# V-Sense/LFBM5D

Hardware: AMD Instinct MI355X
Metric: SAI-megapixels/sec (HT+Wiener, sigma=25) (higher is better)
Workload: dtype f32; 1 GPU; lf17x17x512x512_sigma25; light_field=17x17x512x512x3, asw=1, color_space=opp, noise=MT19937 seed 1 (utilities.cpp:176-183), window_lanes=2, spatial_bands=1, parallelism=single GPU

## Files before the change

lfbm5d_amd/core.py:

```python
import ctypes as C
import os
import subprocess

from typing import NamedTuple, Optional

import numpy as np

_HERE = os.path.dirname(os.path.abspath(__file__))

YUV, YCBCR, OPP, RGB, ID, DCT, SADCT, BIOR, HADAMARD, HAAR = range(10)
ROWMAJOR, COLMAJOR = 11, 12
TAU = {"id": ID, "dct": DCT, "sadct": SADCT, "bior": BIOR, "hw": HADAMARD, "haar": HAAR}
COLOR_SPACE = {"yuv": YUV, "ycbcr": YCBCR, "opp": OPP, "rgb": RGB}
UNIQUE_ID_BYTES = 128
SR_BICUBIC, SR_GAUSSIAN = 0, 1
SR_UP, SR_DOWN = 0, 1
SR_KERNEL = {"bicubic": SR_BICUBIC, "gaussian": SR_GAUSSIAN}


class LfBm5dError(RuntimeError):
    pass


class Params(C.Structure):
# ... 136 lines not shown
        L.lfbm5d_sr_backproject_device.argtypes = [vp, sp, fp, fp, up, fp] + [C.c_uint] * 4
        L.lfbm5d_superres_device.argtypes = [vp, sp, pp, fp, up, fp] + [C.c_uint] * 7
        L.lfbm5d_superres_host_sai.argtypes = [vp, sp, pp, fp, up, fp] + [C.c_uint] * 7
    L.lfbm5d_malloc.argtypes = [C.POINTER(vp), C.c_size_t]
    L.lfbm5d_free.argtypes = [vp]
    L.lfbm5d_memcpy_h2d.argtypes = [vp, vp, C.c_size_t]
    L.lfbm5d_memcpy_d2h.argtypes = [vp, vp, C.c_size_t]
    L.lfbm5d_device_count.restype = C.c_int
    _lib = L
    return L


def plan_windows(awidth, aheight, an=1, ang_major=None, mask=None):
    ang_major = ROWMAJOR if ang_major is None else ang_major
    m = np.ones(awidth * aheight, np.uint32) if mask is None else _u32(mask)
    out = np.zeros(awidth * aheight, np.uint32)
    n = lib().lfbm5d_plan_windows(awidth, aheight, an, ang_major, m.ctypes.data_as(C.POINTER(C.c_uint)),
                                  out.ctypes.data_as(C.POINTER(C.c_uint)), out.size)
    if n < 0:
        raise LfBm5dError("lfbm5d_plan_windows: bad arguments")
    return out[:n].copy()


def plan_graph(awidth, aheight, world, lanes=1, an=1, ang_major=None, mask=None):
    ang_major = ROWMAJOR if ang_major is None else ang_major
    m = np.ones(awidth * aheight, np.uint32) if mask is None else _u32(mask)
    mp = m.ctypes.data_as(C.POINTER(C.c_uint))
    n = lib().lfbm5d_plan_graph(awidth, aheight, an, ang_major, mp, world, lanes, None, None, None, 0)
    if n < 0:
        raise LfBm5dError("lfbm5d_plan_graph: bad arguments")
    r, l, t = (np.zeros(max(n, 1), np.uint32) for _ in range(3))
    p = lambda a: a.ctypes.data_as(C.POINTER(C.c_uint))
    lib().lfbm5d_plan_graph(awidth, aheight, an, ang_major, mp, world, lanes, p(r), p(l), p(t), n)
    return r[:n], l[:n], t[:n]


def plan_messages(awidth, aheight, world, an=1, ang_major=None, mask=None):
    ang_major = ROWMAJOR if ang_major is None else ang_major
    m = np.ones(awidth * aheight, np.uint32) if mask is None else _u32(mask)
    mp = m.ctypes.data_as(C.POINTER(C.c_uint))
    n = lib().lfbm5d_plan_messages(awidth, aheight, an, ang_major, mp, world, None, 0)
    if n < 0:
        raise LfBm5dError("lfbm5d_plan_messages: bad arguments")
    out = np.zeros((max(n, 1), 4), np.uint32)
    lib().lfbm5d_plan_messages(awidth, aheight, an, ang_major, mp, world, out.ctypes.data_as(C.POINTER(C.c_uint)), n)
    return out[:n]


def plan_job(awidth, aheight, world, lanes=1, an=(1, 1), cost=None, ang_major=None, mask=None):
    ang_major = ROWMAJOR if ang_major is None else ang_major
    m = np.ones(awidth * aheight, np.uint32) if mask is None else _u32(mask)
    p = lambda a: a.ctypes.data_as(C.POINTER(C.c_uint))
    an_a = _u32(list(an))
    cost_a = _u32(list(cost)) if cost is not None else None
    cnt = np.zeros(4, np.uint32)
    n = lib().lfbm5d_plan_job(awidth, aheight, ang_major, p(m), len(an_a), p(an_a), p(cost_a) if cost_a is not None else None,
                              world, lanes, None, 0, None, 0, p(cnt))
    if n < 0:
        raise LfBm5dError("lfbm5d_plan_job: bad arguments")
    nodes = np.zeros((max(int(cnt[0]), 1), 8), np.uint32)
    msgs = np.zeros((max(int(cnt[1]), 1), 6), np.uint32)
    lib().lfbm5d_plan_job(awidth, aheight, ang_major, p(m), len(an_a), p(an_a), p(cost_a) if cost_a is not None else None,
                          world, lanes, p(nodes), int(cnt[0]), p(msgs), int(cnt[1]), p(cnt))
    return nodes[:int(cnt[0])], msgs[:int(cnt[1])], {"windows": int(cnt[0]), "messages": int(cnt[1]), "makespan": int(cnt[2]),
                                                     "centre_ok": bool(cnt[3])}


def auto_bands(awidth, aheight, height, halo, world):
    return int(lib().lfbm5d_auto_bands(int(awidth), int(aheight), int(height), int(halo), int(world)))


def noise_level_statistic(cov):
    cov = np.ascontiguousarray(cov, np.float64)
    d = cov.shape[0]
    sig, m, lam = C.c_double(), C.c_uint(), np.zeros(d, np.float64)
    dp = C.POINTER(C.c_double)
    if lib().lfbm5d_noise_level_statistic(d, cov.ctypes.data_as(dp), C.byref(sig), C.byref(m), lam.ctypes.data_as(dp)) != 0:
        raise LfBm5dError("lfbm5d_noise_level_statistic: bad arguments (d must be 1..64)")
    return sig.value, m.value, lam


def sr_defaults(scale, /, **changes):
    sr = SrParams()
    if lib().lfbm5d_sr_defaults(int(scale), C.byref(sr)) != 0:
        raise LfBm5dError("lfbm5d_sr_defaults: scale must be 2, 3 or 4")
    for k, v in changes.items():
        if k == "kernel" and isinstance(v, str):
            v = SR_KERNEL[v]
        if k not in dict(SrParams._fields_):
            raise LfBm5dError(f"SrParams has no field {k}")
        setattr(sr, k, v)
    return sr


def sr_taps(op, sr, n_in):
    op = {"up": SR_UP, "down": SR_DOWN}.get(op, op)
    T = C.c_uint(0)
    if lib().lfbm5d_sr_taps(int(op), C.byref(sr), int(n_in), None, None, C.byref(T), 0) != 0:
        raise LfBm5dError("lfbm5d_sr_taps: rejected parameters (scale, kernel, blur_sigma, n_in)")
    n_out = int(n_in) * sr.scale if op == SR_UP else int(n_in) // sr.scale
    first, w = np.zeros(n_out, np.int32), np.zeros((n_out, T.value), np.float32)
    if lib().lfbm5d_sr_taps(int(op), C.byref(sr), int(n_in), first.ctypes.data, w.ctypes.data, C.byref(T), w.size) != 0:
        raise LfBm5dError("lfbm5d_sr_taps failed")
    return first, w


def shard_rows(n_rows, rank, world):
    b, e = C.c_uint(), C.c_uint()
    lib().lfbm5d_shard_rows(n_rows, rank, world, C.byref(b), C.byref(e))
    return b.value, e.value


def make_params(sigma, lam, N, nSim, nDisp, k, p, tau_2D, tau_4D, tau_5D, useSD=0, color_space=OPP):
    t = lambda v: TAU[v] if isinstance(v, str) else int(v)
    cs = COLOR_SPACE[color_space] if isinstance(color_space, str) else int(color_space)
    return Params(float(sigma), float(lam), int(N), int(nSim), int(nDisp), int(k), int(p),
                  int(bool(useSD)), t(tau_2D), t(tau_4D), t(tau_5D), cs)


def make_bm3d_params(sigma, lam, N, nHW, k, p, tau_2D, useSD=0, color_space=OPP):
    cs = COLOR_SPACE[color_space] if isinstance(color_space, str) else int(color_space)
    return Bm3dParams(float(sigma), float(lam), int(N), int(nHW), int(k), int(p), int(bool(useSD)),
                      TAU[tau_2D] if isinstance(tau_2D, str) else int(tau_2D), cs)


def _u32(a):
    return np.ascontiguousarray(np.asarray(a, dtype=np.uint32))


def _dev_ptr(t):
    import torch
    if not (isinstance(t, torch.Tensor) and t.is_cuda and t.dtype == torch.float32 and t.is_contiguous()):
        raise LfBm5dError("device entry points need contiguous float32 CUDA tensors")
    torch.cuda.current_stream(t.device).synchronize()
    return C.c_void_p(t.data_ptr())


def _sai_ptrs(arrays, mask):
    out = (C.c_void_p * len(arrays))()
    for i, a in enumerate(arrays):
        if a is None or not mask[i]:
            continue
        if not (isinstance(a, np.ndarray) and a.dtype == np.float32 and a.flags.c_contiguous):
            raise LfBm5dError("per-SAI host buffers must be contiguous float32 numpy arrays")
        out[i] = a.ctypes.data
    return out


OPTION_ENV = ("LFBM5D_LANES", "LFBM5D_EMULATE_WORLD", "LFBM5D_MAX_WINDOWS", "LFBM5D_FUSED", "LFBM5D_STEP_SHARDING",
              "LFBM5D_DATA_DRIVEN_SCHEDULE", "LFBM5D_HOST_BLOCKING", "LFBM5D_BAND_MB", "LFBM5D_BM3D_LANES", "LFBM5D_SCAN_LDS_CAP",
              "LFBM5D_FORCE_REDO", "LFBM5D_SPATIAL_BANDS", "LFBM5D_BAND_HALO", "LFBM5D_SCAN_V1", "LFBM5D_SCAN_ANY", "LFBM5D_SCAN_FULL_TABLES", "LFBM5D_DCT8W_V2",
              "LFBM5D_GROUP_GENERIC", "LFBM5D_NO_SA_KERNELS", "LFBM5D_NO_SLAB_KERNEL", "LFBM5D_WIDE_NOSPLIT", "LFBM5D_AGG_64BIT",
              "LFBM5D_AGG_SCALAR_SCAN", "LFBM5D_SUBSET_LIST_HOST", "LFBM5D_SUBSET_SCAN_V1", "LFBM5D_FILT_GROUP_MAJOR",
              "LFBM5D_HT_REF_ORDER", "LFBM5D_WINDOW_SUMS_PADDED")
OPTION_ENV_EMPTY_OFF = ("LFBM5D_WINDOW_SUMS_PADDED",)


class Context:

    def __init__(self, device=0):
        self._L = lib()
        h = C.c_void_p()
        if self._L.lfbm5d_create(C.byref(h), int(device)) != 0:
            raise LfBm5dError(self._L.lfbm5d_last_error(None).decode())
        self._handle = h
        self._env_seen = {k: os.environ.get(k) for k in OPTION_ENV}
        self.device = int(device)

    @property
    def _h(self):
        h = self._handle
        if h and hasattr(self._L, "lfbm5d_set_option"):
            for k in OPTION_ENV:
                v = os.environ.get(k)
                if v != self._env_seen[k]:
                    self._env_seen[k] = v
                    if not v and k in OPTION_ENV_EMPTY_OFF:
                        v = None
                    self._L.lfbm5d_set_option(h, k.encode(), None if v is None else (v or "1").encode())
        return h

    def set_option(self, key, value):
        if self._L.lfbm5d_set_option(self._handle, key.encode(), None if value is None else str(value).encode()) != 0:
            raise LfBm5dError(self._L.lfbm5d_last_error(self._handle).decode())

    def get_option(self, key):
        buf = C.create_string_buffer(64)
        if self._L.lfbm5d_get_option(self._handle, key.encode(), buf, 64) != 0:
            raise LfBm5dError(self._L.lfbm5d_last_error(self._handle).decode())
        return buf.value.decode()

    def close(self):
        if getattr(self, "_handle", None):
            self._L.lfbm5d_destroy(self._handle)
            self._handle = None

    def __del__(self):
        try:
            self.close()
        except Exception:
            pass

    def _ck(self, rc):
        if rc != 0:
            raise LfBm5dError(self._L.lfbm5d_last_error(self._h).decode())

    @staticmethod
    def unique_id():
        buf = (C.c_ubyte * UNIQUE_ID_BYTES)()
        if lib().lfbm5d_comm_unique_id(buf) != 0:
            raise LfBm5dError("ncclGetUniqueId failed")
        return bytes(buf)

    def comm_init(self, unique_id, rank, world):
        buf = (C.c_ubyte * UNIQUE_ID_BYTES).from_buffer_copy(unique_id)
        self._ck(self._L.lfbm5d_comm_init(self._h, buf, rank, world))

    def comm_init_ipc(self, rank, world, rendezvous_dir, timeout_s=30.0):
        self._ck(self._L.lfbm5d_comm_init_ipc(self._h, rank, world, os.fsencode(rendezvous_dir), float(timeout_s)))

    def comm_selftest(self, n=1 << 20):
        self._ck(self._L.lfbm5d_comm_selftest(self._h, n))

    def comm_ranks(self):
        return int(self._L.lfbm5d_comm_ranks(self._h))

    def set_shard(self, rank, world):
        self._ck(self._L.lfbm5d_set_shard(self._h, rank, world))

    def set_tiles(self, nb_tiles):
        self._ck(self._L.lfbm5d_set_tiles(self._h, int(nb_tiles)))

    def reset_stats(self):
        self._L.lfbm5d_reset_stats(self._h)

    def stats(self):
        s = Stats()
        self._L.lfbm5d_get_stats(self._h, C.byref(s))
        return s

    def stream(self):
        return self._L.lfbm5d_stream(self._h)

    def step1(self, P, noisy, mask, basic, ang_major, awidth, aheight, an, W, H, Cc):
        m = _u32(mask)
        mp = m.ctypes.data_as(C.POINTER(C.c_uint))
        tail = (ang_major, awidth, aheight, an, W, H, Cc)
        if isinstance(noisy, (list, tuple)):
            self._ck(self._L.lfbm5d_step1_host_sai(self._h, C.byref(P), _sai_ptrs(noisy, m), mp, _sai_ptrs(basic, m), *tail))
        elif isinstance(noisy, np.ndarray):
            self._ck(self._L.lfbm5d_step1_host(self._h, C.byref(P), noisy.ctypes.data_as(C.c_void_p), mp,
                                               basic.ctypes.data_as(C.c_void_p), *tail))
        else:
            self._ck(self._L.lfbm5d_step1_device(self._h, C.byref(P), _dev_ptr(noisy), mp, _dev_ptr(basic), *tail))

    def step2(self, P, noisy, mask, basic, denoised, ang_major, awidth, aheight, an, W, H, Cc):
        m = _u32(mask)
        mp = m.ctypes.data_as(C.POINTER(C.c_uint))
        tail = (ang_major, awidth, aheight, an, W, H, Cc)
        if isinstance(noisy, (list, tuple)):
            self._ck(self._L.lfbm5d_step2_host_sai(self._h, C.byref(P), _sai_ptrs(noisy, m), mp, _sai_ptrs(basic, m), _sai_ptrs(denoised, m), *tail))
        elif isinstance(noisy, np.ndarray):
            self._ck(self._L.lfbm5d_step2_host(self._h, C.byref(P), noisy.ctypes.data_as(C.c_void_p), mp,
                                               basic.ctypes.data_as(C.c_void_p),
                                               denoised.ctypes.data_as(C.c_void_p), *tail))
        else:
            self._ck(self._L.lfbm5d_step2_device(self._h, C.byref(P), _dev_ptr(noisy), mp, _dev_ptr(basic),
                                                 _dev_ptr(denoised), *tail))

    def denoise(self, P1, P2, noisy, mask, basic, denoised, ang_major, awidth, aheight, an1, an2, W, H, Cc):
        m = _u32(mask)
        mp = m.ctypes.data_as(C.POINTER(C.c_uint))
        tail = (ang_major, awidth, aheight, an1, an2, W, H, Cc)
        if isinstance(noisy, (list, tuple)):
            self._ck(self._L.lfbm5d_denoise_host_sai(self._h, C.byref(P1), C.byref(P2), _sai_ptrs(noisy, m), mp, _sai_ptrs(basic, m),
                                                     _sai_ptrs(denoised, m), *tail))
        elif isinstance(noisy, np.ndarray):
            self._ck(self._L.lfbm5d_denoise_host(self._h, C.byref(P1), C.byref(P2), noisy.ctypes.data_as(C.c_void_p), mp,
                                                 basic.ctypes.data_as(C.c_void_p), denoised.ctypes.data_as(C.c_void_p), *tail))
        else:
            self._ck(self._L.lfbm5d_denoise_device(self._h, C.byref(P1), C.byref(P2), _dev_ptr(noisy), mp, _dev_ptr(basic),
                                                   _dev_ptr(denoised), *tail))

    def core_pass(self, step, P, aw, ah, Wb, Hb, Cc, noisy, basic, num, den, mask, procSAI, cst, pst):
        m, pr = _u32(mask), _u32(procSAI)
        self._ck(self._L.lfbm5d_pass_device(
            self._h, step, C.byref(P), aw, ah, Wb, Hb, Cc, _dev_ptr(noisy),
            _dev_ptr(basic) if basic is not None else None, _dev_ptr(num), _dev_ptr(den),
            m.ctypes.data_as(C.POINTER(C.c_uint)), pr.ctypes.data_as(C.POINTER(C.c_uint)), cst, pst))

    def bm3d_step(self, step, P, Wb, Hb, Cc, noisy, basic, out):
        self._ck(self._L.lfbm5d_bm3d_step_device(self._h, step, C.byref(P), Wb, Hb, Cc, _dev_ptr(noisy),
                                                 _dev_ptr(basic) if basic is not None else None, _dev_ptr(out)))

    def bm3d_lf(self, hard, wien, noisy, mask, basic, denoised, W, H, Cc):
        m = _u32(mask)
        mp = m.ctypes.data_as(C.POINTER(C.c_uint))
        if isinstance(noisy, np.ndarray):
            self._ck(self._L.lfbm5d_bm3d_lf_host(self._h, C.byref(hard), C.byref(wien), noisy.ctypes.data_as(C.c_void_p), mp,
                                                 basic.ctypes.data_as(C.c_void_p), denoised.ctypes.data_as(C.c_void_p),
                                                 m.size, W, H, Cc))
        else:
            self._ck(self._L.lfbm5d_bm3d_lf_device(self._h, C.byref(hard), C.byref(wien), _dev_ptr(noisy), mp, _dev_ptr(basic),
                                                   _dev_ptr(denoised), m.size, W, H, Cc))

    def noise_level(self, LF, LF_SAI_mask, width, height, chnls, patch=8, per_sai=False):
        m = _u32(LF_SAI_mask)
# ... 192 lines not shown
```

lfbm5d_amd/csrc/lfbm5d_aggregate.hip:

```cpp
#include "lfbm5d_kernels.h"

#include <algorithm>
#include <cstdlib>

namespace lfbm5d {

namespace {



constexpr int kAggFlush = 64;
template <bool WINDOWED, int TW, int TH, int kAggPF, int kAggU, bool BIG, bool VEC4>
__global__ __launch_bounds__(64) __attribute__((amdgpu_waves_per_eu((VEC4 && TW == 8 && !BIG) ? 8 : 1))) void k_aggregate(AggArgs a) {
    constexpr int kAggCap = kAggFlush + kAggPF * 64 + kAggU;
    __shared__ uint4 hit_a[kAggCap];
    __shared__ float hit_w2[kAggCap];
    __shared__ float kai[WINDOWED ? 256 : 1];
    const int lane = threadIdx.x;
    const unsigned org = a.direct ? a.nHW : 0u, Wt = a.Wb - 2 * org, Ht = a.Hb - 2 * org;
    const unsigned gx = (Wt + TW - 1) / TW, gy = (Ht + TH - 1) / TH, total_wg = gx * gy * a.A;
    const unsigned per_xcd = gridDim.x / 8;
    const unsigned lin2 = (blockIdx.x % 8) * per_xcd + blockIdx.x / 8;
    if (lin2 >= total_wg) return;
    const int st = (int)(lin2 / (gx * gy));
    const int tile_y = (int)((lin2 / gx) % gy), tile_x = (int)(lin2 % gx);
    if (a.proc_bits.test((unsigned)st)) return;
    if (!a.mask_bits.test((unsigned)st)) return;
    const int tx0 = (int)org + tile_x * TW, ty0 = (int)org + tile_y * TH;
    const int x = tx0 + lane % TW, y = ty0 + lane / TW;
    const bool inside = x < (int)(org + Wt) && y < (int)(org + Ht);
    const int k = a.k, k2 = k * k, C = a.C, N = a.N, A = a.A;
    const int logN = 31 - __builtin_clz((unsigned)N);
    const size_t plane = (size_t)Wt * Ht;
    const int reach = (st == (int)a.pst) ? (int)a.nSim : (int)a.nHW;
    if (WINDOWED) for (int i = lane; i < k2; i += 64) kai[i] = a.tb->kaiser[i];

    const int last_r = (int)a.Hb - k - (int)a.nHW, last_c = (int)a.Wb - k - (int)a.nHW;
    auto lo_idx = [&](int v) { int d = v - (int)a.nHW; return d <= 0 ? 0 : (d + (int)a.p - 1) / (int)a.p; };
    auto hi_idx = [&](int v, int n, int lastv) {
        if (v >= lastv) return n - 1;
        int d = v - (int)a.nHW; if (d < 0) return -1;
        int i = d / (int)a.p; return i > n - 2 ? n - 2 : i;
    };
    int r_lo = lo_idx(ty0 - k + 1 - reach), r_hi = hi_idx(ty0 + TH - 1 + reach, (int)a.n_ref_rows, last_r);
    int c_lo = lo_idx(tx0 - k + 1 - reach), c_hi = hi_idx(tx0 + TW - 1 + reach, (int)a.n_ref_cols, last_c);
    if (r_lo > (int)a.n_ref_rows - 1) r_lo = (int)a.n_ref_rows - 1;
    if (c_lo > (int)a.n_ref_cols - 1) c_lo = (int)a.n_ref_cols - 1;
    if (!a.irregular && a.n_ref_cols) {
        r_lo = max(r_lo, (int)(a.ref_begin / a.n_ref_cols));
        r_hi = min(r_hi, (int)((a.ref_begin + a.n_groups - 1) / a.n_ref_cols));
    }
    const int ncols_span = c_hi - c_lo + 1;
    const int n_rr = a.irregular ? (int)a.n_groups : ((r_hi >= r_lo && c_hi >= c_lo) ? (r_hi - r_lo + 1) * ncols_span : 0);
    const int n_cand = n_rr << logN;
    if (n_cand == 0) return;

    float accn[3] = {0, 0, 0}, accd[3] = {0, 0, 0};
    const size_t pix = (a.direct ? (size_t)a.sai.st[st] * a.lf_stride : (size_t)st * C * plane) + (size_t)(y - (int)org) * Wt + (size_t)(x - (int)org);
    if (inside) for (int c = 0; c < C; c++) { accn[c] = a.num[pix + c * plane]; accd[c] = a.den[pix + c * plane]; }

    const bool mul_div = !a.irregular && (long long)n_rr * ncols_span < (1 << 20);
    const unsigned div_m = ((1u << 20) + (unsigned)max(ncols_span, 1) - 1) / (unsigned)max(ncols_span, 1);
    const unsigned g_end = a.ref_begin + a.n_groups;
    const bool sai_major = a.filt_sai_stride != 0;
    const unsigned Af = sai_major ? 1u : (unsigned)A, stf = sai_major ? 0u : (unsigned)st;
    const float* const filt = a.filt + (sai_major ? (size_t)st * a.filt_sai_stride : (size_t)0);
    const unsigned long long filt_bytes = sai_major ? a.filt_sai_stride * sizeof(float) : a.filt_bytes;
    const bool small24 = (((unsigned long long)a.n_refs_total << logN) + 1) * Af < (1ull << 24);
    const unsigned* apos = a.aggpos + (size_t)st * a.n_refs_total * N;
    const unsigned cstride = C > 1 ? (unsigned)k2 * 4u : 0u;
    const __amdgpu_buffer_rsrc_t rs_filt = __builtin_amdgcn_make_buffer_rsrc((void*)filt, 0, BIG ? 0 : (int)(unsigned)filt_bytes, 0x00020000u);
    unsigned nh = 0;

    auto consume = [&]() {
        const unsigned nh_pad = (nh + kAggU - 1) / kAggU * kAggU;
        if (nh + lane < nh_pad) { hit_a[nh + lane] = make_uint4(0xffffffffu, 0u, 0u, 0u); hit_w2[nh + lane] = 0.0f; }
        __builtin_amdgcn_wave_barrier();
        for (unsigned h0 = 0; h0 < nh_pad; h0 += kAggU) {
            float val[kAggU][3], kw[kAggU][3];
#pragma unroll
            for (int u = 0; u < kAggU; u++) {
                const uint4 ha = hit_a[h0 + u];
                const float w2 = hit_w2[h0 + u];
                const int dy = y - (int)(ha.x >> 16), dx = x - (int)(ha.x & 0xffffu);
                const bool on = (unsigned)dy < (unsigned)k && (unsigned)dx < (unsigned)k;
                const unsigned o = __umul24((unsigned)min(max(dy, 0), k - 1), (unsigned)k) + (unsigned)min(max(dx, 0), k - 1);
                const float kz = WINDOWED ? kai[o] : 1.0f;
                if (BIG) {
                    const char* fp = reinterpret_cast<const char*>(filt) + ((size_t)ha.y + o) * 4;
                    val[u][0] = *reinterpret_cast<const float*>(fp);
                    val[u][1] = *reinterpret_cast<const float*>(fp + cstride);
                    val[u][2] = *reinterpret_cast<const float*>(fp + 2 * cstride);
                } else {
                    const int vo = (int)((ha.y + o) * 4u);
                    val[u][0] = __builtin_bit_cast(float, __builtin_amdgcn_raw_buffer_load_b32(rs_filt, vo, 0, kFiltLoadAux));
                    val[u][1] = __builtin_bit_cast(float, __builtin_amdgcn_raw_buffer_load_b32(rs_filt, vo, (int)cstride, kFiltLoadAux));
                    val[u][2] = __builtin_bit_cast(float, __builtin_amdgcn_raw_buffer_load_b32(rs_filt, vo, (int)(2 * cstride), kFiltLoadAux));
                }
                kw[u][0] = on ? kz * __uint_as_float(ha.z) : 0.0f;
                kw[u][1] = on ? kz * __uint_as_float(ha.w) : 0.0f;
                kw[u][2] = on ? kz * w2 : 0.0f;
            }
#pragma unroll
            for (int u = 0; u < kAggU; u++)
#pragma unroll
                for (int c = 0; c < 3; c++) {
#pragma clang fp contract(off)
                    accn[c] += kw[u][c] * val[u][c];
                    accd[c] += kw[u][c];
                }
        }
        nh = 0;
        __builtin_amdgcn_wave_barrier();
    };

    __builtin_amdgcn_wave_barrier();
    if (VEC4) {
        constexpr unsigned cap_hits = (unsigned)(kAggCap - kAggU);
        const unsigned lo_y = (unsigned)(ty0 - k + 1), lo_x = (unsigned)(tx0 - k + 1);
        const unsigned span_y = (unsigned)(TH + k - 1), span_x = (unsigned)(TW + k - 1);
        const unsigned pstep = Af * (unsigned)(C * k2);
        auto try_append = [&](const int c0, const unsigned l0, const unsigned l1) -> bool {
            const int e = c0 + lane * 4;
            unsigned g = 0, n0 = 0;
            uint4 p4 = make_uint4(0xffffffffu, 0xffffffffu, 0xffffffffu, 0xffffffffu);
            if (e < n_cand && (unsigned)lane >= l0 && (unsigned)lane < l1) {
                n0 = (unsigned)e & (unsigned)(N - 1);
                const unsigned rr = (unsigned)e >> logN;
                if (a.irregular) g = a.ref_begin + rr;
                else {
                    unsigned q = __umul24(rr, div_m) >> 20;
                    if (!mul_div) { asm volatile("" ::: "memory"); q = rr / (unsigned)ncols_span; }
                    g = __umul24((unsigned)r_lo + q, a.n_ref_cols) + (unsigned)c_lo + (rr - __umul24(q, (unsigned)ncols_span));
                }
                if (g >= a.ref_begin && g < g_end) p4 = *reinterpret_cast<const uint4*>(apos + ((size_t)g << logN) + n0);
            }
            const unsigned pj[4] = {p4.x, p4.y, p4.z, p4.w};
            unsigned m4 = 0;
#pragma unroll
            for (int j = 0; j < 4; j++) {
                const bool h = ((pj[j] >> 16) - lo_y) < span_y && ((pj[j] & 0xffffu) - lo_x) < span_x;
                m4 |= h ? (1u << j) : 0u;
            }
            const unsigned cnt = (unsigned)__popc(m4);
            const unsigned long long b0 = __ballot(cnt & 1u), b1 = __ballot(cnt & 2u), b2 = __ballot(cnt & 4u);
            auto below = [&](unsigned long long b) { return __builtin_amdgcn_mbcnt_hi((unsigned)(b >> 32), __builtin_amdgcn_mbcnt_lo((unsigned)b, 0u)); };
            const unsigned total = (unsigned)__popcll(b0) + 2u * (unsigned)__popcll(b1) + 4u * (unsigned)__popcll(b2);
            if (nh + total > cap_hits) return false;
            if (m4) {
                unsigned slot = nh + below(b0) + 2u * below(b1) + 4u * below(b2);
                size_t wbase; unsigned off;
                const unsigned gl = g - a.ref_begin;
                if (small24) { wbase = __umul24(g, (unsigned)C); off = __umul24(__umul24((gl << logN) + n0, Af) + stf, (unsigned)(C * k2)); }
                else { asm volatile("" ::: "memory"); wbase = (size_t)g * C; off = (((gl << logN) + n0) * Af + stf) * C * k2; }
                float w[3];
#pragma unroll
                for (int c = 0; c < 3; c++) w[c] = c < C ? a.wgt[wbase + (a.wchan0 ? 0 : c)] : 0.0f;
#pragma unroll
                for (int j = 0; j < 4; j++) {
                    if (m4 & (1u << j)) {
                        hit_a[slot] = make_uint4(pj[j], off, __float_as_uint(w[0]), __float_as_uint(w[1]));
                        hit_w2[slot] = w[2];
                        slot++;
                    }
                    off += pstep;
                }
            }
            nh += total;
            __builtin_amdgcn_wave_barrier();
            return true;
        };
        for (int c0 = 0; c0 < n_cand; c0 += 256) {
            if (!try_append(c0, 0u, 64u))
                for (unsigned l0 = 0; l0 < 64; l0 += 16) { consume(); (void)try_append(c0, l0, l0 + 16); }
            if (nh >= kAggFlush) consume();
        }
    } else
    for (int c0 = 0; c0 < n_cand; c0 += 64 * kAggPF) {
        unsigned g[kAggPF], p[kAggPF], nn[kAggPF];
#pragma unroll
        for (int u = 0; u < kAggPF; u++) {
            const int e = c0 + u * 64 + lane;
            p[u] = 0xffffffffu; g[u] = 0; nn[u] = 0;
            if (e < n_cand) {
                const unsigned n = (unsigned)e & (unsigned)(N - 1), rr = (unsigned)e >> logN;
                nn[u] = n;
                if (a.irregular) g[u] = a.ref_begin + rr;
                else {
                    unsigned q = __umul24(rr, div_m) >> 20;
                    if (!mul_div) { asm volatile("" ::: "memory"); q = rr / (unsigned)ncols_span; }
                    g[u] = __umul24((unsigned)r_lo + q, a.n_ref_cols) + (unsigned)c_lo + (rr - __umul24(q, (unsigned)ncols_span));
                }
                if (g[u] >= a.ref_begin && g[u] < g_end) p[u] = apos[((size_t)g[u] << logN) + n];
            }
        }
        bool hit[kAggPF];
        float w[kAggPF][3];
        size_t wbase[kAggPF];
        if (small24) {
#pragma unroll
            for (int u = 0; u < kAggPF; u++) wbase[u] = __umul24(g[u], (unsigned)C);
        } else {
            asm volatile("" ::: "memory");
#pragma unroll
            for (int u = 0; u < kAggPF; u++) wbase[u] = (size_t)g[u] * C;
        }
#pragma unroll
        for (int u = 0; u < kAggPF; u++) {
            const int py = (int)(p[u] >> 16), px = (int)(p[u] & 0xffffu);
            hit[u] = p[u] != 0xffffffffu && py < ty0 + TH && py + k > ty0 && px < tx0 + TW && px + k > tx0;
#pragma unroll
            for (int c = 0; c < 3; c++) w[u][c] = (hit[u] && c < C) ? a.wgt[wbase[u] + (a.wchan0 ? 0 : c)] : 0.0f;
        }
#pragma unroll
        for (int u = 0; u < kAggPF; u++) {
            const unsigned long long bal = __ballot(hit[u]);
            if (hit[u]) {
                const unsigned slot = nh + __popcll(bal & ((1ull << lane) - 1ull));
                unsigned off;
                const unsigned gl = g[u] - a.ref_begin;
                if (small24) off = __umul24(__umul24((gl << logN) + nn[u], Af) + stf, (unsigned)(C * k2));
                else { asm volatile("" ::: "memory"); off = (((gl << logN) + nn[u]) * Af + stf) * C * k2; }
                hit_a[slot] = make_uint4(p[u], off, __float_as_uint(w[u][0]), __float_as_uint(w[u][1]));
                hit_w2[slot] = w[u][2];
            }
            nh += __popcll(bal);
        }
        __builtin_amdgcn_wave_barrier();
        if (nh >= kAggFlush) consume();
    }
    if (nh) consume();
    if (inside) for (int c = 0; c < C; c++) { a.num[pix + c * plane] = accn[c]; a.den[pix + c * plane] = accd[c]; }
}

}

hipError_t launch_aggregate(hipStream_t s, const AggArgs& a) {
    const bool wide = a.k >= 12;
    constexpr int kAgg16TW = 16, kAgg16TH = 4, kAgg8TW = 8, kAgg8TH = 8;
    const unsigned tw = wide ? (a.k == 12 ? 16 : kAgg16TW) : (a.k == 8 ? kAgg8TW : 8), th = wide ? (a.k == 12 ? 4 : kAgg16TH) : (a.k == 8 ? kAgg8TH : 8);
    const unsigned org = a.direct ? a.nHW : 0u;
    const unsigned tiles = ((a.Wb - 2 * org + tw - 1) / tw) * ((a.Hb - 2 * org + th - 1) / th) * a.A;
    const dim3 grid(((tiles + 7) / 8) * 8), block(64);
    const bool big = (a.filt_sai_stride ? a.filt_sai_stride * sizeof(float) : a.filt_bytes) > 0xfffff000ull || (a.opt & kOptAgg64Bit);
    const bool vec4 = a.N % 4 == 0 && !wide && !(a.opt & kOptAggScalarScan);
#define LFBM5D_AGG(W_, TW_, TH_, PF_, U_) \
    do { if (big && vec4) hipLaunchKernelGGL((k_aggregate<W_, TW_, TH_, PF_, U_, true, true>), grid, block, 0, s, a); \
         else if (big)    hipLaunchKernelGGL((k_aggregate<W_, TW_, TH_, PF_, U_, true, false>), grid, block, 0, s, a); \
         else if (vec4)   hipLaunchKernelGGL((k_aggregate<W_, TW_, TH_, PF_, U_, false, true>), grid, block, 0, s, a); \
         else             hipLaunchKernelGGL((k_aggregate<W_, TW_, TH_, PF_, U_, false, false>), grid, block, 0, s, a); } while (0)
    constexpr int kAgg16PF = 3, kAgg16U = 12, kAgg8PF = 3, kAgg8U = 6;
    if (a.k == 12)      LFBM5D_AGG(true, 16, 4, 3, 12);
    else if (a.k == 8)  LFBM5D_AGG(true, kAgg8TW, kAgg8TH, kAgg8PF, kAgg8U);
    else if (wide)      LFBM5D_AGG(false, kAgg16TW, kAgg16TH, kAgg16PF, kAgg16U);
    else                LFBM5D_AGG(false, 8, 8, 2, 6);
#undef LFBM5D_AGG
    return hipGetLastError();
}

}
```

lfbm5d_amd/csrc/lfbm5d_group_device.h:

```cpp
#ifndef LFBM5D_GROUP_DEVICE_H
#define LFBM5D_GROUP_DEVICE_H

#include "lfbm5d_kernels.h"

#include <algorithm>
#include <cstdlib>
#include <type_traits>

namespace lfbm5d {

hipError_t launch_group_ht(hipStream_t s, const GroupArgs& a, bool all_sa, bool* launched);
hipError_t launch_group_wiener(hipStream_t s, const GroupArgs& a, bool all_sa, bool* launched);
hipError_t launch_group_wide(hipStream_t s, const GroupArgs& a, bool* launched);
hipError_t prepare_group_wide();
hipError_t launch_group_slab(hipStream_t s, const GroupArgs& a, bool* launched);
hipError_t prepare_group_slab();
bool group_uses_slab(const GroupArgs& a);
size_t group_slab_scratch_bytes(const GroupArgs& a);
hipError_t prepare_group_ht();
hipError_t prepare_group_wiener();
constexpr int kDedicatedLdsLimit = 160 * 1024 - 4096;

namespace {

typedef const __attribute__((address_space(4))) GroupTables* TbPtr;
typedef const __attribute__((address_space(4))) float* TbFloats;
static inline dim3 grid1d(size_t n, unsigned b = 256) { return dim3((unsigned)((n + b - 1) / b)); }


constexpr int kThreads = 256;

template <int MA, int MW>
struct ShapeInfoT {
    int mask[MA], idx[MA], mask_col[MA], idx_col[MA], mask_dct[MA];
    int row_n[MW], col_n[MW];
    int use_sadct;
};
typedef ShapeInfoT<kMaxA, kMaxAw> ShapeInfo;
typedef ShapeInfoT<kBigA, kBigAw> ShapeInfoBig;
static_assert(sizeof(ShapeInfo) == kShapeInfoBytes && sizeof(ShapeInfoBig) == kShapeInfoBigBytes, "GroupArgs::gshape stride");
typedef const __attribute__((address_space(4))) ShapeInfo& ShRef;
typedef const __attribute__((address_space(4))) ShapeInfoBig& ShRefBig;
__device__ __forceinline__ int window_side(int A) { int w = 1; while (w * w < A) w++; return w; }

template <class SH>
__device__ void build_shape(SH& sh, const int* m, int aw) {
    const int A = aw * aw;
    int size = 0;
    for (int i = 0; i < A; i++) { sh.mask[i] = m[i]; sh.idx[i] = 0; sh.mask_col[i] = 0; sh.idx_col[i] = 0; sh.mask_dct[i] = 0; size += m[i]; }
    for (int s = 0; s < aw; s++) {
        int r = 0;
        for (int t = 0; t < aw; t++) if (m[s * aw + t]) sh.idx[s * aw + r++] = t;
        sh.row_n[s] = r;
        for (int t = 0; t < r; t++) sh.mask_col[s * aw + t] = 1;
    }
    for (int t = 0; t < aw; t++) {
        int r = 0;
        for (int s = 0; s < aw; s++) if (sh.mask_col[s * aw + t]) sh.idx_col[(r++) * aw + t] = s;
        sh.col_n[t] = r;
        for (int s = 0; s < r; s++) sh.mask_dct[s * aw + t] = 1;
    }
    sh.use_sadct = size != A;
}

__device__ __forceinline__ void dct9_fwd(float* x, TbPtr tb) {
    float t[9];
#pragma unroll
    for (int s = 0; s < 3; s++)
#pragma unroll
        for (int u = 0; u < 3; u++)
            t[s * 3 + u] = 2.0f * (x[s * 3] * tb->cos3[u * 3] + x[s * 3 + 1] * tb->cos3[u * 3 + 1] + x[s * 3 + 2] * tb->cos3[u * 3 + 2]);
#pragma unroll
    for (int v = 0; v < 3; v++)
#pragma unroll
        for (int u = 0; u < 3; u++)
            x[v * 3 + u] = 2.0f * (t[u] * tb->cos3[v * 3] + t[3 + u] * tb->cos3[v * 3 + 1] + t[6 + u] * tb->cos3[v * 3 + 2]) * tb->cn4[v * 3 + u];
}
__device__ __forceinline__ void dct9_inv(float* x, TbPtr tb) {
    float t[9];
#pragma unroll
    for (int i = 0; i < 9; i++) x[i] *= tb->cni4[i];
#pragma unroll
    for (int s = 0; s < 3; s++)
#pragma unroll
        for (int j = 0; j < 3; j++)
            t[s * 3 + j] = x[s * 3] + 2.0f * (x[s * 3 + 1] * tb->cos3[3 + j] + x[s * 3 + 2] * tb->cos3[6 + j]);
#pragma unroll
    for (int i = 0; i < 3; i++)
#pragma unroll
        for (int j = 0; j < 3; j++)
            x[i * 3 + j] = (t[j] + 2.0f * (t[3 + j] * tb->cos3[3 + i] + t[6 + j] * tb->cos3[6 + i])) * tb->coef4inv;
}

typedef float v2f __attribute__((ext_vector_type(2)));
typedef float v4f __attribute__((ext_vector_type(4)));
struct __attribute__((packed, aligned(4))) f4u { float v[4]; };
__device__ __forceinline__ void dct9_fwd2(v2f* x, TbPtr tb) {
#pragma clang fp contract(on)
    v2f t[9];
#pragma unroll
    for (int s = 0; s < 3; s++)
#pragma unroll
        for (int u = 0; u < 3; u++)
            t[s * 3 + u] = 2.0f * (x[s * 3] * tb->cos3[u * 3] + x[s * 3 + 1] * tb->cos3[u * 3 + 1] + x[s * 3 + 2] * tb->cos3[u * 3 + 2]);
#pragma unroll
    for (int v = 0; v < 3; v++)
#pragma unroll
        for (int u = 0; u < 3; u++)
            x[v * 3 + u] = 2.0f * (t[u] * tb->cos3[v * 3] + t[3 + u] * tb->cos3[v * 3 + 1] + t[6 + u] * tb->cos3[v * 3 + 2]) * tb->cn4[v * 3 + u];
}
__device__ __forceinline__ void dct9_inv2(v2f* x, TbPtr tb) {
    v2f t[9];
#pragma unroll
    for (int i = 0; i < 9; i++) x[i] *= tb->cni4[i];
#pragma unroll
    for (int s = 0; s < 3; s++)
#pragma unroll
        for (int j = 0; j < 3; j++)
            t[s * 3 + j] = x[s * 3] + 2.0f * (x[s * 3 + 1] * tb->cos3[3 + j] + x[s * 3 + 2] * tb->cos3[6 + j]);
#pragma unroll
    for (int i = 0; i < 3; i++)
#pragma unroll
        for (int j = 0; j < 3; j++)
            x[i * 3 + j] = (t[j] + 2.0f * (t[3 + j] * tb->cos3[3 + i] + t[6 + j] * tb->cos3[6 + i])) * tb->coef4inv;
}
__device__ __forceinline__ void dct9_fwd2_fast(v2f* x, TbPtr tb) {
    const float c2 = 2.0f * tb->cos3[3];
    v2f t[9];
#pragma unroll
    for (int s = 0; s < 3; s++) {
        const v2f a = x[s * 3] + x[s * 3 + 2];
        t[s * 3] = 2.0f * (a + x[s * 3 + 1]);
        t[s * 3 + 1] = c2 * (x[s * 3] - x[s * 3 + 2]);
        t[s * 3 + 2] = a - 2.0f * x[s * 3 + 1];
    }
#pragma unroll
    for (int u = 0; u < 3; u++) {
        const v2f a = t[u] + t[6 + u];
        x[u] = (a + t[3 + u]) * (2.0f * tb->cn4[u]);
        x[3 + u] = (t[u] - t[6 + u]) * (c2 * tb->cn4[3 + u]);
        x[6 + u] = (a - 2.0f * t[3 + u]) * tb->cn4[6 + u];
    }
}
__device__ __forceinline__ void dct9_inv2_fast(v2f* x, TbPtr tb) {
    const float c2 = 2.0f * tb->cos3[3];
    v2f t[9];
#pragma unroll
    for (int s = 0; s < 3; s++) {
        const v2f X0 = x[s * 3] * tb->cni4[s * 3], X1 = x[s * 3 + 1] * (c2 * tb->cni4[s * 3 + 1]), X2 = x[s * 3 + 2] * tb->cni4[s * 3 + 2];
        const v2f p = X0 + X2;
        t[s * 3] = p + X1; t[s * 3 + 1] = X0 - 2.0f * X2; t[s * 3 + 2] = p - X1;
    }
#pragma unroll
    for (int j = 0; j < 3; j++) {
        const v2f T0 = t[j] * tb->coef4inv, T1 = t[3 + j] * (c2 * tb->coef4inv), T2 = t[6 + j] * tb->coef4inv;
        const v2f p = T0 + T2;
        x[j] = p + T1; x[3 + j] = T0 - 2.0f * T2; x[6 + j] = p - T1;
    }
}
template <int NS> __device__ __forceinline__ void haar_fwd_pairs(v2f* P) {
#pragma clang fp contract(on)
    const float s = 0.70710678118654752f;
    if (NS == 8) {
        const v2f S01 = (P[0] + P[1]) * s, D01 = (P[0] - P[1]) * s, S23 = (P[2] + P[3]) * s, D23 = (P[2] - P[3]) * s;
        const v2f SS = (S01 + S23) * s, DD = (S01 - S23) * s;
// ... 1191 lines not shown
```

lfbm5d_amd/csrc/lfbm5d_group_generic.hip:

```cpp
#include "lfbm5d_group_device.h"

namespace lfbm5d {

namespace {

__global__ __launch_bounds__(256) void k_group_pos(GroupArgs a) {
    const int A = a.A, N = a.N, NA = N * A;
    const size_t plane = (size_t)a.Wb * a.Hb;
    const size_t idx = (size_t)blockIdx.x * blockDim.x + threadIdx.x;
    if (idx == 0 && a.sa_list) a.sa_list[0] = 0u;
    if (idx >= (size_t)a.n_groups * N) return;
    const unsigned g = a.ref_begin + (unsigned)(idx / N);
    const int n = (int)(idx % N);
    const int nSx = (int)a.self_cnt[g];
    const unsigned k_r = a.refs[g];
    const unsigned ind_pst = n < nSx ? a.self_idx[(size_t)g * N + n] : 0u;
    const bool want_ofs = A == 9 && a.tau2 == 4 && a.step == 1 && (size_t)A * a.C * plane * 4 < 0x7fffffffull;
    unsigned bits = 0;
    for (int st = 0; st < A; st++) {
        const bool masked = a.mask_bits.test((unsigned)st);
        unsigned p = 0xffffffffu;
        if (n < nSx && masked) p = (st == (int)a.pst) ? ind_pst : a.best[(size_t)st * plane + ind_pst];
        const bool zero_patch = a.fill_quirk && p != 0xffffffffu && (p % a.Wb) >= a.Wb - a.k;
        const int i = n * A + st;
        a.gpos[(size_t)g * NA + i] = zero_patch ? 0xffffffffu : p;
        if (want_ofs) {
            const bool there = !zero_patch && p != 0xffffffffu;
            a.gofs[(size_t)g * NA + i] = there ? (unsigned)(((size_t)st * a.C * plane + p) * 4) : 0u;
            bits |= there ? 1u << st : 0u;
        }
        const bool in_shape = st == (int)a.pst || (masked && a.shape[(size_t)st * plane + k_r]);
        a.aggpos[((size_t)st * a.n_refs_total + g) * N + n] = ((a.tau4 != 6 || in_shape) && p != 0xffffffffu) ? ((p / a.Wb) << 16) | (p % a.Wb) : 0xffffffffu;
    }
    if (want_ofs) a.gok[(size_t)g * N + n] = bits;
}
template <bool BIG>
__global__ __launch_bounds__(256) void k_group_shape(GroupArgs a) {
    typedef typename std::conditional<BIG, ShapeInfoBig, ShapeInfo>::type SH;
    const unsigned i = blockIdx.x * blockDim.x + threadIdx.x;
    if (i >= a.n_groups) return;
    const unsigned g = a.ref_begin + i;
    const size_t plane = (size_t)a.Wb * a.Hb;
    const unsigned k_r = a.refs[g];
    SH* out = reinterpret_cast<SH*>(a.gshape) + g;
    if (a.tau4 != 6) { out->use_sadct = 0; return; }
    const int A = (int)a.A, aw = window_side(A);
    if (BIG) {
        int* m = out->mask_dct;
        int full = 0;
        for (int st = 0; st < A; st++) {
            const bool masked = a.mask_bits.test((unsigned)st);
            m[st] = (st == (int)a.pst || (masked && a.shape[(size_t)st * plane + k_r])) ? 1 : 0;
            full += m[st];
        }
        if (full == A) { out->use_sadct = 0; return; }
        for (int st = 0; st < A; st++) out->mask[st] = m[st];
        build_shape(*out, out->mask, aw);
        return;
    }
    SH sh;
    int m[BIG ? 1 : kMaxA], full = 0;
    for (int st = 0; st < A; st++) {
        const bool masked = a.mask_bits.test((unsigned)st);
        m[st] = (st == (int)a.pst || (masked && a.shape[(size_t)st * plane + k_r])) ? 1 : 0;
        full += m[st];
    }
    if (full == A) { out->use_sadct = 0; return; }
    build_shape(sh, m, aw);
    for (int q = 0; q < A; q++) {
        out->mask[q] = sh.mask[q]; out->idx[q] = sh.idx[q]; out->mask_col[q] = sh.mask_col[q];
        out->idx_col[q] = sh.idx_col[q]; out->mask_dct[q] = sh.mask_dct[q];
    }
    for (int q = 0; q < aw; q++) { out->row_n[q] = sh.row_n[q]; out->col_n[q] = sh.col_n[q]; }
    out->use_sadct = sh.use_sadct;
    if (sh.use_sadct && a.sa_list) a.sa_list[1u + atomicAdd(&a.sa_list[0], 1u)] = g | (7u << 29);
}
template <int STEP, bool BIG = false>
__device__ __forceinline__ void group_generic(const GroupArgs& a, const unsigned g, const int c, float* S0, float* S1, float* tmp,
                                              unsigned* pos, float (*red)[kThreads / 64]) {
    const int tid = threadIdx.x;
    const int k = a.k, k2 = k * k, A = a.A, N = a.N;
    const int aw = window_side(A);
    const int nSx = (int)a.self_cnt[g];
    const size_t plane = (size_t)a.Wb * a.Hb;
    const int stack = nSx * A * k2;
    const TbPtr tb = (TbPtr)a.tb;

    for (int i = tid; i < nSx * A; i += kThreads) pos[i] = a.gpos[(size_t)g * N * A + i];
    typename std::conditional<BIG, ShRefBig, ShRef>::type sh = [&]() -> typename std::conditional<BIG, ShRefBig, ShRef>::type {
        if constexpr (BIG) return group_shape_big(a, g); else return group_shape(a, g); }();
    __syncthreads();
    const bool use_sadct = a.tau4 == 6 && sh.use_sadct;

    {
        constexpr int G = 12;
        for (int e0 = tid; e0 < stack; e0 += kThreads * G) {
            float v0[G], v1[G];
#pragma unroll
            for (int u = 0; u < G; u++) {
                const int e = e0 + u * kThreads;
                v0[u] = 0.0f; v1[u] = 0.0f;
                if (e < stack) {
                    const int pq = e % k2, ns = e / k2;
                    const int st = ns % A;
                    const unsigned p = pos[ns];
                    if (p != 0xffffffffu) {
                        const size_t off = ((size_t)st * a.C + c) * plane + p + (size_t)(pq / k) * a.Wb + pq % k;
                        v0[u] = a.noisy[off];
                        if (STEP == 2) v1[u] = a.basic[off];
                    }
                }
            }
#pragma unroll
            for (int u = 0; u < G; u++) {
                const int e = e0 + u * kThreads;
                if (e < stack) { S0[e] = v0[u]; if (STEP == 2) S1[e] = v1[u]; }
            }
        }
    }
    __syncthreads();

    if (a.tau2 != 4) {
        fwd2d(S0, tmp, nSx * A, k, a.tau2, tb);
        if (STEP == 2) fwd2d(S1, tmp, nSx * A, k, a.tau2, tb);
    }

    const bool do_dct4 = a.tau4 == 5 || (a.tau4 == 6 && !use_sadct);
    const bool do_sa4 = !do_dct4 && a.tau4 == 6;
    if (do_dct4 || do_sa4) {
        for (int f = tid; f < nSx * k2; f += kThreads) {
            const int n = f / k2, pq = f % k2;
            for (int s = 0; s < (STEP == 2 ? 2 : 1); s++) {
                float* S = s ? S1 : S0;
                if constexpr (BIG) {
                    float x[kBigA], t[kBigA];
                    for (int st = 0; st < A; st++) x[st] = S[(size_t)(n * A + st) * k2 + pq];
                    if (do_dct4) dctw_fwd_rt(x, t, aw, tb); else sadctw_fwd<ShRefBig>(x, aw, sh, tb);
                    for (int st = 0; st < A; st++) S[(size_t)(n * A + st) * k2 + pq] = x[st];
                } else
                if (A == 9) {
                    float x[9];
#pragma unroll
                    for (int st = 0; st < 9; st++) x[st] = S[(n * A + st) * k2 + pq];
                    if (do_dct4) dct9_fwd(x, tb); else sadct9_fwd(x, sh, tb);
#pragma unroll
                    for (int st = 0; st < 9; st++) S[(n * A + st) * k2 + pq] = x[st];
                } else if (do_dct4 && A == 25) {
                    float x[25];
#pragma unroll
                    for (int st = 0; st < 25; st++) x[st] = S[(n * 25 + st) * k2 + pq];
                    dctw_fwd_t<5>(x, tb);
#pragma unroll
                    for (int st = 0; st < 25; st++) S[(n * 25 + st) * k2 + pq] = x[st];
                } else if (do_dct4) {
                    float x[49];
#pragma unroll
                    for (int st = 0; st < 49; st++) x[st] = S[(n * 49 + st) * k2 + pq];
                    dctw_fwd_t<7>(x, tb);
#pragma unroll
                    for (int st = 0; st < 49; st++) S[(n * 49 + st) * k2 + pq] = x[st];
                } else {
                    float x[kMaxA];
                    for (int st = 0; st < A; st++) x[st] = S[(n * A + st) * k2 + pq];
                    if constexpr (!BIG) sadctw_fwd<ShRef>(x, aw, sh, tb);
                    for (int st = 0; st < A; st++) S[(n * A + st) * k2 + pq] = x[st];
                }
            }
        }
        __syncthreads();
    }

    float wacc = 0.0f, s1 = 0.0f, s2 = 0.0f;
    {
        const float sig = a.sigma[c];
        const float T = a.bm3d ? a.lambda * sig : a.lambda * sig * 1.41421356237309505f;
        const float sig2 = sig * sig;
        for (int f = tid; f < A * k2; f += kThreads) {
            const int st = f / k2, pq = f % k2;
            const bool in_shape = !use_sadct || sh.mask_dct[st];
            const int base = st * k2 + pq, stride = A * k2;
            switch (nSx) {
                case 1:  filter5<1, STEP>(S0, S1, base, stride, a.tau5, T, sig2, in_shape, wacc, s1, s2, tb); break;
                case 2:  filter5<2, STEP>(S0, S1, base, stride, a.tau5, T, sig2, in_shape, wacc, s1, s2, tb); break;
                case 4:  filter5<4, STEP>(S0, S1, base, stride, a.tau5, T, sig2, in_shape, wacc, s1, s2, tb); break;
                case 8:  filter5<8, STEP>(S0, S1, base, stride, a.tau5, T, sig2, in_shape, wacc, s1, s2, tb); break;
                case 16: filter5<16, STEP>(S0, S1, base, stride, a.tau5, T, sig2, in_shape, wacc, s1, s2, tb); break;
                default: filter5<32, STEP>(S0, S1, base, stride, a.tau5, T, sig2, in_shape, wacc, s1, s2, tb); break;   
            }
        }
    }
    for (int o = 32; o > 0; o >>= 1) { wacc += __shfl_xor(wacc, o); s1 += __shfl_xor(s1, o); s2 += __shfl_xor(s2, o); }
    if ((tid & 63) == 0) { red[0][tid >> 6] = wacc; red[1][tid >> 6] = s1; red[2][tid >> 6] = s2; }
    __syncthreads();
    if (tid == 0) {
        float w = 0.0f, m = 0.0f, q = 0.0f;
        for (int i = 0; i < kThreads / 64; i++) { w += red[0][i]; m += red[1][i]; q += red[2][i]; }
        float wx;
        if (a.useSD) {
            const float Nn = a.bm3d ? (float)(nSx * k2) : (float)(nSx * A);
            const float res = (q - m * m / Nn) / (Nn - 1.0f);
            wx = res > 0.0f ? 1.0f / sqrtf(res) : 0.0f;
        } else {
            const float sig = a.sigma[c];
            wx = w > 0.0f ? (sig > 0.0f ? 1.0f / (sig * sig * w) : 1.0f / w) : 1.0f;
        }
        a.wgt[(size_t)g * a.C + c] = wx;
        if (c == 0) {
            atomicAdd(&a.counters[0], (unsigned long long)nSx);
            if (use_sadct) atomicAdd(&a.counters[1], 1ull);
        }
    }
    float* F = STEP == 2 ? S1 : S0;

    if (do_dct4 || do_sa4) {
        for (int f = tid; f < nSx * k2; f += kThreads) {
            const int n = f / k2, pq = f % k2;
            if constexpr (BIG) {
                float x[kBigA], t[kBigA];
                for (int st = 0; st < A; st++) x[st] = F[(size_t)(n * A + st) * k2 + pq];
                if (do_dct4) dctw_inv_rt(x, t, aw, tb); else sadctw_inv<ShRefBig>(x, aw, sh, tb);
                for (int st = 0; st < A; st++) F[(size_t)(n * A + st) * k2 + pq] = x[st];
            } else
            if (A == 9) {
                float x[9];
#pragma unroll
                for (int st = 0; st < 9; st++) x[st] = F[(n * A + st) * k2 + pq];
                if (do_dct4) dct9_inv(x, tb); else sadct9_inv(x, sh, tb);
#pragma unroll
                for (int st = 0; st < 9; st++) F[(n * A + st) * k2 + pq] = x[st];
            } else if (do_dct4 && A == 25) {
                float x[25];
#pragma unroll
                for (int st = 0; st < 25; st++) x[st] = F[(n * 25 + st) * k2 + pq];
                dctw_inv_t<5>(x, tb);
#pragma unroll
                for (int st = 0; st < 25; st++) F[(n * 25 + st) * k2 + pq] = x[st];
            } else if (do_dct4) {
                float x[49];
#pragma unroll
                for (int st = 0; st < 49; st++) x[st] = F[(n * 49 + st) * k2 + pq];
                dctw_inv_t<7>(x, tb);
#pragma unroll
                for (int st = 0; st < 49; st++) F[(n * 49 + st) * k2 + pq] = x[st];
            } else {
                float x[kMaxA];
                for (int st = 0; st < A; st++) x[st] = F[(n * A + st) * k2 + pq];
                if constexpr (!BIG) sadctw_inv<ShRef>(x, aw, sh, tb);
                for (int st = 0; st < A; st++) F[(n * A + st) * k2 + pq] = x[st];
            }
        }
    }
    __syncthreads();
    if (a.tau2 != 4) inv2d(F, tmp, nSx * A, k, a.tau2, tb);

    for (int e = tid; e < stack; e += kThreads) {
        const int pq = e % k2, ns = e / k2;
        filt_put(&a.filt[filt_patch(a, g, ns / A, ns % A, k2) + (size_t)c * k2 + pq], F[e]);
    }
}

template <int STEP>
__global__ __launch_bounds__(kThreads) void k_group(GroupArgs a) {
    extern __shared__ float lds[];
    __shared__ unsigned pos[kMaxN3 * kMaxA];
    __shared__ float red[3][kThreads / 64];
    const unsigned g = a.ref_begin + blockIdx.x;
    const int stack = (int)a.self_cnt[g] * (int)a.A * (int)(a.k * a.k);
    group_generic<STEP>(a, g, (int)blockIdx.y, lds, STEP == 2 ? lds + stack : nullptr, lds + (STEP == 2 ? 2 : 1) * stack, pos, red);
}

template <int STEP, bool BIG>
__global__ __launch_bounds__(kThreads) void k_group_big(GroupArgs a, float* scratch, unsigned long long slice_floats, unsigned tmp_floats) {
    extern __shared__ float lds[];
    __shared__ unsigned pos_small[BIG ? 1 : kMaxN3 * kMaxA];
    __shared__ float red[3][kThreads / 64];
    unsigned* pos = BIG ? reinterpret_cast<unsigned*>(lds + tmp_floats) : pos_small;
    float* S0 = scratch + (size_t)blockIdx.x * slice_floats;
    const unsigned items = a.n_groups * a.C;
    for (unsigned it = blockIdx.x; it < items; it += gridDim.x) {
        const unsigned g = a.ref_begin + it / a.C;
        const int stack = (int)a.self_cnt[g] * (int)a.A * (int)(a.k * a.k);
        group_generic<STEP, BIG>(a, g, (int)(it % a.C), S0, STEP == 2 ? S0 + stack : nullptr, lds, pos, red);
        __syncthreads();
    }
}

}

constexpr int kGenericLdsLimit = 160 * 1024 - 8192;
hipError_t prepare_group_kernels() {
    const void* fns[] = {reinterpret_cast<const void*>(&k_group<1>), reinterpret_cast<const void*>(&k_group<2>)};
    for (const void* f : fns) {
        const hipError_t e = hipFuncSetAttribute(f, hipFuncAttributeMaxDynamicSharedMemorySize, kGenericLdsLimit);
        if (e != hipSuccess) return e;
    }
    hipError_t e = prepare_group_ht();
    if (e == hipSuccess) e = prepare_group_wiener();
    if (e == hipSuccess) e = prepare_group_wide();
    if (e == hipSuccess) e = prepare_group_slab();
    return e;
}

constexpr unsigned kBigBlocks = 1024;
static size_t group_tmp_floats(const GroupArgs& a) {
    const bool rows_form = (a.tau2 == 7 && (a.k == 8 || a.k == 16)) || (a.tau2 == 5 && (a.k == 8 || a.k == 12 || a.k == 16));
    return rows_form ? (size_t)(kThreads / a.k) * a.k * (a.k + 1) : std::max<size_t>(256, (size_t)a.k * a.k);
}
size_t group_lds_bytes(const GroupArgs& a) {
    const size_t stack = (size_t)a.N * a.A * a.k * a.k;
    return ((a.step == 2 ? 2 : 1) * stack + group_tmp_floats(a)) * sizeof(float);
}
static bool group_uses_generic(const GroupArgs& a) {
    if (a.opt & kOptGroupGeneric) return true;
    bool wide_window = false;
    for (unsigned w = 5; w <= 17; w += 2) wide_window |= a.A == w * w;
    if (wide_window && a.tau2 == 4 && a.step == 1 && !a.bm3d && a.N <= 8 && a.k * a.k <= 256 && (size_t)a.A * a.C * a.Wb * a.Hb * 4 < 0x7fffffffull) return false;
    if (a.A != 9 && !(a.bm3d && a.A == 1)) return true;
    if (a.A == 9 && a.tau2 == 4 && a.N <= 8 && a.k * a.k <= 256 && a.step == 1) return false;
    if (a.A == 9 && (a.tau2 == 7 || a.tau2 == 5) && a.k == 16 && a.N <= 8 && a.step == 1) return false;
    if (a.A == 9 && a.tau2 == 7 && a.k == 8 && a.step == 2 && a.N <= (unsigned)kMaxN) return false;
    if (a.A == 9 && a.tau2 == 5 && a.k == 8 && a.N <= (unsigned)kMaxN) return false;
    if (a.bm3d && a.A == 1 && a.k == 8 && a.tau5 == 8 && (a.tau2 == 5 || a.tau2 == 7)) return false;
    return true;
}
size_t group_scratch_bytes(const GroupArgs& a) {
    if (group_uses_generic(a) && !(a.opt & kOptGroupGeneric) && group_uses_slab(a)) return group_slab_scratch_bytes(a);
    if (!group_uses_generic(a) || (group_lds_bytes(a) <= (size_t)kGenericLdsLimit && a.A <= (unsigned)kMaxA)) return 0;
    return (size_t)kBigBlocks * (a.step == 2 ? 2 : 1) * a.N * a.A * a.k * a.k * sizeof(float);
}
hipError_t launch_group(hipStream_t s, const GroupArgs& a) {
    hipLaunchKernelGGL(k_group_pos, grid1d((size_t)a.n_groups * a.N), dim3(256), 0, s, a);
    const bool bigA = a.A > (unsigned)kMaxA;
    if (bigA) hipLaunchKernelGGL(k_group_shape<true>, grid1d(a.n_groups), dim3(256), 0, s, a);
    else      hipLaunchKernelGGL(k_group_shape<false>, grid1d(a.n_groups), dim3(256), 0, s, a);
    const bool all_sa = a.tau4 == 6 && !a.mask_bits.holds_all(a.A) && !(a.opt & kOptNoSaKernels);
    if (!(a.opt & kOptGroupGeneric)) {
        bool launched = false;
        hipError_t e = launch_group_ht(s, a, all_sa, &launched);
        if (launched) return e;
        e = launch_group_wiener(s, a, all_sa, &launched);
        if (launched) return e;
        e = launch_group_wide(s, a, &launched);
        if (launched) return e;
        e = launch_group_slab(s, a, &launched);
        if (launched) return e;
    }
    const size_t lds = group_lds_bytes(a);
    if (lds > (size_t)kGenericLdsLimit || bigA) {
        const unsigned long long slice = (unsigned long long)(a.step == 2 ? 2 : 1) * a.N * a.A * a.k * a.k;
        if (!a.scratch || a.scratch_floats < slice * kBigBlocks) return hipErrorInvalidValue;
        const unsigned blocks = std::min<unsigned>(kBigBlocks, a.n_groups * a.C);
        const unsigned tf = (unsigned)group_tmp_floats(a);
        const size_t ltmp = (size_t)tf * sizeof(float) + (bigA ? (size_t)a.N * a.A * sizeof(unsigned) : 0);
        if (bigA) {
            if (a.step == 2) hipLaunchKernelGGL((k_group_big<2, true>), dim3(blocks), dim3(kThreads), ltmp, s, a, a.scratch, slice, tf);
            else             hipLaunchKernelGGL((k_group_big<1, true>), dim3(blocks), dim3(kThreads), ltmp, s, a, a.scratch, slice, tf);
        }
        else if (a.step == 2) hipLaunchKernelGGL((k_group_big<2, false>), dim3(blocks), dim3(kThreads), ltmp, s, a, a.scratch, slice, tf);
        else                  hipLaunchKernelGGL((k_group_big<1, false>), dim3(blocks), dim3(kThreads), ltmp, s, a, a.scratch, slice, tf);
        return hipGetLastError();
    }
    if (a.step == 2) hipLaunchKernelGGL(k_group<2>, dim3(a.n_groups, a.C), dim3(kThreads), lds, s, a);
    else             hipLaunchKernelGGL(k_group<1>, dim3(a.n_groups, a.C), dim3(kThreads), lds, s, a);
    return hipGetLastError();
}
}
```

lfbm5d_amd/csrc/lfbm5d_group_ht.hip:

```cpp
#include "lfbm5d_group_device.h"

namespace lfbm5d {

namespace {

__device__ __forceinline__ constexpr float ht_guard(int st) { return st == 0 ? 1.0f / 65536.0f : (st == 3 || st == 6) ? 1.0f / 131072.0f : 1.0f / 262144.0f; }
template <int NS> __device__ __forceinline__ void haar_fwd_pairs_u(v2f* P) {
    if (NS == 8) {
        const v2f S01 = P[0] + P[1], D01 = P[0] - P[1], S23 = P[2] + P[3], D23 = P[2] - P[3];
        const v2f SS = S01 + S23, DD = S01 - S23;
        P[0] = v2f{SS.x + SS.y, SS.x - SS.y}; P[1] = DD; P[2] = D01; P[3] = D23;
    } else if (NS == 4) {
        const v2f S = P[0] + P[1], D = P[0] - P[1];
        P[0] = v2f{S.x + S.y, S.x - S.y}; P[1] = D;
    } else if (NS == 2) {
        P[0] = v2f{P[0].x + P[0].y, P[0].x - P[0].y};
    }
}
template <int NS> __device__ __forceinline__ void haar_inv_pairs_u(v2f* P) {
    if (NS == 8) {
        const v2f X = v2f{P[0].x + P[0].y, P[0].x - P[0].y};
        const v2f U = P[1] * 2.0f + X, V = X - P[1] * 2.0f, D01 = P[2], D23 = P[3];
        P[0] = D01 * 4.0f + U; P[1] = U - D01 * 4.0f; P[2] = D23 * 4.0f + V; P[3] = V - D23 * 4.0f;
    } else if (NS == 4) {
// ... 26 lines not shown
            const v2f p = t[u] + t[6 + u];
            V[h][u] = p + t[3 + u]; V[h][3 + u] = t[u] - t[6 + u]; V[h][6 + u] = p - 2.0f * t[3 + u];
        }
    }
    const float inv_n = 1.0f / (float)NS;
    unsigned kept = 0;
    unsigned long long near = 0ull;
#pragma unroll
    for (int st = 0; st < 9; st++) {
        v2f P[NH];
#pragma unroll
        for (int h = 0; h < NH; h++) P[h] = V[h][st];
        haar_fwd_pairs_u<NS>(P);
        const float gs = fmaxf(ht_guard(st), a.ht3_K[c][st] * M);
#pragma unroll
        for (int h = 0; h < NH; h++) {
            const int lvl = h == 0 ? LV : (NS == 8 && h == 1) ? 2 : 1;
            const float Tq = a.ht3_T[c][st][lvl], Gq = Tq * gs;
            const float ax = fabsf(P[h].x), ay = fabsf(P[h].y);
            const bool kx = ax > Tq, ky = (NS > 1) && ay > Tq;
            near |= __ballot(fabsf(ax - Tq) < Gq);
            if (NS > 1) near |= __ballot(fabsf(ay - Tq) < Gq);
            kept += (unsigned)__popcll(__ballot(kx)) + (NS > 1 ? (unsigned)__popcll(__ballot(ky)) : 0u);
            P[h].x = kx ? P[h].x : 0.0f;
            P[h].y = ky ? P[h].y : 0.0f;
        }
        haar_inv_pairs_u<NS>(P);
#pragma unroll
        for (int h = 0; h < NH; h++) V[h][st] = P[h];
    }
    if (near) return true;
    wacc += (__lane_id() == 0) ? (float)kept : 0.0f;
    if (a.useSD) {
#pragma unroll
        for (int h = 0; h < NH; h++)
#pragma unroll
            for (int st = 0; st < 9; st++) {
                const v2f y = V[h][st] * (tb->ht3_f[st] * inv_n);
                s1 += y.x; s2 += y.x * y.x;
                if (NS > 1) { s1 += y.y; s2 += y.y * y.y; }
            }
    }
#pragma unroll
    for (int h = 0; h < NH; h++) {
        v2f t[9];
#pragma unroll
        for (int s = 0; s < 3; s++) {
            const v2f Z0 = V[h][s * 3] * (tb->ht3_gf[s * 3] * inv_n), Z1 = V[h][s * 3 + 1] * (tb->ht3_gf[s * 3 + 1] * inv_n), Z2 = V[h][s * 3 + 2] * (tb->ht3_gf[s * 3 + 2] * inv_n);
            const v2f p = Z0 + Z2;
            t[s * 3] = p + Z1; t[s * 3 + 1] = Z0 - 2.0f * Z2; t[s * 3 + 2] = p - Z1;
        }
#pragma unroll
        for (int j = 0; j < 3; j++) {
            const v2f p = t[j] + t[6 + j];
            V[h][j] = p + t[3 + j]; V[h][3 + j] = t[j] - 2.0f * t[6 + j]; V[h][6 + j] = p - t[3 + j];
        }
    }
    return false;
}

template <int NS, bool HAAR, int SA_MODE = 0>
__device__ __forceinline__ void group_id_compute(const GroupArgs& a, int c, ShRef sh, bool use_sadct, v2f (&V)[NS > 1 ? NS / 2 : 1][9],
                                                 float& wacc, float& s1, float& s2, float* sa_lds = nullptr) {
    constexpr int NH = NS > 1 ? NS / 2 : 1;
    const TbPtr tb = (TbPtr)a.tb;
    const bool do_dct4 = a.tau4 == 5 || (a.tau4 == 6 && !use_sadct);
    const bool do_sa4 = SA_MODE != 3 && !do_dct4 && a.tau4 == 6;
    auto sadct_pairs = [&](bool fwd) {
#pragma unroll
        for (int h = 0; h < NH; h++)
#pragma unroll
            for (int half = 0; half < (NS > 1 ? 2 : 1); half++) {
                if (SA_MODE == 1) {
#pragma unroll
                    for (int i = 0; i < 9; i++) sa_lds[i] = half ? V[h][i].y : V[h][i].x;
                    if (fwd) sadct9_fwd_lds(sa_lds, sh, tb); else sadct9_inv_lds(sa_lds, sh, tb);
#pragma unroll
                    for (int i = 0; i < 9; i++) { if (half) V[h][i].y = sa_lds[i]; else V[h][i].x = sa_lds[i]; }
                } else {
                    float t9[9];
#pragma unroll
                    for (int i = 0; i < 9; i++) t9[i] = half ? V[h][i].y : V[h][i].x;
                    if (SA_MODE == 2) { if (fwd) sadct9_fwd_sel(t9, sh, tb); else sadct9_inv_sel(t9, sh, tb); }
                    else if (fwd) sadct9_fwd(t9, sh, tb); else sadct9_inv(t9, sh, tb);
#pragma unroll
                    for (int i = 0; i < 9; i++) { if (half) V[h][i].y = t9[i]; else V[h][i].x = t9[i]; }
                }
            }
    };
    if (do_dct4) {
#pragma unroll
        for (int h = 0; h < NH; h++) dct9_fwd2(V[h], tb);
    } else if (do_sa4) sadct_pairs(true);
    const float sig = a.sigma[c];
    const float T = a.lambda * sig * 1.41421356237309505f;
#pragma unroll
    for (int st = 0; st < 9; st++) {
        const bool in_shape = !use_sadct || sh.mask_dct[st];
        if (HAAR) {
            v2f P[NH];
#pragma unroll
            for (int h = 0; h < NH; h++) P[h] = V[h][st];
            haar_fwd_pairs<NS>(P);
            if (in_shape) {
#pragma unroll
                for (int h = 0; h < NH; h++) {
                    const bool kx = fabsf(P[h].x) > T, ky = (NS > 1) && fabsf(P[h].y) > T;
                    wacc += (kx ? 1.0f : 0.0f) + (ky ? 1.0f : 0.0f);
                    P[h].x = kx ? P[h].x : 0.0f;
                    P[h].y = ky ? P[h].y : 0.0f;
                }
            }
            haar_inv_pairs<NS>(P);
#pragma unroll
            for (int h = 0; h < NH; h++) V[h][st] = P[h];
        } else {
            float o[NS], e[1] = {0.0f};
#pragma unroll
            for (int n = 0; n < NS; n++) o[n] = n < NH ? V[n][st].x : V[n - NH][st].y;
            shrink_fibre<NS, 1>(o, e, a.tau5, T, sig * sig, in_shape, wacc, tb);
#pragma unroll
            for (int n = 0; n < NS; n++) { if (n < NH) V[n][st].x = o[n]; else V[n - NH][st].y = o[n]; }
        }
    }
    if (a.useSD) {
#pragma unroll
        for (int h = 0; h < NH; h++)
#pragma unroll
            for (int st = 0; st < 9; st++) {
                s1 += V[h][st].x; s2 += V[h][st].x * V[h][st].x;
                if (NS > 1) { s1 += V[h][st].y; s2 += V[h][st].y * V[h][st].y; }
            }
    }
    if (do_dct4) {
#pragma unroll
        for (int h = 0; h < NH; h++) dct9_inv2(V[h], tb);
    } else if (do_sa4) sadct_pairs(false);
}

template <int NS, bool HAAR, bool LDSW = false, int SA_MODE = 0, bool FAST = false>
__device__ __forceinline__ bool group_id_body(const GroupArgs& a, unsigned g, int c, int pq, const __attribute__((address_space(4))) unsigned* pos,
                                              ShRef sh, bool use_sadct, float& wacc, float& s1, float& s2, float* work = nullptr) {
    const int k = a.k, k2 = k * k, A = 9;
    const unsigned plane = a.Wb * a.Hb;
    const unsigned kRsrcFlags = 0x00020000u;
    const __amdgpu_buffer_rsrc_t rs_in = __builtin_amdgcn_make_buffer_rsrc((void*)a.noisy, 0, (int)((size_t)a.A * a.C * plane * 4), kRsrcFlags);
    float* const out = a.filt + (size_t)g * a.N * A * a.C * k2;
    const __amdgpu_buffer_rsrc_t rs_out = __builtin_amdgcn_make_buffer_rsrc((void*)out, 0, (int)((size_t)a.N * A * a.C * k2 * 4), kRsrcFlags);
    constexpr int NH = NS > 1 ? NS / 2 : 1;
    v2f V[NH][9];
    const int voff = (int)(((unsigned)(pq / k) * a.Wb + pq % k) * 4u);
    const int woff = (pq / k) * (k + 1) + pq % k;
    unsigned okbits[NS];
    typedef const __attribute__((address_space(4))) unsigned* cuptr_;
    const cuptr_ ofs = (cuptr_)(a.gofs + (size_t)g * a.N * A), ok = (cuptr_)(a.gok + (size_t)g * a.N);
    const unsigned cbase = (unsigned)c * plane * 4u;
    auto load_all = [&]() {
        if (LDSW) {
#pragma unroll
            for (int n = 0; n < NS; n++)
#pragma unroll
                for (int st = 0; st < 9; st++) {
                    const float x = work[(n * A + st) * kT16Patch + woff];
                    if (n < NH) V[n][st].x = x; else V[n - NH][st].y = x;
                    okbits[n] = 0x1ffu;
                }
        } else
#pragma unroll
        for (int n = 0; n < NS; n++) {
            okbits[n] = ok[n];
#pragma unroll
            for (int st = 0; st < 9; st++) {
                const unsigned so = ofs[n * A + st] + cbase;
                const float x = __builtin_bit_cast(float, __builtin_amdgcn_raw_buffer_load_b32(rs_in, voff, (int)so, 0));
                if (n < NH) V[n][st].x = x; else V[n - NH][st].y = x;
            }
        }
        if (NS == 1) {
#pragma unroll
            for (int st = 0; st < 9; st++) V[0][st].y = 0.0f;
        }
#pragma unroll
        for (int n = 0; n < NS; n++)
            if (okbits[n] != 0x1ffu) {
#pragma unroll
                for (int st = 0; st < 9; st++) {
                    if (n < NH) V[n][st].x = ((okbits[n] >> st) & 1) ? V[n][st].x : 0.0f;
                    else V[n - NH][st].y = ((okbits[n] >> st) & 1) ? V[n - NH][st].y : 0.0f;
                }
            }
    };
    load_all();
    bool near = false;
    if (FAST) near = group_id_compute_fast<NS>(a, c, V, wacc, s1, s2);
    else
    group_id_compute<NS, HAAR, SA_MODE>(a, c, sh, use_sadct, V, wacc, s1, s2);
    const int vout = pq * 4;
#pragma unroll
    for (int n = 0; n < NS; n++)
#pragma unroll
        for (int st = 0; st < 9; st++) {
            const float r = n < NH ? V[n][st].x : V[n - NH][st].y;
            if (LDSW) work[(n * A + st) * kT16Patch + woff] = r;
            else __builtin_amdgcn_raw_buffer_store_b32(__builtin_bit_cast(int, r), rs_out, vout, (int)((((unsigned)(n * A + st) * a.C + c) * k2) * 4u), kFiltStoreAux);
        }
    return near;
}

template <bool HAAR, int SA_MODE, bool FAST = false>
__device__ __forceinline__ void group_id_one(const GroupArgs& a, const unsigned g, const int c, float (*red)[4]) {
    const int tid = threadIdx.x;
    const int A = 9, N = a.N;
    const int nSx = (int)a.self_cnt[g];
    typedef const __attribute__((address_space(4))) unsigned* cuptr;
    const cuptr pos = (cuptr)(a.gpos + (size_t)g * N * A);
    ShRef sh = group_shape(a, g);
    const bool use_sadct = a.tau4 == 6 && sh.use_sadct;
    if (SA_MODE == 3 && use_sadct) return;
    float wacc = 0.0f, s1 = 0.0f, s2 = 0.0f;
    bool near = false;
    if (tid < (int)(a.k * a.k)) {
        switch (nSx) {
            case 1:  near = group_id_body<1, HAAR, false, SA_MODE, FAST>(a, g, c, tid, pos, sh, use_sadct, wacc, s1, s2); break;
            case 2:  near = group_id_body<2, HAAR, false, SA_MODE, FAST>(a, g, c, tid, pos, sh, use_sadct, wacc, s1, s2); break;
            case 4:  near = group_id_body<4, HAAR, false, SA_MODE, FAST>(a, g, c, tid, pos, sh, use_sadct, wacc, s1, s2); break;
            default: near = group_id_body<8, HAAR, false, SA_MODE, FAST>(a, g, c, tid, pos, sh, use_sadct, wacc, s1, s2); break;
        }
    }
    for (int o = 32; o > 0; o >>= 1) { wacc += __shfl_xor(wacc, o); s1 += __shfl_xor(s1, o); s2 += __shfl_xor(s2, o); }
    if ((tid & 63) == 0) { red[0][tid >> 6] = wacc; red[1][tid >> 6] = s1; red[2][tid >> 6] = s2; if (FAST) red[3][tid >> 6] = near ? 1.0f : 0.0f; }
    __syncthreads();
    if (tid == 0) {
        if (FAST) {
            float nr = 0.0f;
            for (unsigned i = 0; i < (blockDim.x + 63) / 64; i++) nr += red[3][i];
            if (nr != 0.0f) {
                a.sa_list[1u + atomicAdd(&a.sa_list[0], 1u)] = g | (1u << (29 + c)); return;
            }
        }
        float w = 0.0f, m = 0.0f, q = 0.0f;
        for (unsigned i = 0; i < (blockDim.x + 63) / 64; i++) { w += red[0][i]; m += red[1][i]; q += red[2][i]; }
        float wx;
        if (a.useSD) {
            const float Nn = (float)(nSx * A);
            const float res = (q - m * m / Nn) / (Nn - 1.0f);
            wx = res > 0.0f ? 1.0f / sqrtf(res) : 0.0f;
        } else {
            const float sig = a.sigma[c];
            wx = w > 0.0f ? (sig > 0.0f ? 1.0f / (sig * sig * w) : 1.0f / w) : 1.0f;
        }
        a.wgt[(size_t)g * a.C + c] = wx;
        if (c == 0) {
            atomicAdd(&a.counters[0], (unsigned long long)nSx);
            if (use_sadct) atomicAdd(&a.counters[1], 1ull);
        }
    }
}

template <bool HAAR, int SA_MODE, bool FAST>
__device__ __forceinline__ void group_id_kernel(const GroupArgs& a) {
    __shared__ float red[4][4];
    const unsigned gi = xcd_group_index(a);
    if (gi >= a.n_groups) return;
    group_id_one<HAAR, SA_MODE, FAST>(a, a.ref_begin + gi, (int)blockIdx.y, red);
}
template <bool HAAR>
__device__ __forceinline__ void group_id_list_kernel(const GroupArgs& a) {
    __shared__ float red[4][4];
    const unsigned n = a.sa_list[0];
    for (unsigned i = blockIdx.x; i < n; i += gridDim.x) {
        const unsigned e = a.sa_list[1u + i];
        for (unsigned c = 0; c < a.C; c++)
            if ((e >> (29 + c)) & 1u) {
                group_id_one<HAAR, 2>(a, e & 0x1fffffffu, (int)c, red);
                __syncthreads();
            }
    }
}
__global__ __launch_bounds__(256) void k_group_id_haar_fast(GroupArgs a) { group_id_kernel<true, 3, true>(a); }
__global__ __launch_bounds__(256) void k_group_id_haar(GroupArgs a) { group_id_kernel<true, 3, false>(a); }
__global__ __launch_bounds__(256) void k_group_id_any(GroupArgs a) { group_id_kernel<false, 3, false>(a); }
__global__ __launch_bounds__(256) __attribute__((amdgpu_waves_per_eu(3, 3))) void k_group_id_haar_sa(GroupArgs a) { group_id_kernel<true, 2, false>(a); }
__global__ __launch_bounds__(256) void k_group_id_any_sa(GroupArgs a) { group_id_kernel<false, 2, false>(a); }
constexpr unsigned kSaListBlocks = 2048;
__global__ __launch_bounds__(256) void k_group_id_haar_list(GroupArgs a) { group_id_list_kernel<true>(a); }
__global__ __launch_bounds__(256) void k_group_id_any_list(GroupArgs a) { group_id_list_kernel<false>(a); }

constexpr int kT16Groups = 3;
constexpr int kT16Half = 40;
constexpr int kT16Waves = 3;
template <bool HAAR, bool BIOR, bool MULTI, bool SPLIT = false, bool SA = false>
__device__ __forceinline__ void group_t16_kernel(const GroupArgs& a) {
    extern __shared__ float lds[];
    __shared__ float red[MULTI ? kT16Groups : 1][3][4];
    constexpr int K = 16, RS = K + 1, PSZ = kT16Patch, A = 9;
    const int tid = threadIdx.x;
    const unsigned g = a.ref_begin + blockIdx.x * (MULTI ? kT16Groups : 1);
    const int ngr = MULTI ? (int)min((unsigned)kT16Groups, a.ref_begin + a.n_groups - g) : 1;
    const int c = blockIdx.y;
    const int N = a.N;
    const int nSx = MULTI ? 1 : (int)a.self_cnt[g], NP = MULTI ? ngr * A : nSx * A;
    typedef const __attribute__((address_space(4))) unsigned* cuptr;
    const cuptr pos = (cuptr)(a.gpos + (size_t)g * N * A);
    ShRef sh = group_shape(a, g);
    const bool use_sadct = a.tau4 == 6 && sh.use_sadct;
    const TbPtr tb = (TbPtr)a.tb;
    float* work = lds;
#ifdef LFBM5D_PHASE_TIMING
    long long tq[6]; int tqi = 0;
#define T16_MARK() do { if (tid == 0) tq[tqi] = (long long)__builtin_readcyclecounter(); tqi++; } while (0)
    T16_MARK();
#else
#define T16_MARK() do {} while (0)
#endif
    const size_t plane = (size_t)a.Wb * a.Hb;
    auto patch_src = [&](int patch, bool& ok) -> const float* {
        const unsigned p = a.gpos[(size_t)g * N * A + patch];
        ok = p != 0xffffffffu;
        return a.noisy + ((size_t)(patch % A) * a.C + c) * plane + (ok ? p : 0u);
    };
    auto fwd2d = [&](const int base, const int np) {
        if (BIOR) {
            constexpr int TPP = 8, PPI = kThreads / TPP;
            const int slot = tid / TPP, r = tid % TPP;
            for (int p0 = 0; p0 < np; p0 += PPI) {
                const int patch = p0 + slot;
                if (patch < np) {
                    bool ok;
                    const float* src = patch_src(base + patch, ok);
                    v2f v[K], o[K];
    #pragma unroll
                    for (int q = 0; q < 4; q++) {
                        const f4u lo = *reinterpret_cast<const f4u*>(src + (size_t)r * a.Wb + 4 * q);
                        const f4u hi = *reinterpret_cast<const f4u*>(src + (size_t)(r + 8) * a.Wb + 4 * q);
    #pragma unroll
                        for (int e = 0; e < 4; e++) v[4 * q + e] = ok ? v2f{lo.v[e], hi.v[e]} : v2f{0.0f, 0.0f};
                    }
                    bior_taps2<K, true>(v, o, tb);
                    float* Tp = work + patch * PSZ;
    #pragma unroll
                    for (int cc = 0; cc < K; cc++) { Tp[r * RS + cc] = o[cc].x; Tp[(r + 8) * RS + cc] = o[cc].y; }
                    __builtin_amdgcn_wave_barrier();
                    bior16_pass2<K, true, false>(Tp, r, tb);
                }
            }
            __syncthreads();
            bior16_level_all<8, true>(work, np, tid, tb);
            bior16_level_all<4, true>(work, np, tid, tb);
            bior16_level_all<2, true>(work, np, tid, tb);
        } else {
            const int slot = tid / K, r = tid % K;
            for (int p0 = 0; p0 < np; p0 += kThreads / K) {
                const int patch = p0 + slot;
                if (patch < np) {
                    bool ok;
                    const float* src = patch_src(base + patch, ok);
                    float x[K];
// ... 35 lines not shown
                    v2f v[K], o[K];
    #pragma unroll
                    for (int cc = 0; cc < K; cc++) v[cc] = v2f{Tp[r * RS + cc], Tp[(r + 8) * RS + cc]};
                    bior_taps2<K, false>(v, o, tb);
                    float4* dst = reinterpret_cast<float4*>(out + ((size_t)(base + patch) * a.C + c) * K * K);
    #pragma unroll
                    for (int q = 0; q < 4; q++) {
                        filt_put4(&dst[r * 4 + q], make_float4(o[4 * q].x, o[4 * q + 1].x, o[4 * q + 2].x, o[4 * q + 3].x));
                        filt_put4(&dst[(r + 8) * 4 + q], make_float4(o[4 * q].y, o[4 * q + 1].y, o[4 * q + 2].y, o[4 * q + 3].y));
                    }
                }
            }
        } else {
            const int slot = tid / K, r = tid % K;
            for (int p0 = 0; p0 < np; p0 += kThreads / K) {
                const int patch = p0 + slot;
                if (patch < np) {
                    float* Tp = work + patch * PSZ;
                    float x[K];
    #pragma unroll
                    for (int i = 0; i < K; i++) x[i] = Tp[i * RS + r];
                    dct16_inv(x);
    #pragma unroll
                    for (int i = 0; i < K; i++) Tp[i * RS + r] = x[i];
                    __builtin_amdgcn_wave_barrier();
    #pragma unroll
                    for (int cc = 0; cc < K; cc++) x[cc] = Tp[r * RS + cc];
                    dct16_inv(x);
                    float4* dst = reinterpret_cast<float4*>(out + ((size_t)(base + patch) * a.C + c) * K * K);
    #pragma unroll
                    for (int q = 0; q < 4; q++) filt_put4(&dst[r * 4 + q], make_float4(x[4 * q], x[4 * q + 1], x[4 * q + 2], x[4 * q + 3]));
                }
            }
        }
    };
    float wacc[MULTI ? kT16Groups : 1], s1[MULTI ? kT16Groups : 1], s2[MULTI ? kT16Groups : 1];
    const bool split = SPLIT && !MULTI;
    if (!split) { fwd2d(0, NP); T16_MARK(); }
    if (MULTI) {
#pragma unroll
        for (int gi = 0; gi < kT16Groups; gi++) {
            wacc[gi] = 0.0f; s1[gi] = 0.0f; s2[gi] = 0.0f;
            if (gi < ngr) {
                ShRef shg = group_shape(a, g + gi);
                group_id_body<1, HAAR, true, SA ? 2 : 0>(a, g + gi, c, tid, pos + gi * A, shg, a.tau4 == 6 && shg.use_sadct, wacc[gi], s1[gi], s2[gi],
                                                         work + gi * A * PSZ);
            }
        }
    } else if (SPLIT) {
        wacc[0] = 0.0f; s1[0] = 0.0f; s2[0] = 0.0f;
        const int woff = (tid / K) * RS + tid % K;
        auto rounds = [&](auto ns_tag) {
            constexpr int NS = decltype(ns_tag)::value, NH = NS > 1 ? NS / 2 : 1, NPc = NS * A, PR = kT16Half, NR = (NPc + PR - 1) / PR, F0 = NPc - (NR - 1) * PR;
            v2f V[NH][9];
            auto put = [&](const int pch, const float x) { if (pch / 9 < NH) V[pch / 9][pch % 9].x = x; else V[pch / 9 - NH][pch % 9].y = x; };
            auto get = [&](const int pch) { return pch / 9 < NH ? V[pch / 9][pch % 9].x : V[pch / 9 - NH][pch % 9].y; };
            if (NS == 1) {
#pragma unroll
                for (int st = 0; st < 9; st++) V[0][st].y = 0.0f;
            }
#pragma unroll
            for (int r = 0; r < NR; r++) {
                const int b0 = r == 0 ? 0 : F0 + (r - 1) * PR, cnt = r == 0 ? F0 : PR;
                fwd2d(b0, cnt);
#pragma unroll
                for (int q = 0; q < PR; q++) if (q < cnt) put(b0 + q, work[q * PSZ + woff]);
                __syncthreads();
            }
            T16_MARK();
            group_id_compute<NS, HAAR, BIOR ? 2 : 1>(a, c, sh, use_sadct, V, wacc[0], s1[0], s2[0], work + tid * 9);
            __syncthreads();
            T16_MARK();
#pragma unroll
            for (int r = NR - 1; r >= 0; r--) {
                const int b0 = r == 0 ? 0 : F0 + (r - 1) * PR, cnt = r == 0 ? F0 : PR;
#pragma unroll
                for (int q = 0; q < PR; q++) if (q < cnt) work[q * PSZ + woff] = get(b0 + q);
                __syncthreads();
                inv2d(b0, cnt);
                if (r > 0) __syncthreads();
            }
        };
        switch (nSx) {
            case 1:  rounds(std::integral_constant<int, 1>{}); break;
            case 2:  rounds(std::integral_constant<int, 2>{}); break;
            case 4:  rounds(std::integral_constant<int, 4>{}); break;
            default: rounds(std::integral_constant<int, 8>{}); break;
        }
    } else {
        wacc[0] = 0.0f; s1[0] = 0.0f; s2[0] = 0.0f;
        switch (nSx) {
            case 1:  group_id_body<1, HAAR, true>(a, g, c, tid, pos, sh, use_sadct, wacc[0], s1[0], s2[0], work); break;
            case 2:  group_id_body<2, HAAR, true>(a, g, c, tid, pos, sh, use_sadct, wacc[0], s1[0], s2[0], work); break;
            case 4:  group_id_body<4, HAAR, true>(a, g, c, tid, pos, sh, use_sadct, wacc[0], s1[0], s2[0], work); break;
            default: group_id_body<8, HAAR, true>(a, g, c, tid, pos, sh, use_sadct, wacc[0], s1[0], s2[0], work); break;
        }
    }
    if (!split) { __syncthreads(); T16_MARK(); inv2d(0, NP); }
    T16_MARK();
#ifdef LFBM5D_PHASE_TIMING
    T16_MARK();
    if (tid == 0) { for (int i = 0; i < 5; i++) atomicAdd(&a.counters[4 + i], (unsigned long long)(tq[i + 1] - tq[i])); atomicAdd(&a.counters[9], 1ull); }
#endif
#pragma unroll
    for (int gi = 0; gi < (MULTI ? kT16Groups : 1); gi++) {
        for (int o = 32; o > 0; o >>= 1) { wacc[gi] += __shfl_xor(wacc[gi], o); s1[gi] += __shfl_xor(s1[gi], o); s2[gi] += __shfl_xor(s2[gi], o); }
        if ((tid & 63) == 0) { red[gi][0][tid >> 6] = wacc[gi]; red[gi][1][tid >> 6] = s1[gi]; red[gi][2][tid >> 6] = s2[gi]; }
    }
    __syncthreads();
    if (tid < ngr) {
        const int gi = tid;
        float w = 0.0f, m = 0.0f, q = 0.0f;
        for (int i = 0; i < 4; i++) { w += red[gi][0][i]; m += red[gi][1][i]; q += red[gi][2][i]; }
        float wx;
        if (a.useSD) {
            const float Nn = (float)(nSx * A);
            const float res = (q - m * m / Nn) / (Nn - 1.0f);
            wx = res > 0.0f ? 1.0f / sqrtf(res) : 0.0f;
        } else {
            const float sig = a.sigma[c];
            wx = w > 0.0f ? (sig > 0.0f ? 1.0f / (sig * sig * w) : 1.0f / w) : 1.0f;
        }
        a.wgt[(size_t)(g + gi) * a.C + c] = wx;
        if (c == 0) {
            atomicAdd(&a.counters[0], (unsigned long long)nSx);
            if (a.tau4 == 6 && group_shape(a, g + gi).use_sadct) atomicAdd(&a.counters[1], 1ull);
        }
    }
}
__global__ __launch_bounds__(256) __attribute__((amdgpu_waves_per_eu(kT16Waves, kT16Waves))) void k_group_bior16_haar(GroupArgs a) { group_t16_kernel<true, true, false, true>(a); }
__global__ __launch_bounds__(256) void k_group_bior16_any(GroupArgs a) { group_t16_kernel<false, true, false>(a); }
__global__ __launch_bounds__(256) __attribute__((amdgpu_waves_per_eu(kT16Waves, kT16Waves))) void k_group_dct16_haar(GroupArgs a) { group_t16_kernel<true, false, false, true>(a); }
__global__ __launch_bounds__(256) void k_group_dct16_any(GroupArgs a) { group_t16_kernel<false, false, false>(a); }
__global__ __launch_bounds__(256) void k_group_bior16_n1(GroupArgs a) { group_t16_kernel<true, true, true>(a); }
__global__ __launch_bounds__(256) void k_group_dct16_n1(GroupArgs a) { group_t16_kernel<true, false, true>(a); }
__global__ __launch_bounds__(256) void k_group_bior16_n1_sa(GroupArgs a) { group_t16_kernel<true, true, true, false, true>(a); }
__global__ __launch_bounds__(256) void k_group_dct16_n1_sa(GroupArgs a) { group_t16_kernel<true, false, true, false, true>(a); }

}

hipError_t prepare_group_ht() {
    const void* fns[] = {
        reinterpret_cast<const void*>(&k_group_bior16_haar), reinterpret_cast<const void*>(&k_group_bior16_any),
        reinterpret_cast<const void*>(&k_group_dct16_haar), reinterpret_cast<const void*>(&k_group_dct16_any),
        reinterpret_cast<const void*>(&k_group_bior16_n1), reinterpret_cast<const void*>(&k_group_dct16_n1),
        reinterpret_cast<const void*>(&k_group_bior16_n1_sa), reinterpret_cast<const void*>(&k_group_dct16_n1_sa)};
    for (const void* f : fns) {
        const hipError_t e = hipFuncSetAttribute(f, hipFuncAttributeMaxDynamicSharedMemorySize, kDedicatedLdsLimit);
        if (e != hipSuccess) return e;
    }
    return hipSuccess;
}

hipError_t launch_group_ht(hipStream_t s, const GroupArgs& a, bool all_sa, bool* launched) {
    *launched = true;
    if (a.tau2 == 4 && a.N <= 8 && a.k * a.k <= 256 && a.step == 1 && a.A == 9 && (size_t)a.A * a.C * a.Wb * a.Hb * 4 < 0x7fffffffull) {
        const unsigned threads = ((a.k * a.k + 63) / 64) * 64;
        const unsigned gx = ((a.n_groups + 7) / 8) * 8;
        if (all_sa) {
            if (a.tau5 == 9) hipLaunchKernelGGL(k_group_id_haar_sa, dim3(gx, a.C), dim3(threads), 0, s, a);
            else             hipLaunchKernelGGL(k_group_id_any_sa, dim3(gx, a.C), dim3(threads), 0, s, a);
        }
        else {
            if (!a.sa_list) return hipErrorInvalidValue;
            const bool fast = a.tau5 == 9 && (a.tau4 == 5 || a.tau4 == 6) && a.C <= 3 && !(a.opt & kOptHtReferenceOrder);
            if (fast)             hipLaunchKernelGGL(k_group_id_haar_fast, dim3(gx, a.C), dim3(threads), 0, s, a);
            else if (a.tau5 == 9) hipLaunchKernelGGL(k_group_id_haar, dim3(gx, a.C), dim3(threads), 0, s, a);
            else                  hipLaunchKernelGGL(k_group_id_any, dim3(gx, a.C), dim3(threads), 0, s, a);
            if (a.tau4 == 6 || fast) {
                if (a.tau5 == 9) hipLaunchKernelGGL(k_group_id_haar_list, dim3(kSaListBlocks), dim3(threads), 0, s, a);
                else             hipLaunchKernelGGL(k_group_id_any_list, dim3(kSaListBlocks), dim3(threads), 0, s, a);
            }
        }
        return hipGetLastError();
    }
    if ((a.tau2 == 7 || a.tau2 == 5) && a.k == 16 && a.N <= 8 && a.step == 1 && a.A == 9) {
        const size_t lb = (size_t)a.N * 9 * kT16Patch * sizeof(float);
        const dim3 grid(a.n_groups, a.C), block(256);
        if (a.N == 1 && a.tau5 != 5) {
            const dim3 grid8((a.n_groups + kT16Groups - 1) / kT16Groups, a.C);
            const size_t l1 = (size_t)kT16Groups * 9 * kT16Patch * sizeof(float);
            if (all_sa) {
                if (a.tau2 == 7) hipLaunchKernelGGL(k_group_bior16_n1_sa, grid8, block, l1, s, a);
                else             hipLaunchKernelGGL(k_group_dct16_n1_sa, grid8, block, l1, s, a);
            }
            else if (a.tau2 == 7) hipLaunchKernelGGL(k_group_bior16_n1, grid8, block, l1, s, a);
            else                  hipLaunchKernelGGL(k_group_dct16_n1, grid8, block, l1, s, a);
            return hipGetLastError();
        }
        if (a.tau2 == 7) {
            if (a.tau5 == 9) hipLaunchKernelGGL(k_group_bior16_haar, grid, block, std::min(lb, (size_t)kT16Half * kT16Patch * sizeof(float)), s, a);
            else             hipLaunchKernelGGL(k_group_bior16_any, grid, block, lb, s, a);
        } else {
            if (a.tau5 == 9) hipLaunchKernelGGL(k_group_dct16_haar, grid, block, std::min(lb, (size_t)kT16Half * kT16Patch * sizeof(float)), s, a);
            else             hipLaunchKernelGGL(k_group_dct16_any, grid, block, lb, s, a);
        }
        return hipGetLastError();
    }
    *launched = false;
    return hipSuccess;
}
}
```

lfbm5d_amd/csrc/lfbm5d_group_wiener.hip:

```cpp
#include "lfbm5d_group_device.h"

namespace lfbm5d {

namespace {

constexpr int kDct8Threads = 320;

__global__ __launch_bounds__(kDct8Threads) void k_group_dct8(GroupArgs a) {
    extern __shared__ float lds[];
    __shared__ unsigned pos[kMaxN * kA3];
    __shared__ float red[3][kDct8Threads / 64];
    const int tid = threadIdx.x;
    const unsigned g = a.ref_begin + blockIdx.x;
    const int c = blockIdx.y;
    constexpr int A = 9, K2 = 64;
    const int N = a.N;
    const int nSx = (int)a.self_cnt[g];
    const size_t plane = (size_t)a.Wb * a.Hb;
    const int NP = nSx * A;
    const int NPp = (N * A) | 1;
    float* S0 = lds;
    float* S1 = lds + K2 * NPp;
    const TbPtr tb = (TbPtr)a.tb;

// ... 713 lines not shown

    if (tid == 0) {
        float w = 0.0f, m = 0.0f, q = 0.0f;
        for (int i = 0; i < TH / 64; i++) { w += red[0][i]; m += red[1][i]; q += red[2][i]; }
        float wx;
        if (a.useSD) {
            const float Nn = (float)(nSx * A);
            const float res = (q - m * m / Nn) / (Nn - 1.0f);
            wx = res > 0.0f ? 1.0f / sqrtf(res) : 0.0f;
        } else {
            const float sig = a.sigma[c];
            wx = w > 0.0f ? (sig > 0.0f ? 1.0f / (sig * sig * w) : 1.0f / w) : 1.0f;
        }
        a.wgt[(size_t)g * a.C + c] = wx;
        if (c == 0) {
            atomicAdd(&a.counters[0], (unsigned long long)nSx);
            if (use_sadct) atomicAdd(&a.counters[1], 1ull);
        }
    }

    PHASE_MARK();
    const int NPh = (NP + 1) / 2;
    for (int it = tid; it < NPh * 8; it += TH) {
        const int j = (int)__umulhi((unsigned)it, rcpNPh), pa = it - j * NPh;
        const int pb = pa + NPh < NP ? pa + NPh : pa;
        float* ca = stackf + 2 * (j * NPp + pa) + 1;
        float* cb = stackf + 2 * (j * NPp + pb) + 1;
        v2f x[8];
#pragma unroll
        for (int i = 0; i < 8; i++) x[i] = v2f{ca[2 * (i * 8) * NPp], cb[2 * (i * 8) * NPp]};
        dct8_inv_t(x);
#pragma unroll
        for (int i = 0; i < 8; i++) { ca[2 * (i * 8) * NPp] = x[i].x; if (pb != pa) cb[2 * (i * 8) * NPp] = x[i].y; }
    }
    __syncthreads();
    PHASE_MARK();
    for (int it = tid; it < NP * 8; it += TH) {
        const int patch = it >> 3, i = it & 7;
        const float* ra = stackf + 2 * ((i * 8) * NPp + patch) + 1;
        float x[8];
#pragma unroll
        for (int j = 0; j < 8; j++) x[j] = ra[2 * j * NPp];
        dct8_inv_t(x);
        float4* oa = reinterpret_cast<float4*>(a.filt + ((size_t)g * N * A + patch) * a.C * K2 + (size_t)c * K2 + i * 8);
        filt_put4(&oa[0], make_float4(x[0], x[1], x[2], x[3]));
        filt_put4(&oa[1], make_float4(x[4], x[5], x[6], x[7]));
    }
#ifdef LFBM5D_PHASE_TIMING
    PHASE_MARK();
    if (tid == 0) {
        for (int i = 0; i < 5; i++) atomicAdd(&a.counters[4 + i], (unsigned long long)(tc[i + 1] - tc[i]));
        atomicAdd(&a.counters[9], 1ull);
    }
#endif
}

constexpr int kDct8w3Threads = 256;
constexpr int kW3Stride = 146;
constexpr unsigned kW3Lds = 64 * kW3Stride * sizeof(float);
constexpr unsigned kW3Empty = 0xf0000000u;

template <int NS, int TH> struct W3Rows {
    static constexpr int kIt = (((NS * 9 + 1) / 2) * 8 + TH - 1) / TH;
    v4f ra0[kIt], ra1[kIt], rb0[kIt], rb1[kIt];
};
template <int NS, int TH>
__device__ __forceinline__ void w3_load_rows(__amdgpu_buffer_rsrc_t img, unsigned row_bytes, const unsigned* pos, int tid, W3Rows<NS, TH>& r) {
    constexpr int A = 9, NP = NS * A, NPh = (NP + 1) / 2;
#pragma unroll
    for (int q = 0; q < W3Rows<NS, TH>::kIt; q++) {
        const int it = tid + q * TH;
        if (it < NPh * 8) {
            const int i = it / NPh, pp = it - i * NPh;
            const int pA = 2 * pp, pB = pA + 1 < NP ? pA + 1 : pA;
            const int oa = (int)(pos[pA] + (unsigned)i * row_bytes), ob = (int)(pos[pB] + (unsigned)i * row_bytes);
            r.ra0[q] = __builtin_bit_cast(v4f, __builtin_amdgcn_raw_buffer_load_b128(img, oa, 0, 0));
            r.ra1[q] = __builtin_bit_cast(v4f, __builtin_amdgcn_raw_buffer_load_b128(img, oa + 16, 0, 0));
            r.rb0[q] = __builtin_bit_cast(v4f, __builtin_amdgcn_raw_buffer_load_b128(img, ob, 0, 0));
            r.rb1[q] = __builtin_bit_cast(v4f, __builtin_amdgcn_raw_buffer_load_b128(img, ob + 16, 0, 0));
        }
    }
}
template <int NS, int TH, bool SA, bool U = false>
__device__ __forceinline__ void w3_forward(__amdgpu_buffer_rsrc_t img, unsigned row_bytes, float* S, const unsigned* pos,
                                           int tid, ShRef sh, bool do_dct4, bool do_sa4, TbPtr tb, const W3Rows<NS, TH>* pre = nullptr) {
    constexpr int A = 9, NP = NS * A, NPh = (NP + 1) / 2, NPf = kW3Stride;
    constexpr int kIt = (NPh * 8 + TH - 1) / TH;
    {
        W3Rows<NS, TH> own;
        if (!pre) w3_load_rows<NS, TH>(img, row_bytes, pos, tid, own);
        const W3Rows<NS, TH>& R = pre ? *pre : own;
        const v4f (&ra0)[kIt] = R.ra0; const v4f (&ra1)[kIt] = R.ra1; const v4f (&rb0)[kIt] = R.rb0; const v4f (&rb1)[kIt] = R.rb1;
#pragma unroll
        for (int q = 0; q < kIt; q++) {
            const int it = tid + q * TH;
            if (it < NPh * 8) {
                const int i = it / NPh, pp = it - i * NPh;
                v2f x[8];
#pragma unroll
                for (int j = 0; j < 4; j++) {
                    x[j] = v2f{ra0[q][j], rb0[q][j]};
                    x[4 + j] = v2f{ra1[q][j], rb1[q][j]};
                }
                dct8_fwd_t(x);
                float* dst = S + (i * 8) * NPf + 2 * pp;
#pragma unroll
                for (int j = 0; j < 8; j++) *reinterpret_cast<v2f*>(dst + j * NPf) = x[j];
            }
        }
    }
    __syncthreads();
    for (int it = tid; it < NPh * 8; it += TH) {
        const int j = it / NPh, pp = it - j * NPh;
        float* col = S + j * NPf + 2 * pp;
        v2f x[8];
#pragma unroll
        for (int i = 0; i < 8; i++) x[i] = *reinterpret_cast<const v2f*>(col + (i * 8) * NPf);
        dct8_fwd_t(x);
#pragma unroll
        for (int i = 0; i < 8; i++) *reinterpret_cast<v2f*>(col + (i * 8) * NPf) = x[i];
    }
    __syncthreads();
    if (do_dct4 || do_sa4) {
        for (int f = tid; f < NS * 32; f += TH) {
            int n, pq;
            if (NS > 1) { pq = (f & 15) | ((f >> 1) & 16); n = ((f >> 4) & 1) | ((f >> 5) & ~1); }
            else { n = 0; pq = f; }
            float* b0 = S + pq * NPf + n * A;
            float* b1 = b0 + 32 * NPf;
            v2f x[9];
#pragma unroll
            for (int st = 0; st < 9; st++) x[st] = v2f{b0[st], b1[st]};
            if (U) dct9_fwd2_u(x);
            else if (do_dct4) dct9_fwd2_fast(x, tb);
            else {
                float t9[9];
#pragma unroll
                for (int i = 0; i < 9; i++) t9[i] = x[i].x;
                if (SA) sadct9_fwd_sel(t9, sh, tb); else sadct9_fwd(t9, sh, tb);
#pragma unroll
                for (int i = 0; i < 9; i++) { x[i].x = t9[i]; t9[i] = x[i].y; }
                if (SA) sadct9_fwd_sel(t9, sh, tb); else sadct9_fwd(t9, sh, tb);
#pragma unroll
                for (int i = 0; i < 9; i++) x[i].y = t9[i];
            }
#pragma unroll
            for (int st = 0; st < 9; st++) { b0[st] = x[st].x; b1[st] = x[st].y; }
        }
        __syncthreads();
    }
}

template <int NS, int TH, bool SA>
__device__ __forceinline__ void w3_body(const GroupArgs& a, float* S, const unsigned* pos, float (*red)[TH / 64], int tid,
                                        unsigned g, int c) {
    constexpr int A = 9, K2 = 64, NP = NS * A, NPh = (NP + 1) / 2, NPf = kW3Stride;
    static_assert(TH == 256, "the fibre phases deal st 0..3 / 4..7 to 256 threads");
    const int N = a.N;
    const unsigned win_bytes = (unsigned)((size_t)A * a.C * a.Wb * a.Hb * 4);
    const TbPtr tb = (TbPtr)a.tb;
    ShRef sh = group_shape(a, g);
    const bool use_sadct = a.tau4 == 6 && sh.use_sadct;
    const bool do_dct4 = a.tau4 == 5 || (a.tau4 == 6 && !use_sadct);
    const bool do_sa4 = !do_dct4 && a.tau4 == 6;
    const float sig = a.sigma[c];
    const float sig2 = sig * sig;
    const bool useSD = a.useSD != 0;

    w3_forward<NS, TH, SA>(__builtin_amdgcn_make_buffer_rsrc((void*)a.basic, 0, (int)win_bytes, 0x00020000u), a.Wb * 4u, S, pos, tid, sh, do_dct4, do_sa4, tb);
    const int fpq = (tid & 15) | ((tid >> 1) & 48), fst = ((tid >> 4) & 1) | ((tid >> 6) & 2);
    float* const fbase = S + fpq * NPf + fst;
    float* const f8base = S + (tid & 63) * NPf + 8;
    const bool own8 = tid < 64;
    v2f vv[NS];
    float v8[NS];
    {
        v2f e[NS];
#pragma unroll
        for (int n = 0; n < NS; n++) e[n] = v2f{fbase[n * A], fbase[n * A + 4]};
        if (NS > 1) haar_fwd2<NS>(e);
#pragma unroll
        for (int n = 0; n < NS; n++) {
            const v2f value = e[n] * e[n], den = value + sig2;
            vv[n] = v2f{wiener_div(value.x, den.x), wiener_div(value.y, den.y)};
        }
        if (use_sadct) {
#pragma unroll
            for (int n = 0; n < NS; n++) {
                if (!sh.mask_dct[fst]) vv[n].x = e[n].x;
                if (!sh.mask_dct[fst + 4]) vv[n].y = e[n].y;
            }
        }
    }
    if (own8) {
        float e[NS];
#pragma unroll
        for (int n = 0; n < NS; n++) e[n] = f8base[n * A];
        if (NS > 1) haar_fwd<NS>(e);
        const bool in8 = !use_sadct || sh.mask_dct[8];
#pragma unroll
        for (int n = 0; n < NS; n++) {
            const float value = e[n] * e[n];
            v8[n] = in8 ? wiener_div(value, value + sig2) : e[n];
        }
    }
    __syncthreads();
    w3_forward<NS, TH, SA>(__builtin_amdgcn_make_buffer_rsrc((void*)a.noisy, 0, (int)win_bytes, 0x00020000u), a.Wb * 4u, S, pos, tid, sh, do_dct4, do_sa4, tb);
    float wacc = 0.0f, s1 = 0.0f, s2 = 0.0f;
    {
        v2f o[NS];
#pragma unroll
        for (int n = 0; n < NS; n++) o[n] = v2f{fbase[n * A], fbase[n * A + 4]};
        if (NS > 1) haar_fwd2<NS>(o);
        if (!use_sadct) {
            v2f w2 = v2f{0.f, 0.f};
#pragma unroll
            for (int n = 0; n < NS; n++) { o[n] = o[n] * vv[n]; w2 += vv[n]; }
            wacc = w2.x + w2.y;
        } else {
            const bool ina = sh.mask_dct[fst], inb = sh.mask_dct[fst + 4];
#pragma unroll
            for (int n = 0; n < NS; n++) {
                o[n].x = ina ? o[n].x * vv[n].x : vv[n].x;
                o[n].y = inb ? o[n].y * vv[n].y : vv[n].y;
                wacc += (ina ? vv[n].x : 0.f) + (inb ? vv[n].y : 0.f);
            }
        }
        if (NS > 1) haar_inv2<NS>(o);
#pragma unroll
        for (int n = 0; n < NS; n++) { fbase[n * A] = o[n].x; fbase[n * A + 4] = o[n].y; }
        if (useSD) {
#pragma unroll
            for (int n = 0; n < NS; n++) { s1 += o[n].x + o[n].y; s2 += o[n].x * o[n].x + o[n].y * o[n].y; }
        }
    }
    if (own8) {
        float o[NS];
#pragma unroll
        for (int n = 0; n < NS; n++) o[n] = f8base[n * A];
        if (NS > 1) haar_fwd<NS>(o);
        if (!use_sadct || sh.mask_dct[8]) {
#pragma unroll
            for (int n = 0; n < NS; n++) { o[n] = o[n] * v8[n]; wacc += v8[n]; }
        } else {
#pragma unroll
            for (int n = 0; n < NS; n++) o[n] = v8[n];
        }
        if (NS > 1) haar_inv<NS>(o);
#pragma unroll
        for (int n = 0; n < NS; n++) f8base[n * A] = o[n];
        if (useSD) {
#pragma unroll
            for (int n = 0; n < NS; n++) { s1 += o[n]; s2 += o[n] * o[n]; }
        }
    }
    for (int o = 32; o > 0; o >>= 1) { wacc += __shfl_xor(wacc, o); s1 += __shfl_xor(s1, o); s2 += __shfl_xor(s2, o); }
    if ((tid & 63) == 0) { red[0][tid >> 6] = wacc; red[1][tid >> 6] = s1; red[2][tid >> 6] = s2; }
    __syncthreads();
    if (do_dct4 || do_sa4) {
        for (int f = tid; f < NS * 32; f += TH) {
            int n, pq;
            if (NS > 1) { pq = (f & 15) | ((f >> 1) & 16); n = ((f >> 4) & 1) | ((f >> 5) & ~1); }
            else { n = 0; pq = f; }
            float* b0 = S + pq * NPf + n * A;
            float* b1 = b0 + 32 * NPf;
            v2f x[9];
#pragma unroll
            for (int st = 0; st < 9; st++) x[st] = v2f{b0[st], b1[st]};
            if (do_dct4) dct9_inv2_fast(x, tb);
            else {
                float t9[9];
#pragma unroll
                for (int i = 0; i < 9; i++) t9[i] = x[i].x;
                if (SA) sadct9_inv_sel(t9, sh, tb); else sadct9_inv(t9, sh, tb);
#pragma unroll
                for (int i = 0; i < 9; i++) { x[i].x = t9[i]; t9[i] = x[i].y; }
                if (SA) sadct9_inv_sel(t9, sh, tb); else sadct9_inv(t9, sh, tb);
#pragma unroll
                for (int i = 0; i < 9; i++) x[i].y = t9[i];
            }
#pragma unroll
            for (int st = 0; st < 9; st++) { b0[st] = x[st].x; b1[st] = x[st].y; }
        }
    }
    __syncthreads();
    if (tid == 0) {
        float w = 0.0f, m = 0.0f, q = 0.0f;
        for (int i = 0; i < TH / 64; i++) { w += red[0][i]; m += red[1][i]; q += red[2][i]; }
        float wx;
        if (a.useSD) {
            const float Nn = (float)(NS * A);
            const float res = (q - m * m / Nn) / (Nn - 1.0f);
            wx = res > 0.0f ? 1.0f / sqrtf(res) : 0.0f;
        } else {
            wx = w > 0.0f ? (sig > 0.0f ? 1.0f / (sig * sig * w) : 1.0f / w) : 1.0f;
        }
        a.wgt[(size_t)g * a.C + c] = wx;
        if (c == 0) {
            atomicAdd(&a.counters[0], (unsigned long long)NS);
            if (use_sadct) atomicAdd(&a.counters[1], 1ull);
        }
    }
    for (int it = tid; it < NPh * 8; it += TH) {
        const int j = it / NPh, pp = it - j * NPh;
        float* col = S + j * NPf + 2 * pp;
        v2f x[8];
#pragma unroll
        for (int i = 0; i < 8; i++) x[i] = *reinterpret_cast<const v2f*>(col + (i * 8) * NPf);
        dct8_inv_t(x);
#pragma unroll
        for (int i = 0; i < 8; i++) *reinterpret_cast<v2f*>(col + (i * 8) * NPf) = x[i];
    }
    __syncthreads();
    for (int it = tid; it < NPh * 8; it += TH) {
        const int pa = it >> 3, i = it & 7;
        const bool has_b = pa + NPh < NP;
        const float* ra = S + (i * 8) * NPf + pa;
        v2f x[8];
#pragma unroll
        for (int j = 0; j < 8; j++) x[j] = v2f{ra[j * NPf], ra[j * NPf + (NP > NPh ? NPh : 0)]};
        dct8_inv_t(x);
        v4f* oa = reinterpret_cast<v4f*>(a.filt + ((size_t)g * N * A + pa) * a.C * K2 + (size_t)c * K2 + i * 8);
        filt_put4_nt(oa, v4f{x[0].x, x[1].x, x[2].x, x[3].x});
        filt_put4_nt(oa + 1, v4f{x[4].x, x[5].x, x[6].x, x[7].x});
        if (has_b) {
            v4f* ob = oa + (size_t)NPh * a.C * (K2 / 4);
            filt_put4_nt(ob, v4f{x[0].y, x[1].y, x[2].y, x[3].y});
            filt_put4_nt(ob + 1, v4f{x[4].y, x[5].y, x[6].y, x[7].y});
        }
    }
}

template <int NS, int TH>
__device__ __forceinline__ void w3_body_u(const GroupArgs& a, float* S, const unsigned* pos, float (*red)[TH / 64], int tid, unsigned g, int c) {
    constexpr int A = 9, K2 = 64, NP = NS * A, NPh = (NP + 1) / 2, NPf = kW3Stride;
    constexpr int L = NS == 16 ? 4 : NS == 8 ? 3 : NS == 4 ? 2 : NS == 2 ? 1 : 0;
    static_assert(TH == 256, "the fibre phases deal st 0..3 / 4..7 to 256 threads");
    const int N = a.N;
    const unsigned win_bytes = (unsigned)((size_t)A * a.C * a.Wb * a.Hb * 4);
    const TbPtr tb = (TbPtr)a.tb;
    ShRef sh = group_shape(a, g);
    const float sig = a.sigma[c];
    const float sig2 = sig * sig;
    const bool useSD = a.useSD != 0;

    w3_forward<NS, TH, false, true>(__builtin_amdgcn_make_buffer_rsrc((void*)a.basic, 0, (int)win_bytes, 0x00020000u), a.Wb * 4u, S, pos, tid, sh, true, false, tb);
    const int fpq = (tid & 15) | ((tid >> 1) & 48), fst = ((tid >> 4) & 1) | ((tid >> 6) & 2);
    float* const fbase = S + fpq * NPf + fst;
    float* const f8base = S + (tid & 63) * NPf + 8;
    const bool own8 = tid < 64;
    v2f kq[L + 1];
    float k8[L + 1];
    {
        const float fa = tb->ht3_f[fst], fb = tb->ht3_f[fst + 4], f8 = tb->ht3_f[8];
        const v2f q = v2f{sig2 / (fa * fa), sig2 / (fb * fb)};
        const float q8 = sig2 / (f8 * f8);
#pragma unroll
        for (int l = 0; l <= L; l++) { kq[l] = q * (float)(1 << l); k8[l] = q8 * (float)(1 << l); }
    }
    v2f vv[NS];
    float v8[NS];
    {
        v2f e[NS];
#pragma unroll
        for (int n = 0; n < NS; n++) e[n] = v2f{fbase[n * A], fbase[n * A + 4]};
        haar_fwd_u<NS>(e);
#pragma unroll
        for (int n = 0; n < NS; n++) {
            const v2f value = e[n] * e[n], den = value + kq[haar_level<NS>(n)];
            vv[n] = v2f{wiener_div(value.x, den.x), wiener_div(value.y, den.y)};
        }
    }
    if (own8) {
        float e[NS];
#pragma unroll
        for (int n = 0; n < NS; n++) e[n] = f8base[n * A];
        haar_fwd_u<NS>(e);
#pragma unroll
        for (int n = 0; n < NS; n++) {
            const float value = e[n] * e[n];
            v8[n] = wiener_div(value, value + k8[haar_level<NS>(n)]);
        }
    }
    __syncthreads();
    w3_forward<NS, TH, false, true>(__builtin_amdgcn_make_buffer_rsrc((void*)a.noisy, 0, (int)win_bytes, 0x00020000u), a.Wb * 4u, S, pos, tid, sh, true, false, tb);
    float wacc = 0.0f, s1 = 0.0f, s2 = 0.0f;
    const float inv_n = 1.0f / (float)NS;
    {
        v2f o[NS];
#pragma unroll
        for (int n = 0; n < NS; n++) o[n] = v2f{fbase[n * A], fbase[n * A + 4]};
        haar_fwd_u<NS>(o);
        v2f w2 = v2f{0.f, 0.f};
#pragma unroll
        for (int n = 0; n < NS; n++) { o[n] = o[n] * vv[n]; w2 += vv[n]; }
        wacc = w2.x + w2.y;
        haar_inv_u<NS>(o);
#pragma unroll
        for (int n = 0; n < NS; n++) { fbase[n * A] = o[n].x; fbase[n * A + 4] = o[n].y; }
        if (useSD) {
            const v2f f2 = v2f{tb->ht3_f[fst], tb->ht3_f[fst + 4]} * inv_n;
#pragma unroll
            for (int n = 0; n < NS; n++) { const v2f y = o[n] * f2; s1 += y.x + y.y; s2 += y.x * y.x + y.y * y.y; }
        }
    }
    if (own8) {
        float o[NS];
#pragma unroll
        for (int n = 0; n < NS; n++) o[n] = f8base[n * A];
        haar_fwd_u<NS>(o);
#pragma unroll
        for (int n = 0; n < NS; n++) { o[n] = o[n] * v8[n]; wacc += v8[n]; }
        haar_inv_u<NS>(o);
#pragma unroll
        for (int n = 0; n < NS; n++) f8base[n * A] = o[n];
        if (useSD) {
            const float f2 = tb->ht3_f[8] * inv_n;
#pragma unroll
            for (int n = 0; n < NS; n++) { const float y = o[n] * f2; s1 += y; s2 += y * y; }
        }
    }
    for (int o = 32; o > 0; o >>= 1) { wacc += __shfl_xor(wacc, o); s1 += __shfl_xor(s1, o); s2 += __shfl_xor(s2, o); }
    if ((tid & 63) == 0) { red[0][tid >> 6] = wacc; red[1][tid >> 6] = s1; red[2][tid >> 6] = s2; }
    __syncthreads();
    for (int f = tid; f < NS * 32; f += TH) {
        int n, pq;
        if (NS > 1) { pq = (f & 15) | ((f >> 1) & 16); n = ((f >> 4) & 1) | ((f >> 5) & ~1); }
        else { n = 0; pq = f; }
        float* b0 = S + pq * NPf + n * A;
        float* b1 = b0 + 32 * NPf;
        v2f x[9];
#pragma unroll
        for (int st = 0; st < 9; st++) x[st] = v2f{b0[st], b1[st]};
        dct9_inv2_u(x, tb, inv_n);
#pragma unroll
        for (int st = 0; st < 9; st++) { b0[st] = x[st].x; b1[st] = x[st].y; }
    }
    __syncthreads();
    if (tid == 0) {
        float w = 0.0f, m = 0.0f, q = 0.0f;
        for (int i = 0; i < TH / 64; i++) { w += red[0][i]; m += red[1][i]; q += red[2][i]; }
        float wx;
        if (a.useSD) {
            const float Nn = (float)(NS * A);
            const float res = (q - m * m / Nn) / (Nn - 1.0f);
            wx = res > 0.0f ? 1.0f / sqrtf(res) : 0.0f;
        } else {
            wx = w > 0.0f ? (sig > 0.0f ? 1.0f / (sig * sig * w) : 1.0f / w) : 1.0f;
        }
        a.wgt[(size_t)g * a.C + c] = wx;
        if (c == 0) atomicAdd(&a.counters[0], (unsigned long long)NS);
    }
    for (int it = tid; it < NPh * 8; it += TH) {
        const int j = it / NPh, pp = it - j * NPh;
        float* col = S + j * NPf + 2 * pp;
        v2f x[8];
#pragma unroll
        for (int i = 0; i < 8; i++) x[i] = *reinterpret_cast<const v2f*>(col + (i * 8) * NPf);
        dct8_inv_t(x);
#pragma unroll
        for (int i = 0; i < 8; i++) *reinterpret_cast<v2f*>(col + (i * 8) * NPf) = x[i];
    }
    __syncthreads();
    for (int it = tid; it < NPh * 8; it += TH) {
        const int pa = it >> 3, i = it & 7;
        const bool has_b = pa + NPh < NP;
        const float* ra = S + (i * 8) * NPf + pa;
        v2f x[8];
#pragma unroll
        for (int j = 0; j < 8; j++) x[j] = v2f{ra[j * NPf], ra[j * NPf + (NP > NPh ? NPh : 0)]};
        dct8_inv_t(x);
        v4f* oa = reinterpret_cast<v4f*>(a.filt + ((size_t)g * N * A + pa) * a.C * K2 + (size_t)c * K2 + i * 8);
        filt_put4_nt(oa, v4f{x[0].x, x[1].x, x[2].x, x[3].x});
        filt_put4_nt(oa + 1, v4f{x[4].x, x[5].x, x[6].x, x[7].x});
        if (has_b) {
            v4f* ob = oa + (size_t)NPh * a.C * (K2 / 4);
            filt_put4_nt(ob, v4f{x[0].y, x[1].y, x[2].y, x[3].y});
            filt_put4_nt(ob + 1, v4f{x[4].y, x[5].y, x[6].y, x[7].y});
        }
    }
}

constexpr int kW3SaWaves = 4;
template <bool SA>
__global__ __launch_bounds__(kDct8w3Threads) __attribute__((amdgpu_waves_per_eu(SA ? kW3SaWaves : 1))) void k_group_dct8w3(GroupArgs a) {
    extern __shared__ float lds[];
    __shared__ float red[3][kDct8w3Threads / 64];
    __shared__ unsigned pos[kMaxN * kA3];
    constexpr int TH = kDct8w3Threads;
    const int tid = threadIdx.x;
    const unsigned gi = xcd_group_index(a);
    if (gi >= a.n_groups) return;
    const unsigned g = a.ref_begin + gi;
    const int c = blockIdx.y;
    const int nSx = (int)a.self_cnt[g];
    const unsigned plane = a.Wb * a.Hb;
    for (int i = tid; i < nSx * 9; i += TH) {
        const unsigned p = a.gpos[(size_t)g * a.N * 9 + i];
        pos[i] = p != 0xffffffffu ? (((unsigned)(i % 9) * a.C + c) * plane + p) * 4u : kW3Empty;
    }
    __syncthreads();
    switch (nSx) {
        case 1:  w3_body<1, TH, SA>(a, lds, pos, red, tid, g, c); break;
        case 2:  w3_body<2, TH, SA>(a, lds, pos, red, tid, g, c); break;
        case 4:  w3_body<4, TH, SA>(a, lds, pos, red, tid, g, c); break;
        case 8:  w3_body<8, TH, SA>(a, lds, pos, red, tid, g, c); break;
        default: w3_body<16, TH, SA>(a, lds, pos, red, tid, g, c); break;
    }
}

__global__ __launch_bounds__(kDct8w3Threads) void k_group_dct8w3_u(GroupArgs a) {
    extern __shared__ float lds[];
    __shared__ float red[3][kDct8w3Threads / 64];
    __shared__ unsigned pos[kMaxN * kA3];
    constexpr int TH = kDct8w3Threads;
    const int tid = threadIdx.x;
    const unsigned gi = xcd_group_index(a);
    if (gi >= a.n_groups) return;
    const unsigned g = a.ref_begin + gi;
    if (a.tau4 == 6 && group_shape(a, g).use_sadct) return;
    const int c = blockIdx.y;
    const int nSx = (int)a.self_cnt[g];
    const unsigned plane = a.Wb * a.Hb;
    for (int i = tid; i < nSx * 9; i += TH) {
        const unsigned p = a.gpos[(size_t)g * a.N * 9 + i];
        pos[i] = p != 0xffffffffu ? (((unsigned)(i % 9) * a.C + c) * plane + p) * 4u : kW3Empty;
    }
    __syncthreads();
    switch (nSx) {
        case 1:  w3_body_u<1, TH>(a, lds, pos, red, tid, g, c); break;
        case 2:  w3_body_u<2, TH>(a, lds, pos, red, tid, g, c); break;
        case 4:  w3_body_u<4, TH>(a, lds, pos, red, tid, g, c); break;
        case 8:  w3_body_u<8, TH>(a, lds, pos, red, tid, g, c); break;
        default: w3_body_u<16, TH>(a, lds, pos, red, tid, g, c); break;
    }
}
constexpr unsigned kW3ListBlocks = 256;
__global__ __launch_bounds__(kDct8w3Threads) void k_group_dct8w3_list(GroupArgs a) {
    extern __shared__ float lds[];
    __shared__ float red[3][kDct8w3Threads / 64];
    __shared__ unsigned pos[kMaxN * kA3];
    constexpr int TH = kDct8w3Threads;
    const int tid = threadIdx.x;
    const unsigned n_list = a.sa_list[0];
    const int c = blockIdx.y;
    for (unsigned li = blockIdx.x; li < n_list; li += gridDim.x) {
        const unsigned g = a.sa_list[1u + li] & 0x1fffffffu;
        const int nSx = (int)a.self_cnt[g];
        const unsigned plane = a.Wb * a.Hb;
        for (int i = tid; i < nSx * 9; i += TH) {
            const unsigned p = a.gpos[(size_t)g * a.N * 9 + i];
            pos[i] = p != 0xffffffffu ? (((unsigned)(i % 9) * a.C + c) * plane + p) * 4u : kW3Empty;
        }
        __syncthreads();
        switch (nSx) {
            case 1:  w3_body<1, TH, true>(a, lds, pos, red, tid, g, c); break;
            case 2:  w3_body<2, TH, true>(a, lds, pos, red, tid, g, c); break;
            case 4:  w3_body<4, TH, true>(a, lds, pos, red, tid, g, c); break;
            case 8:  w3_body<8, TH, true>(a, lds, pos, red, tid, g, c); break;
            default: w3_body<16, TH, true>(a, lds, pos, red, tid, g, c); break;
        }
        __syncthreads();
    }
}

constexpr int kBm3dWaves = 4;
template <int STEP> struct Bm3dT { typedef float type; };
template <> struct Bm3dT<2> { typedef v2f type; };
__device__ __forceinline__ float bm3d_first(float x) { return x; }
__device__ __forceinline__ float bm3d_first(v2f x) { return x.x; }

template <int STEP, bool BIOR>
__global__ __launch_bounds__(64 * kBm3dWaves) void k_group_bm3d8(GroupArgs a) {
    extern __shared__ float lds[];
    typedef typename Bm3dT<STEP>::type T;
    constexpr int K2 = 64, ST = kMaxN3 + 1;
    const int wave = threadIdx.x >> 6, lane = threadIdx.x & 63;
    const unsigned gi = blockIdx.x * kBm3dWaves + wave;
    if (gi >= a.n_groups) return;
    const unsigned g = a.ref_begin + gi;
    const int c = blockIdx.y;
    const int N = a.N, nSx = (int)a.self_cnt[g];
    const size_t plane = (size_t)a.Wb * a.Hb;
    const TbPtr tb = (TbPtr)a.tb;
    T* S = reinterpret_cast<T*>(lds) + (size_t)wave * K2 * ST;

    if (lane < nSx) {
        const unsigned p = a.gpos[(size_t)g * N + lane];
        const bool ok = p != 0xffffffffu;
        const size_t off = (size_t)c * plane + (ok ? p : 0u);
        T x[8][8];
#pragma unroll
        for (int i = 0; i < 8; i++)
#pragma unroll
            for (int h = 0; h < 2; h++) {
                const f4u q0 = *reinterpret_cast<const f4u*>(a.noisy + off + (size_t)i * a.Wb + 4 * h);
                if (STEP == 2) {
                    const f4u q1 = *reinterpret_cast<const f4u*>(a.basic + off + (size_t)i * a.Wb + 4 * h);
#pragma unroll
                    for (int e = 0; e < 4; e++) reinterpret_cast<v2f&>(x[i][4 * h + e]) = ok ? v2f{q0.v[e], q1.v[e]} : v2f{0.0f, 0.0f};
                } else {
#pragma unroll
                    for (int e = 0; e < 4; e++) reinterpret_cast<float&>(x[i][4 * h + e]) = ok ? q0.v[e] : 0.0f;
                }
            }
        if (BIOR) bior8_fwd_2d(x, tb);
        else {
#pragma unroll
            for (int i = 0; i < 8; i++) dct8_fwd_t(x[i]);
#pragma unroll
            for (int j = 0; j < 8; j++) {
                T col[8];
#pragma unroll
                for (int i = 0; i < 8; i++) col[i] = x[i][j];
                dct8_fwd_t(col);
#pragma unroll
                for (int i = 0; i < 8; i++) x[i][j] = col[i];
            }
        }
#pragma unroll
        for (int i = 0; i < 8; i++)
#pragma unroll
            for (int j = 0; j < 8; j++) S[(i * 8 + j) * ST + lane] = x[i][j];
    }
    __builtin_amdgcn_wave_barrier();

    float wacc = 0.0f, s1 = 0.0f, s2 = 0.0f;
    {
        const float sig = a.sigma[c];
        const float Tthr = a.lambda * sig;
        T* F = S + lane * ST;
        auto fibre = [&](auto ns_tag) {
            constexpr int NS = decltype(ns_tag)::value;
            float o[NS], e[NS];
#pragma unroll
            for (int n = 0; n < NS; n++) {
                if (STEP == 2) { const v2f t = reinterpret_cast<const v2f&>(F[n]); o[n] = t.x; e[n] = t.y; }
                else { o[n] = reinterpret_cast<const float&>(F[n]); e[n] = 0.0f; }
            }
            shrink_fibre<NS, STEP>(o, e, 8u, Tthr, sig * sig, true, wacc, tb);
#pragma unroll
            for (int n = 0; n < NS; n++) {
                const float r = STEP == 1 ? o[n] : e[n];
                s1 += r; s2 += r * r;
                if (STEP == 2) reinterpret_cast<v2f&>(F[n]).y = r; else reinterpret_cast<float&>(F[n]) = r;
            }
        };
        switch (nSx) {
            case 2:  fibre(std::integral_constant<int, 2>{}); break;
            case 4:  fibre(std::integral_constant<int, 4>{}); break;
            case 8:  fibre(std::integral_constant<int, 8>{}); break;
            case 16: fibre(std::integral_constant<int, 16>{}); break;
            default: fibre(std::integral_constant<int, 32>{}); break;
        }
    }
    for (int o = 32; o > 0; o >>= 1) { wacc += __shfl_xor(wacc, o); s1 += __shfl_xor(s1, o); s2 += __shfl_xor(s2, o); }
    if (lane == 0) {
        float wx;
        if (a.useSD) {
            const float Nn = (float)(nSx * K2);
            const float res = (s2 - s1 * s1 / Nn) / (Nn - 1.0f);
            wx = res > 0.0f ? 1.0f / sqrtf(res) : 0.0f;
        } else {
            const float sig = a.sigma[c];
            wx = wacc > 0.0f ? (sig > 0.0f ? 1.0f / (sig * sig * wacc) : 1.0f / wacc) : 1.0f;
        }
        a.wgt[(size_t)g * a.C + c] = wx;
        if (c == 0) atomicAdd(&a.counters[0], (unsigned long long)nSx);
    }
    __builtin_amdgcn_wave_barrier();

    if (lane < nSx) {
        float x[8][8];
#pragma unroll
        for (int i = 0; i < 8; i++)
#pragma unroll
            for (int j = 0; j < 8; j++) {
                const T t = S[(i * 8 + j) * ST + lane];
                if (STEP == 2) x[i][j] = reinterpret_cast<const v2f&>(t).y; else x[i][j] = bm3d_first(t);
            }
        if (BIOR) bior8_inv_2d(x, tb);
        else {
#pragma unroll
            for (int j = 0; j < 8; j++) {
                float col[8];
#pragma unroll
                for (int i = 0; i < 8; i++) col[i] = x[i][j];
                dct8_inv_t(col);
#pragma unroll
                for (int i = 0; i < 8; i++) x[i][j] = col[i];
            }
#pragma unroll
            for (int i = 0; i < 8; i++) dct8_inv_t(x[i]);
        }
        float4* dst = reinterpret_cast<float4*>(a.filt + (((size_t)g * N + lane) * a.C + c) * K2);
#pragma unroll
        for (int i = 0; i < 8; i++) {
            filt_put4(&dst[2 * i], make_float4(x[i][0], x[i][1], x[i][2], x[i][3]));
            filt_put4(&dst[2 * i + 1], make_float4(x[i][4], x[i][5], x[i][6], x[i][7]));
        }
    }
}

}

hipError_t prepare_group_wiener() {
    const void* fns[] = {
        reinterpret_cast<const void*>(&k_group_dct8),
        reinterpret_cast<const void*>(&k_group_dct8w2<true>), reinterpret_cast<const void*>(&k_group_dct8w2<false>),
        reinterpret_cast<const void*>(&k_group_dct8w<true>), reinterpret_cast<const void*>(&k_group_dct8w<false>),
        reinterpret_cast<const void*>(&k_group_bm3d8<2, true>), reinterpret_cast<const void*>(&k_group_bm3d8<2, false>)};
    for (const void* f : fns) {
        const hipError_t e = hipFuncSetAttribute(f, hipFuncAttributeMaxDynamicSharedMemorySize, kDedicatedLdsLimit);
        if (e != hipSuccess) return e;
    }
    return hipSuccess;
}

hipError_t launch_group_wiener(hipStream_t s, const GroupArgs& a, bool all_sa, bool* launched) {
    *launched = true;
    if (a.tau2 == 7 && a.k == 8 && a.A == 9 && a.step == 2 && a.N <= (unsigned)kMaxN) {
        const size_t l8 = (size_t)2 * 64 * ((a.N * 9) | 1) * sizeof(float);
        if (a.tau5 == 9) hipLaunchKernelGGL((k_group_dct8w<true>), dim3(a.n_groups, a.C), dim3(kDct8wThreads), l8, s, a);
        else             hipLaunchKernelGGL((k_group_dct8w<false>), dim3(a.n_groups, a.C), dim3(kDct8wThreads), l8, s, a);
        return hipGetLastError();
    }
    if (a.tau2 == 5 && a.k == 8 && a.A == 9 && a.N <= (unsigned)kMaxN) {
        const size_t l8 = (size_t)(a.step == 2 ? 2 : 1) * 64 * ((a.N * 9) | 1) * sizeof(float);
        if (a.step == 2) {
            const unsigned gx = ((a.n_groups + 7) / 8) * 8;
            if (a.tau5 == 9 && (size_t)9 * a.C * a.Wb * a.Hb * 4 < 0x70000000ull && !(a.opt & kOptDct8wV2)) {
                if (all_sa) hipLaunchKernelGGL(k_group_dct8w3<true>, dim3(gx, a.C), dim3(kDct8w3Threads), kW3Lds, s, a);
                else if (a.tau4 == 5 || a.tau4 == 6) {
                    if (!a.sa_list) return hipErrorInvalidValue;
                    hipLaunchKernelGGL(k_group_dct8w3_u, dim3(gx, a.C), dim3(kDct8w3Threads), kW3Lds, s, a);
                    if (a.tau4 == 6) hipLaunchKernelGGL(k_group_dct8w3_list, dim3(kW3ListBlocks, a.C), dim3(kDct8w3Threads), kW3Lds, s, a);
                }
                else        hipLaunchKernelGGL(k_group_dct8w3<false>, dim3(gx, a.C), dim3(kDct8w3Threads), kW3Lds, s, a);
            }
            else if (a.tau5 == 9) hipLaunchKernelGGL((k_group_dct8w2<true>), dim3(gx, a.C), dim3(kDct8w2Threads), l8, s, a);
            else                  hipLaunchKernelGGL((k_group_dct8w2<false>), dim3(gx, a.C), dim3(kDct8w2Threads), l8, s, a);
            return hipGetLastError();
        }
        hipLaunchKernelGGL(k_group_dct8, dim3(a.n_groups, a.C), dim3(kDct8Threads), l8, s, a);
        return hipGetLastError();
    }
    if (a.bm3d && a.A == 1 && a.k == 8 && a.tau5 == 8 && (a.tau2 == 5 || a.tau2 == 7)) {
        const dim3 grid((a.n_groups + kBm3dWaves - 1) / kBm3dWaves, a.C), block(64 * kBm3dWaves);
        const size_t lb = (size_t)kBm3dWaves * 64 * (kMaxN3 + 1) * (a.step == 2 ? sizeof(v2f) : sizeof(float));
        if (a.step == 2) { if (a.tau2 == 7) hipLaunchKernelGGL((k_group_bm3d8<2, true>), grid, block, lb, s, a); else hipLaunchKernelGGL((k_group_bm3d8<2, false>), grid, block, lb, s, a); }
        else             { if (a.tau2 == 7) hipLaunchKernelGGL((k_group_bm3d8<1, true>), grid, block, lb, s, a); else hipLaunchKernelGGL((k_group_bm3d8<1, false>), grid, block, lb, s, a); }
        return hipGetLastError();
    }
    *launched = false;
    return hipSuccess;
}
}
```

lfbm5d_amd/csrc/lfbm5d_kernels.h:

```cpp
#ifndef LFBM5D_KERNELS_H
#define LFBM5D_KERNELS_H

#include <hip/hip_runtime.h>
#include <vector>

#include "lfbm5d_options.h"

constexpr int kFiltStoreAux = 2;
constexpr int kFiltLoadAux = 0;

#if defined(__HIPCC__)
typedef float filt_v4f __attribute__((ext_vector_type(4)));
typedef float filt_v2f __attribute__((ext_vector_type(2)));
__device__ __forceinline__ void filt_put(float* p, const float v) { *p = v; }
__device__ __forceinline__ void filt_put2(filt_v2f* p, const filt_v2f v) { *p = v; }
__device__ __forceinline__ void filt_put4(filt_v4f* p, const filt_v4f v) { *p = v; }
__device__ __forceinline__ void filt_put4(float4* p, const float4 v) { *p = v; }
__device__ __forceinline__ void filt_put4_nt(filt_v4f* p, const filt_v4f v) { __builtin_nontemporal_store(v, p); }
#endif

namespace lfbm5d {

constexpr int kMaxK = 32;
constexpr int kMaxA = 49;
constexpr int kA3 = 9;
constexpr int kMaxAw = 7;
constexpr int kBigAw = 17;
constexpr int kBigA = kBigAw * kBigAw;
constexpr int kMaskWords = (kBigA + 63) / 64;
struct SaiMask {
    unsigned long long w[kMaskWords];
    __host__ __device__ bool test(unsigned i) const { return (w[i >> 6] >> (i & 63)) & 1ull; }
    __host__ __device__ void set(unsigned i) { w[i >> 6] |= 1ull << (i & 63); }
    __host__ __device__ unsigned count() const { unsigned n = 0; for (int i = 0; i < kMaskWords; i++) n += (unsigned)__builtin_popcountll(w[i]); return n; }
    __host__ __device__ bool holds_all(unsigned n) const { for (unsigned i = 0; i < n; i++) if (!test(i)) return false; return true; }
};
inline SaiMask sai_mask_none() { SaiMask m; for (int i = 0; i < kMaskWords; i++) m.w[i] = 0; return m; }
constexpr int kMaxN = 16;
constexpr int kMaxN3 = 32;

struct GroupTables {
    float kaiser[kMaxK * kMaxK];
    float cn2[kMaxK * kMaxK];
    float cni2[kMaxK * kMaxK];
    float cos2[kMaxK * kMaxK];
    float cn4[kBigA];
    float cni4[kBigA];
    float cos3[9];
    float cosw[kBigA];
    float cos1[kBigAw + 1][kBigA];
    float cn1[kBigAw + 1][kBigAw];
    float cni1[kBigAw + 1][kBigAw];
    float c1inv[kBigAw + 1];
    float cos5[5][256];
    float cos5x[1024];
    float cn5_0[6], cn5[6];
    float c5inv[6];
    float lpd[10], hpd[10], lpr[10], hpr[10];
    float coef2inv;
    float coef4inv;
    float ht3_f[9];
    float ht3_gf[9];
};

constexpr float kHtGuardAbs[9][4] = {
    {1.5e-7f, 8.1e-6f, 1.7e-5f, 3.5e-5f}, {5.6e-7f, 1.4e-6f, 1.9e-6f, 3.5e-6f}, {7.8e-7f, 2.3e-6f, 2.8e-6f, 3.7e-6f},
    {2.1e-6f, 3.6e-6f, 5.4e-6f, 6.4e-6f}, {4.1e-7f, 1.1e-6f, 1.6e-6f, 2.4e-6f}, {5.3e-7f, 1.8e-6f, 2.3e-6f, 4.0e-6f},
    {3.8e-6f, 6.6e-6f, 9.4e-6f, 1.4e-5f}, {7.6e-7f, 1.7e-6f, 2.5e-6f, 4.2e-6f}, {1.0e-6f, 3.0e-6f, 3.9e-6f, 6.5e-6f}};

constexpr unsigned kShapeInfoBytes = (5 * kMaxA + 2 * kMaxAw + 1) * 4;
constexpr unsigned kShapeInfoBigBytes = (5 * kBigA + 2 * kBigAw + 1) * 4;

struct GroupArgs {
    const float* noisy;
    const float* basic;
    float* num;
    float* den;
    const unsigned* refs;
    const unsigned* self_idx;
    const unsigned* self_cnt;
    const unsigned* best;
    const unsigned char* shape;
    const GroupTables* tb;
    float* filt;
    float* wgt;
    unsigned* aggpos;
    unsigned* gpos;
    unsigned* sa_list;
    unsigned* gofs;
    unsigned* gok;
    void* gshape;
    unsigned n_refs_total;
    unsigned long long* counters;
    unsigned ref_begin, n_groups;
    unsigned Wb, Hb, C, A, k, N, pst;
    SaiMask mask_bits, proc_bits;
    unsigned tau2, tau4, tau5, useSD;
    unsigned fill_quirk;
    int step;
    float lambda;
    float sigma[3];
    float ht3_T[3][9][4];
    float ht3_K[3][9];
    float* scratch;
    unsigned long long scratch_floats;
    unsigned opt;
    unsigned long long filt_sai_stride;
    unsigned bm3d;
};

constexpr unsigned kSaiMajorMinA = 121;
__device__ __forceinline__ size_t filt_patch(const GroupArgs& a, unsigned g, unsigned n, unsigned st, unsigned k2) {
    return a.filt_sai_stride ? (size_t)st * a.filt_sai_stride + ((size_t)g * a.N + n) * a.C * k2
                             : (((size_t)g * a.N + n) * a.A + st) * a.C * k2;
}


struct SaiList { unsigned st[kBigA]; unsigned n; };

struct AggArgs {
    float* num;
    float* den;
    const float* filt;
    unsigned long long filt_sai_stride;
    unsigned long long filt_bytes;
    const float* wgt;
    const unsigned* aggpos;
    unsigned n_refs_total;
    const unsigned* refs;
    const unsigned* self_idx;
    const unsigned* self_cnt;
    const unsigned* best;
    const unsigned char* shape;
    const GroupTables* tb;
    unsigned ref_begin, n_groups;
    unsigned n_ref_rows, n_ref_cols;
    unsigned Wb, Hb, C, A, k, N, pst, p, nHW, nSim, nDisp;
    SaiMask mask_bits, proc_bits; unsigned tau4;
    unsigned irregular;
    unsigned opt;
    unsigned wchan0;
    unsigned direct;
    unsigned long long lf_stride;
    SaiList sai;
};

__host__ __device__ inline size_t stereo_table_stride(unsigned W, unsigned H, unsigned k, unsigned nDisp) {
    const unsigned ncols = W - 2 * nDisp - (k - 1), nrows = H - 2 * nDisp - (k - 1);
    return (size_t)((ncols + 63) / 64) * 64 * (nrows + 63);
}

__host__ __device__ inline unsigned stereo_table_srq(unsigned H, unsigned k, unsigned nDisp) {
    const unsigned nrows = H - 2 * nDisp - (k - 1);
    return ((nrows - 1 + 63 + 15) / 16) * 4 + 1;
}
__host__ __device__ inline size_t stereo_table_stride2(unsigned W, unsigned H, unsigned k, unsigned nDisp) {
    const unsigned ncols = W - 2 * nDisp - (k - 1);
    return (size_t)((ncols - 1 + 63) / 64) * stereo_table_srq(H, k, nDisp) * 256 + stereo_table_srq(H, k, nDisp) * 4;
}

__host__ __device__ inline unsigned stereo_part_chunks(unsigned H, unsigned k, unsigned nDisp) {
    const unsigned nrows = H - 2 * nDisp - (k - 1);
    return ((nrows - 1 + 63 + 15) / 16) * 2;
}
__host__ __device__ inline size_t stereo_part_stride(unsigned W, unsigned H, unsigned k, unsigned nDisp) {
    const unsigned ncols = W - 2 * nDisp - (k - 1);
    return (size_t)((ncols - 1 + 63) / 64) * stereo_part_chunks(H, k, nDisp) * 512;
}
__host__ __device__ inline size_t stereo_edge_stride(unsigned W, unsigned H, unsigned k, unsigned nDisp) {
    const unsigned ncols = W - 2 * nDisp - (k - 1), nrows = H - 2 * nDisp - (k - 1);
    return ((size_t)nrows + (ncols - 1 + 63) / 64 + 3) & ~(size_t)3;
}

struct Scan2Wg {
    short tab[16];
    short slot;
    short r2lo, c2lo;
    short rh, ch;
    short wgj;
    short pad[2];
    short ord[16];
};

struct ScanArgs {
    const float* est;
    unsigned W, H, k;
    unsigned nSim, nDisp, nHW;
    unsigned pst;
    unsigned n_self;
    unsigned n_stereo;
    unsigned n_ref_rows, n_ref_cols, p;
    const int* rslot;
    const int* refmap;
    float* scores;
    unsigned scores_bytes;
    unsigned long long* dbg;
    unsigned opt;
    unsigned lds_cap;
    float* tables;
    unsigned st_of_slot[kBigA];
    unsigned est_planes;
    const Scan2Wg* wgs;
    unsigned n_wgs;
    float* lcol;
    unsigned lcol_stride;
    unsigned nwg_slot;
};

hipError_t launch_color(hipStream_t s, float* img, unsigned cs, unsigned n_px, int forward);
hipError_t launch_color_lf(hipStream_t s, float* lf, size_t sai_stride, unsigned n_sai, const unsigned* d_mask, unsigned cs,
                           unsigned n_px, int forward);
hipError_t launch_color_roundtrip_lf(hipStream_t s, const float* in, float* out, size_t sai_stride, unsigned n_sai, const unsigned* d_mask,
                                     unsigned cs, unsigned n_px);
hipError_t launch_estimate_lf(hipStream_t s, const float* num, const float* den, const float* sub, float* est, size_t seg,
                              unsigned n_sai, const unsigned* d_mask);
hipError_t launch_symetrize(hipStream_t s, const float* src, float* dst, unsigned W, unsigned H,
                            unsigned C, unsigned N);
hipError_t launch_unsymetrize(hipStream_t s, float* dst, const float* src, unsigned W, unsigned H,
                              unsigned C, unsigned N);
hipError_t launch_crop(hipStream_t s, float* dst, const float* src, unsigned W, unsigned H, unsigned C, unsigned N, unsigned off);
hipError_t launch_estimate(hipStream_t s, const float* num, const float* den, const float* sub,
                           float* est, size_t n);
hipError_t launch_finalize_multi(hipStream_t s, const float* num, const float* den, const float* sub, float* basic, size_t sai_stride,
                                 const SaiList& L, unsigned cs, unsigned n_px, int colour);
hipError_t launch_output_multi(hipStream_t s, const float* num, const float* den, const float* sub, float* out, float* basic,
                               const float* noisy_src, float* noisy_dst, size_t sai_stride, const SaiList& L, unsigned cs, unsigned n_px,
                               int colour);
hipError_t launch_ipc_set(hipStream_t s, unsigned* p, unsigned v);
hipError_t launch_ipc_wait(hipStream_t s, const unsigned* p, unsigned want, unsigned* err, double timeout_s);
hipError_t launch_symetrize_multi(hipStream_t s, const float* src, size_t src_stride, float* dst, size_t dst_stride,
                                  const SaiList& L, unsigned W, unsigned H, unsigned C, unsigned N);
hipError_t launch_unsymetrize_multi(hipStream_t s, float* dst, size_t dst_stride, const float* src, size_t src_stride,
                                    const SaiList& L, unsigned W, unsigned H, unsigned C, unsigned N);
constexpr unsigned kWinCounters = 32;
hipError_t launch_window_begin(hipStream_t s, const float* noisy, const float* basic, const float* num, const float* den, size_t lf_stride,
                               float* w_noisy, float* w_basic, float* w_num, float* w_den, float* est, size_t w_stride, const SaiList& L,
                               unsigned W, unsigned H, unsigned C, unsigned N, unsigned* zero);
hipError_t launch_window_end(hipStream_t s, float* num, float* den, size_t lf_stride, const float* w_num, const float* w_den, size_t w_stride,
                             const SaiList& L, unsigned W, unsigned H, unsigned C, unsigned N, unsigned k, unsigned* count);
hipError_t launch_estimate_multi(hipStream_t s, const float* num, const float* den, const float* sub, float* est,
                                 size_t plane, unsigned C, unsigned A, const SaiMask& mask_bits);
hipError_t launch_copy_rect(hipStream_t s, float* dst, size_t dst_stride, unsigned dW, unsigned dH, unsigned dx0, unsigned dy0,
                            const float* src, size_t src_stride, unsigned sW, unsigned sH, unsigned sx0, unsigned sy0,
                            unsigned w, unsigned h, unsigned C, unsigned n_slots, const SaiMask& mask_bits);
hipError_t launch_copy_rows(hipStream_t s, const float* src, unsigned src_H, unsigned src_row0, float* dst, unsigned dst_H, unsigned dst_row0,
                            unsigned n_rows, unsigned W, unsigned planes);
hipError_t launch_fill_f32(hipStream_t s, float* p, float v, size_t n);
hipError_t launch_fill_i32(hipStream_t s, int* p, int v, size_t n);
hipError_t launch_add(hipStream_t s, float* dst, const float* src, size_t n);
hipError_t launch_count_zeros(hipStream_t s, const float* den, size_t seg, unsigned n_seg,
                              unsigned* counts);
hipError_t launch_count_denoised(hipStream_t s, const float* den, size_t sai_stride, unsigned n_slots, const SaiMask& mask_bits,
                                 unsigned W, unsigned H, unsigned C, unsigned N, unsigned k, unsigned* count);
hipError_t launch_refmap(hipStream_t s, const unsigned* refs, unsigned n_refs, int* refmap);
hipError_t launch_subset_list(hipStream_t s, const float* den0, unsigned Wb, unsigned k, unsigned nHW, unsigned p, unsigned n_rows,
                              unsigned n_cols, unsigned last_r, unsigned last_c, unsigned char* flags, unsigned* refs, unsigned* count);
hipError_t launch_bm_scan(hipStream_t s, const ScanArgs& a);
int bm_scan_version(const ScanArgs& a);
bool scan2_plan(const ScanArgs& a, std::vector<Scan2Wg>& wgs, size_t* lds_bytes, unsigned* nwg_slot = nullptr);
size_t scan_tables_floats(const ScanArgs& a, int version, unsigned n_slots, unsigned nwg_slot);
unsigned scan2_lcol_stride(const ScanArgs& a);
hipError_t prepare_scan2_kernels();
hipError_t launch_bm_scan2(hipStream_t s, const ScanArgs& a, size_t lds_bytes, bool combined);
hipError_t launch_stereo_argmin3(hipStream_t s, const float* tables, const unsigned* st_of_slot, unsigned n_slots, unsigned nwg_slot,
                                 unsigned W, unsigned H, unsigned k, unsigned nDisp, float thr,
                                 unsigned* best, unsigned char* shape);
hipError_t launch_stereo_argmin2(hipStream_t s, const float* tables, const unsigned* st_of_slot, unsigned n_slots,
                                 unsigned W, unsigned H, unsigned k, unsigned nDisp, float thr,
                                 unsigned* best, unsigned char* shape);
hipError_t launch_self_select(hipStream_t s, const float* scores, const unsigned* refs, unsigned n_refs,
                              unsigned W, unsigned nSim, unsigned N, float thr, unsigned* self_idx,
                              unsigned* self_cnt,
                              unsigned grid_cols = 0, unsigned nHW = 0, unsigned p = 1, unsigned last_r = 0, unsigned last_c = 0);
hipError_t launch_self_trivial(hipStream_t s, const unsigned* refs, unsigned n_refs, unsigned* self_idx,
                               unsigned* self_cnt);
hipError_t launch_stereo_argmin(hipStream_t s, const float* tables, const unsigned* st_of_slot, unsigned n_slots,
                                unsigned W, unsigned H, unsigned k, unsigned nDisp, float thr,
                                unsigned* best, unsigned char* shape);
hipError_t prepare_group_kernels();
hipError_t launch_group(hipStream_t s, const GroupArgs& a);
size_t group_lds_bytes(const GroupArgs& a);
size_t group_scratch_bytes(const GroupArgs& a);
hipError_t launch_aggregate(hipStream_t s, const AggArgs& a);

}
#endif
```

lfbm5d_amd/csrc/lfbm5d_options.h:

```cpp
#ifndef LFBM5D_OPTIONS_H
#define LFBM5D_OPTIONS_H

#include <cstddef>
#include <cstdlib>
#include <cstring>
#include <string>

namespace lfbm5d {

enum : unsigned {
    kOptScanV1 = 1u << 0,
    kOptScanAny = 1u << 1,
    kOptScanFullTables = 1u << 2,
    kOptDct8wV2 = 1u << 3,
    kOptGroupGeneric = 1u << 4,
    kOptNoSaKernels = 1u << 5,
    kOptNoSlabKernel = 1u << 6,
    kOptWideNoSplit = 1u << 7,
    kOptAgg64Bit = 1u << 8,
    kOptAggScalarScan = 1u << 9,
    kOptSubsetListHost = 1u << 10,
    kOptSubsetScanV1 = 1u << 11,
    kOptFiltGroupMajor = 1u << 12,
    kOptHtReferenceOrder = 1u << 13,
};

struct Options {
    int lanes = 2;
    int emulate_world = 0;
    int max_windows = 0;
    int fused = 1;
    int step_sharding = 0;
    int data_driven_schedule = 0;
    int host_blocking = 0;
    int band_mb = 0;
    int bm3d_lanes = 3;
    int scan_lds_cap = 0;
    int force_redo = 0;
    int spatial_bands = 1;
    int band_halo = 0;
    int window_sums_padded = 0;
    unsigned kernels = 0;
};

struct OptionKey { const char* key; const char* env; int Options::* field; unsigned bit; };

inline const OptionKey* option_keys(size_t* n) {
    static const OptionKey keys[] = {
        {"lanes", "LFBM5D_LANES", &Options::lanes, 0}, {"emulate_world", "LFBM5D_EMULATE_WORLD", &Options::emulate_world, 0},
        {"max_windows", "LFBM5D_MAX_WINDOWS", &Options::max_windows, 0}, {"fused", "LFBM5D_FUSED", &Options::fused, 0},
        {"step_sharding", "LFBM5D_STEP_SHARDING", &Options::step_sharding, 0},
        {"data_driven_schedule", "LFBM5D_DATA_DRIVEN_SCHEDULE", &Options::data_driven_schedule, 0},
        {"host_blocking", "LFBM5D_HOST_BLOCKING", &Options::host_blocking, 0}, {"band_mb", "LFBM5D_BAND_MB", &Options::band_mb, 0},
        {"bm3d_lanes", "LFBM5D_BM3D_LANES", &Options::bm3d_lanes, 0}, {"scan_lds_cap", "LFBM5D_SCAN_LDS_CAP", &Options::scan_lds_cap, 0},
        {"force_redo", "LFBM5D_FORCE_REDO", &Options::force_redo, 0}, {"spatial_bands", "LFBM5D_SPATIAL_BANDS", &Options::spatial_bands, 0},
        {"band_halo", "LFBM5D_BAND_HALO", &Options::band_halo, 0},
        {"window_sums_padded", "LFBM5D_WINDOW_SUMS_PADDED", &Options::window_sums_padded, 0},
        {"scan_v1", "LFBM5D_SCAN_V1", nullptr, kOptScanV1}, {"scan_any", "LFBM5D_SCAN_ANY", nullptr, kOptScanAny},
        {"scan_full_tables", "LFBM5D_SCAN_FULL_TABLES", nullptr, kOptScanFullTables}, {"dct8w_v2", "LFBM5D_DCT8W_V2", nullptr, kOptDct8wV2},
        {"group_generic", "LFBM5D_GROUP_GENERIC", nullptr, kOptGroupGeneric}, {"no_sa_kernels", "LFBM5D_NO_SA_KERNELS", nullptr, kOptNoSaKernels},
        {"no_slab_kernel", "LFBM5D_NO_SLAB_KERNEL", nullptr, kOptNoSlabKernel}, {"wide_nosplit", "LFBM5D_WIDE_NOSPLIT", nullptr, kOptWideNoSplit},
        {"agg_64bit", "LFBM5D_AGG_64BIT", nullptr, kOptAgg64Bit}, {"agg_scalar_scan", "LFBM5D_AGG_SCALAR_SCAN", nullptr, kOptAggScalarScan},
        {"subset_list_host", "LFBM5D_SUBSET_LIST_HOST", nullptr, kOptSubsetListHost}, {"subset_scan_v1", "LFBM5D_SUBSET_SCAN_V1", nullptr, kOptSubsetScanV1},
        {"filt_group_major", "LFBM5D_FILT_GROUP_MAJOR", nullptr, kOptFiltGroupMajor},
        {"ht_reference_order", "LFBM5D_HT_REF_ORDER", nullptr, kOptHtReferenceOrder},
    };
    *n = sizeof(keys) / sizeof(keys[0]);
    return keys;
}

inline bool option_set(Options& o, const char* key, const char* value) {
    size_t n; const OptionKey* keys = option_keys(&n);
    static const Options defaults;
    for (size_t i = 0; i < n; i++) {
        if (std::strcmp(key, keys[i].key) != 0 && std::strcmp(key, keys[i].env) != 0) continue;
        const bool unset = value == nullptr || value[0] == 0;
        if (keys[i].field) {
            int v = defaults.*(keys[i].field);
            if (!unset) {
                if (keys[i].field == &Options::step_sharding) v = std::strcmp(value, "rows") == 0 ? 1 : std::strcmp(value, "blocks") == 0 ? 2 : std::atoi(value);
                else if (keys[i].field == &Options::data_driven_schedule || keys[i].field == &Options::host_blocking || keys[i].field == &Options::force_redo)
                    v = std::strcmp(value, "0") != 0;
                else v = std::atoi(value);
            }
            o.*(keys[i].field) = v;
        } else {
            if (!unset && std::strcmp(value, "0") != 0) o.kernels |= keys[i].bit; else o.kernels &= ~keys[i].bit;
        }
        return true;
    }
    return false;
}
inline bool option_get(const Options& o, const char* key, std::string& out) {
    size_t n; const OptionKey* keys = option_keys(&n);
    for (size_t i = 0; i < n; i++) {
        if (std::strcmp(key, keys[i].key) != 0 && std::strcmp(key, keys[i].env) != 0) continue;
        if (keys[i].field == &Options::step_sharding) out = o.step_sharding == 1 ? "rows" : o.step_sharding == 2 ? "blocks" : "0";
        else if (keys[i].field) out = std::to_string(o.*(keys[i].field));
        else out = (o.kernels & keys[i].bit) ? "1" : "0";
        return true;
    }
    return false;
}
inline void options_from_env(Options& o) {
    size_t n; const OptionKey* keys = option_keys(&n);
    for (size_t i = 0; i < n; i++)
        if (const char* e = std::getenv(keys[i].env)) {
            const bool flag = !keys[i].field || keys[i].field == &Options::data_driven_schedule || keys[i].field == &Options::host_blocking ||
                              keys[i].field == &Options::force_redo;
            if (e[0]) (void)option_set(o, keys[i].key, e); else if (flag) (void)option_set(o, keys[i].key, "1");
        }
}

}
#endif
```

lfbm5d_amd/csrc/lfbm5d_pass.hip:

```cpp
#include "lfbm5d_ctx.h"

namespace lfbm5d_host {

lfbm5d_ctx* new_ctx(int device, std::string& err) {
    hipError_t e;
    lfbm5d_ctx* c = new lfbm5d_ctx();
    c->device = device;
    std::memset(&c->stats, 0, sizeof(c->stats));
    if ((e = hipStreamCreateWithFlags(&c->stream, hipStreamNonBlocking)) != hipSuccess) { err = hipGetErrorString(e); delete c; return nullptr; }
    if ((e = prepare_group_kernels()) != hipSuccess || (e = prepare_scan2_kernels()) != hipSuccess) { err = std::string("kernel LDS limits: ") + hipGetErrorString(e); (void)hipStreamDestroy(c->stream); delete c; return nullptr; }
    if ((e = hipHostMalloc((void**)&c->h_small, 64 * sizeof(unsigned))) != hipSuccess) { err = hipGetErrorString(e); (void)hipStreamDestroy(c->stream); delete c; return nullptr; }
    return c;
}


hipEvent_t get_event(lfbm5d_ctx* c) {
    if (c->ev_used == c->ev_pool.size()) {
        hipEvent_t e; (void)hipEventCreate(&e); c->ev_pool.push_back(e);
    }
    return c->ev_pool[c->ev_used++];
}

void drain_events(lfbm5d_ctx* c) {
    for (const PassEvents& pe : c->pending) {
// ... 266 lines not shown
            const size_t rows_fit = std::max<size_t>(1, cap / (per_group * sizeof(float) * row_groups));
            band_groups = (unsigned)std::min<size_t>(R, rows_fit * row_groups);
        }
    }
    HIPCK(c, c->filt.reserve((size_t)band_groups * per_group * sizeof(float)));
    HIPCK(c, c->wgt.reserve((size_t)R * C * sizeof(float)));
    HIPCK(c, c->aggpos.reserve((size_t)A * R * Nst * sizeof(unsigned)));
    HIPCK(c, c->gpos.reserve((size_t)A * R * Nst * sizeof(unsigned)));
    HIPCK(c, c->gofs.reserve((size_t)A * R * Nst * sizeof(unsigned)));
    HIPCK(c, c->gok.reserve((size_t)R * Nst * sizeof(unsigned)));
    HIPCK(c, c->sa_list.reserve((size_t)(4 * (size_t)R + 1) * sizeof(unsigned)));
    HIPCK(c, c->gshape.reserve((size_t)R * (A > (unsigned)kMaxA ? kShapeInfoBigBytes : kShapeInfoBytes)));
    HIPCK(c, gc.tb.reserve(sizeof(GroupTables)));
    if (!c->counters.p) {
        HIPCK(c, c->counters.reserve(32 * sizeof(unsigned long long)));
        HIPCK(c, hipMemsetAsync(c->counters.p, 0, 32 * sizeof(unsigned long long), s));
    }
    unsigned long long* const d_counters = c->counters.as<unsigned long long>() + 16 * c->gslot;
    if (gc.tb_key[0] != k || gc.tb_key[1] != aw || gc.tb_key[2] != ah) {
        GroupTables tb;
        build_tables(tb, k, aw, ah);
        HIPCK(c, hipMemcpyAsync(gc.tb.p, &tb, sizeof(tb), hipMemcpyHostToDevice, s));
        HIPCK(c, hipStreamSynchronize(s));
        gc.tb_key[0] = k; gc.tb_key[1] = aw; gc.tb_key[2] = ah;
    }

    PassEvents pe; pe.comm = false;
    for (int i = 0; i < 5; i++) pe.e[i] = get_event(c);

    const float* sub = step == 1 ? d_noisy : d_basic;
    if (!est_ready) HIPCK(c, launch_estimate_multi(s, d_num, d_den, sub, est, plane, C, A, mask_bits));
    if (c->pass_world > 1 && c->pass_rank > 0) {
        HIPCK(c, hipMemsetAsync(d_num, 0, A * C * plane * sizeof(float), s));
        HIPCK(c, hipMemsetAsync(d_den, 0, A * C * plane * sizeof(float), s));
    }

    HIPCK(c, hipEventRecord(pe.e[0], s));
    ScanArgs sa;
    std::memset(&sa, 0, sizeof(sa));
    sa.dbg = d_counters + 4;
    sa.est = est; sa.W = Wb; sa.H = Hb; sa.k = k; sa.pst = pst;
    sa.nSim = P->nSim; sa.nDisp = P->nDisp; sa.nHW = nHW;
    sa.n_ref_rows = gc.n_ref_rows; sa.n_ref_cols = gc.n_ref_cols; sa.p = P->p;
    sa.scores = c->scores.as<float>(); sa.tables = c->tables.as<float>(); sa.rslot = gc.rslot.as<int>(); sa.refmap = (centre || full_scan) ? nullptr : c->refmap.as<int>(); sa.scores_bytes = (unsigned)((size_t)R_sc * NsS * NsS * sizeof(float));
    sa.n_self = N > 1 ? (P->nSim + 1) * NsS : 0;
    sa.n_stereo = n_slots * NsD * NsD;
    for (unsigned i = 0; i < n_slots; i++) sa.st_of_slot[i] = slots[i];
    sa.est_planes = A;
    if (N > 1) HIPCK(c, launch_fill_f32(s, c->scores.as<float>(), 2 * thr, (size_t)R_sc * NsS * NsS));
    sa.opt = c->opt->kernels; sa.lds_cap = (unsigned)std::max(0, c->opt->scan_lds_cap);
    const bool opt_v1 = (sa.opt & (kOptScanV1 | kOptScanAny)) != 0, opt_ft = (sa.opt & kOptScanFullTables) != 0;
    const unsigned skey[8] = {sa.n_self, sa.n_stereo, sa.nSim, sa.nDisp, sa.k, Hb, Wb,
                              1u | ((centre || full_scan) ? 0u : 2u) | (opt_v1 ? 4u : 0u) | (opt_ft ? 8u : 0u) | ((sa.opt & kOptScanAny) ? 16u : 0u)};
    const bool scan_changed = std::memcmp(skey, gc.scan_key, sizeof(skey)) != 0;
    if (scan_changed) gc.scan_version = bm_scan_version(sa);
    const int scan_version = gc.scan_version;
    c->last_scan_version = scan_version;
    if (scan_version == 1) {
        HIPCK(c, c->tables.reserve(std::max<size_t>(1, scan_tables_floats(sa, 1, n_slots, 0)) * sizeof(float)));
        sa.tables = c->tables.as<float>();
    }
    if (scan_version >= 2) {
        if (scan_changed) {
            if (!scan2_plan(sa, gc.scan_plan, &gc.scan_lds, &gc.scan_nwg_slot)) return fail(c, "scan plan");
            HIPCK(c, gc.scan_wgs.reserve(gc.scan_plan.size() * sizeof(Scan2Wg)));
            HIPCK(c, hipMemcpyAsync(gc.scan_wgs.p, gc.scan_plan.data(), gc.scan_plan.size() * sizeof(Scan2Wg), hipMemcpyHostToDevice, s));
            HIPCK(c, hipStreamSynchronize(s));
        }
        sa.wgs = gc.scan_wgs.as<Scan2Wg>(); sa.n_wgs = (unsigned)gc.scan_plan.size();
        sa.lcol_stride = scan2_lcol_stride(sa);
        HIPCK(c, c->scan_lcol.reserve((size_t)(sa.n_self + sa.n_stereo) * sa.lcol_stride * sizeof(float)));
        sa.lcol = c->scan_lcol.as<float>();
        sa.nwg_slot = gc.scan_nwg_slot;
        HIPCK(c, c->tables.reserve(std::max<size_t>(1, scan_tables_floats(sa, scan_version, n_slots, sa.nwg_slot)) * sizeof(float)));
        sa.tables = c->tables.as<float>();
        HIPCK(c, launch_bm_scan2(s, sa, gc.scan_lds, scan_version == 3));
    } else
        HIPCK(c, launch_bm_scan(s, sa));
    std::memcpy(gc.scan_key, skey, sizeof(skey));
    if (N > 1)
        HIPCK(c, launch_self_select(s, c->scores.as<float>(), gc.refs.as<unsigned>(), R, Wb, P->nSim, N, thr,
                                    c->self_idx.as<unsigned>(), c->self_cnt.as<unsigned>(),
                                    full_scan ? gc.n_ref_cols : 0u, nHW, P->p, Hb - k - nHW, Wb - k - nHW));
    else
        HIPCK(c, launch_self_trivial(s, gc.refs.as<unsigned>(), R, c->self_idx.as<unsigned>(), c->self_cnt.as<unsigned>()));
    if (n_slots && scan_version == 3)
        HIPCK(c, launch_stereo_argmin3(s, c->tables.as<float>(), slots, n_slots, sa.nwg_slot, Wb, Hb, k, P->nDisp, thr,
                                       c->best.as<unsigned>(), c->shape.as<unsigned char>()));
    else if (n_slots && scan_version == 2)
        HIPCK(c, launch_stereo_argmin2(s, c->tables.as<float>(), slots, n_slots, Wb, Hb, k, P->nDisp, thr,
                                       c->best.as<unsigned>(), c->shape.as<unsigned char>()));
    else if (n_slots)
        HIPCK(c, launch_stereo_argmin(s, c->tables.as<float>(), slots, n_slots, Wb, Hb, k, P->nDisp, thr,
                                      c->best.as<unsigned>(), c->shape.as<unsigned char>()));
    HIPCK(c, hipEventRecord(pe.e[1], s));

    unsigned ref_begin, n_groups;
    if (centre) {
        unsigned rb = 0, re = gc.n_ref_rows;
        lfbm5d_shard_rows(gc.n_ref_rows, c->pass_rank, c->pass_world, &rb, &re);
        ref_begin = rb * gc.n_ref_cols; n_groups = (re - rb) * gc.n_ref_cols;
    } else {
        unsigned rb = 0, re = (unsigned)row_start.size() - 1;
        lfbm5d_shard_rows((unsigned)row_start.size() - 1, c->pass_rank, c->pass_world, &rb, &re);
        ref_begin = row_start[rb]; n_groups = row_start[re] - row_start[rb];
    }

    GroupArgs ga;
    std::memset(&ga, 0, sizeof(ga));
    ga.noisy = d_noisy; ga.basic = d_basic; ga.num = d_num; ga.den = d_den;
    ga.refs = gc.refs.as<unsigned>(); ga.self_idx = c->self_idx.as<unsigned>(); ga.self_cnt = c->self_cnt.as<unsigned>();
    ga.best = c->best.as<unsigned>(); ga.shape = c->shape.as<unsigned char>(); ga.tb = gc.tb.as<GroupTables>();
    ga.wgt = c->wgt.as<float>(); ga.aggpos = c->aggpos.as<unsigned>(); ga.gpos = c->gpos.as<unsigned>(); ga.gofs = c->gofs.as<unsigned>(); ga.gok = c->gok.as<unsigned>(); ga.sa_list = c->sa_list.as<unsigned>(); ga.gshape = c->gshape.p; ga.n_refs_total = R; ga.counters = d_counters;
    ga.ref_begin = ref_begin; ga.n_groups = n_groups;
    ga.Wb = Wb; ga.Hb = Hb; ga.C = C; ga.A = A; ga.k = k; ga.N = Nst; ga.pst = pst;
    ga.mask_bits = mask_bits; ga.proc_bits = proc_bits;
    ga.tau2 = P->tau_2D; ga.tau4 = P->tau_4D; ga.tau5 = P->tau_5D; ga.useSD = P->useSD;
    ga.step = step; ga.lambda = lambda; ga.fill_quirk = centre ? 1u : 0u;
    for (int i = 0; i < 3; i++) ga.sigma[i] = sig[i];
    if (A == 9 && step == 1) {
        GroupTables ht;
        build_tables(ht, k, 3, 3);
        for (int ch = 0; ch < 3; ch++) {
            const float T = lambda * sig[ch] * 1.41421356237309505f;
            for (int st = 0; st < 9; st++)
                for (int l = 0; l < 4; l++) ga.ht3_T[ch][st][l] = (float)((double)T / ((double)ht.ht3_f[st] * std::pow(2.0, -0.5 * l)));
            for (int st = 0; st < 9; st++) {
                double K = 0.0;
                for (int l = 0; l < 4; l++) K = std::max(K, (double)kHtGuardAbs[st][l] / (double)ga.ht3_T[ch][st][l]);
                ga.ht3_K[ch][st] = std::nextafter((float)std::min(K, 1e30), INFINITY);
            }
        }
    }
    ga.bm3d = bm3d ? 1u : 0u;
    ga.opt = c->opt->kernels;
    if (const size_t sb = group_scratch_bytes(ga)) {
        HIPCK(c, c->gscratch.reserve(sb));
        ga.scratch = c->gscratch.as<float>(); ga.scratch_floats = sb / sizeof(float);
    }
    AggArgs aa;
    std::memset(&aa, 0, sizeof(aa));
    aa.num = d_num; aa.den = d_den; aa.wgt = ga.wgt; aa.aggpos = ga.aggpos; aa.n_refs_total = R; aa.refs = ga.refs;
    aa.self_idx = ga.self_idx; aa.self_cnt = ga.self_cnt; aa.best = ga.best; aa.shape = ga.shape; aa.tb = ga.tb;
    aa.ref_begin = ref_begin; aa.n_groups = n_groups; aa.n_ref_rows = gc.n_ref_rows; aa.n_ref_cols = gc.n_ref_cols;
    aa.Wb = Wb; aa.Hb = Hb; aa.C = C; aa.A = A; aa.k = k; aa.N = Nst; aa.pst = pst; aa.p = P->p;
    aa.nHW = nHW; aa.nSim = P->nSim; aa.nDisp = P->nDisp;
    aa.mask_bits = mask_bits; aa.proc_bits = proc_bits; aa.tau4 = P->tau_4D; aa.irregular = centre ? 0u : 1u;
    aa.wchan0 = (bm3d && P->useSD) ? 1u : 0u;
    aa.opt = c->opt->kernels;
    if (direct) {
        aa.num = c->direct.num; aa.den = c->direct.den; aa.direct = 1u; aa.lf_stride = c->direct.lf_stride; aa.sai = c->direct.sai;
    }
    const bool sai_major = A >= kSaiMajorMinA && !(c->opt->kernels & kOptFiltGroupMajor);
    const size_t per_group_bias = sai_major ? per_group / A : per_group;
    if (n_groups <= band_groups) {
        ga.filt_sai_stride = aa.filt_sai_stride = sai_major ? (unsigned long long)n_groups * (per_group / A) : 0ull;
        ga.filt = c->filt.as<float>() - (size_t)ref_begin * per_group_bias;
        aa.filt = c->filt.as<float>(); aa.filt_bytes = (unsigned long long)n_groups * per_group * sizeof(float);
        if (n_groups) HIPCK(c, launch_group(s, ga));
        HIPCK(c, hipEventRecord(pe.e[2], s));
        if (n_groups) HIPCK(c, launch_aggregate(s, aa));
        HIPCK(c, hipEventRecord(pe.e[3], s));
    } else {
        bool first = true;
        for (unsigned b0 = ref_begin; b0 < ref_begin + n_groups; b0 += band_groups) {
            const unsigned nb = std::min(band_groups, ref_begin + n_groups - b0);
            ga.filt_sai_stride = aa.filt_sai_stride = sai_major ? (unsigned long long)nb * (per_group / A) : 0ull;
            ga.ref_begin = b0; ga.n_groups = nb; ga.filt = c->filt.as<float>() - (size_t)b0 * per_group_bias;
            aa.ref_begin = b0; aa.n_groups = nb; aa.filt = c->filt.as<float>(); aa.filt_bytes = (unsigned long long)nb * per_group * sizeof(float);
            HIPCK(c, launch_group(s, ga));
            if (first) HIPCK(c, hipEventRecord(pe.e[2], s));
            first = false;
            HIPCK(c, launch_aggregate(s, aa));
            c->stats.launches_group += 1; c->stats.launches_aggregate += 1;
        }
        c->stats.launches_group -= 1; c->stats.launches_aggregate -= 1;
        HIPCK(c, hipEventRecord(pe.e[3], s));
    }

    if (c->comm && c->pass_reduce) {
        const size_t cnt = (size_t)A * C * plane;
        if (ncclAllReduce(d_num, d_num, cnt, ncclFloat, ncclSum, c->comm, s) != ncclSuccess) return fail(c, "ncclAllReduce(num) failed");
        if (ncclAllReduce(d_den, d_den, cnt, ncclFloat, ncclSum, c->comm, s) != ncclSuccess) return fail(c, "ncclAllReduce(den) failed");
        HIPCK(c, hipEventRecord(pe.e[4], s));
        pe.comm = true;
    }
    c->pending.push_back(pe);

    c->stats.passes += 1;
    c->stats.groups += n_groups;
    c->stats.launches_group += n_groups ? 1 : 0;
    c->stats.launches_aggregate += n_groups ? 1 : 0;
    c->last_n_refs = R; c->last_N = Nst; c->last_A = A; c->last_plane = plane; c->last_gslot = c->gslot;
    return 0;
}

int fold_counters(lfbm5d_ctx* c, const lfbm5d_params* P, unsigned A, unsigned C, int step, int slot) {
    unsigned long long h[4] = {0, 0, 0, 0};
    if (!c->counters.p) return 0;
    unsigned long long* const d_counters = c->counters.as<unsigned long long>() + 16 * slot;
    HIPCK(c, hipMemcpyAsync(h, d_counters, sizeof(h), hipMemcpyDeviceToHost, c->stream));
    HIPCK(c, hipStreamSynchronize(c->stream));
    HIPCK(c, hipMemsetAsync(d_counters, 0, sizeof(h), c->stream));
    c->stats.stack_patches += h[0];
    c->stats.sadct_groups += h[1];
#ifdef LFBM5D_PHASE_TIMING
    {
        unsigned long long ph[12];
        (void)hipMemcpy(ph, d_counters + 4, sizeof(ph), hipMemcpyDeviceToHost);
        (void)hipMemset(d_counters + 4, 0, sizeof(ph));
        std::fprintf(stderr, "[phases step %d]", step);
        for (int i = 0; i < 12; i++) std::fprintf(stderr, " %.3g", (double)ph[i]);
        std::fprintf(stderr, "\n");
    }
#endif
    c->stats.algorithmic_bytes += (double)h[0] * A * P->k * P->k * C * (4.0 * (step == 2 ? 2 : 1) + 16.0);
    return 0;
}

}
```

Measured before the change: 253.0 SAI-megapixels/s.

## Rotate filtered-patch rows by image row phase to spread aggregate filt loads

The group kernels (HT k=16 register-resident path and Wiener dct8w3 k=8 path) now store each filtered patch's rows rotated by an offset derived from the patch's image row modulo a small mask, and the aggregate kernel undoes that rotation when it gathers. The goal appears to be spreading the aggregate's scattered filt reads across memory channels or cache lines and reducing conflicts between adjacent tiles. The aggregate tiles for k=8 also change from 8x8 to 16x4, with new waves-per-EU occupancy hints for the rotated variants. This adds index arithmetic and per-entry rotation bits in the gok word and in shared memory, and the rotated path only supports k=8 and k=16. An env option turns the layout off.

```diff
diff --git a/lfbm5d_amd/core.py b/lfbm5d_amd/core.py
--- a/lfbm5d_amd/core.py
+++ b/lfbm5d_amd/core.py
@@ -312,7 +312,7 @@
               "LFBM5D_FORCE_REDO", "LFBM5D_SPATIAL_BANDS", "LFBM5D_BAND_HALO", "LFBM5D_SCAN_V1", "LFBM5D_SCAN_ANY", "LFBM5D_SCAN_FULL_TABLES", "LFBM5D_DCT8W_V2",
               "LFBM5D_GROUP_GENERIC", "LFBM5D_NO_SA_KERNELS", "LFBM5D_NO_SLAB_KERNEL", "LFBM5D_WIDE_NOSPLIT", "LFBM5D_AGG_64BIT",
               "LFBM5D_AGG_SCALAR_SCAN", "LFBM5D_SUBSET_LIST_HOST", "LFBM5D_SUBSET_SCAN_V1", "LFBM5D_FILT_GROUP_MAJOR",
-              "LFBM5D_HT_REF_ORDER", "LFBM5D_WINDOW_SUMS_PADDED")
+              "LFBM5D_HT_REF_ORDER", "LFBM5D_WINDOW_SUMS_PADDED", "LFBM5D_FILT_ROWS_PLAIN")
 OPTION_ENV_EMPTY_OFF = ("LFBM5D_WINDOW_SUMS_PADDED",)
 
 
diff --git a/lfbm5d_amd/csrc/lfbm5d_aggregate.hip b/lfbm5d_amd/csrc/lfbm5d_aggregate.hip
--- a/lfbm5d_amd/csrc/lfbm5d_aggregate.hip
+++ b/lfbm5d_amd/csrc/lfbm5d_aggregate.hip
@@ -10,8 +10,8 @@
 
 
 constexpr int kAggFlush = 64;
-template <bool WINDOWED, int TW, int TH, int kAggPF, int kAggU, bool BIG, bool VEC4>
-__global__ __launch_bounds__(64) __attribute__((amdgpu_waves_per_eu((VEC4 && TW == 8 && !BIG) ? 8 : 1))) void k_aggregate(AggArgs a) {
+template <bool WINDOWED, int TW, int TH, int kAggPF, int kAggU, bool BIG, bool VEC4, bool ROT>
+__global__ __launch_bounds__(64) __attribute__((amdgpu_waves_per_eu((VEC4 && (TW == 8 || (WINDOWED && ROT)) && !BIG) ? 8 : (ROT && !WINDOWED && !BIG) ? 5 : 1))) void k_aggregate(AggArgs a) {
     constexpr int kAggCap = kAggFlush + kAggPF * 64 + kAggU;
     __shared__ uint4 hit_a[kAggCap];
     __shared__ float hit_w2[kAggCap];
@@ -70,6 +70,7 @@
     const unsigned* apos = a.aggpos + (size_t)st * a.n_refs_total * N;
     const unsigned cstride = C > 1 ? (unsigned)k2 * 4u : 0u;
     const __amdgpu_buffer_rsrc_t rs_filt = __builtin_amdgcn_make_buffer_rsrc((void*)filt, 0, BIG ? 0 : (int)(unsigned)filt_bytes, 0x00020000u);
+    const unsigned rot_mask = ROT ? a.filt_rot_mask : 0u, rot_org = a.filt_rot_org, k2m1 = (unsigned)k2 - 1u;
     unsigned nh = 0;
 
     auto consume = [&]() {
@@ -86,13 +87,14 @@
                 const bool on = (unsigned)dy < (unsigned)k && (unsigned)dx < (unsigned)k;
                 const unsigned o = __umul24((unsigned)min(max(dy, 0), k - 1), (unsigned)k) + (unsigned)min(max(dx, 0), k - 1);
                 const float kz = WINDOWED ? kai[o] : 1.0f;
+                const unsigned fo = ROT ? (((o - (ha.y & 63u)) & k2m1) | (ha.y & ~k2m1)) : ha.y + o;
                 if (BIG) {
-                    const char* fp = reinterpret_cast<const char*>(filt) + ((size_t)ha.y + o) * 4;
+                    const char* fp = reinterpret_cast<const char*>(filt) + (size_t)fo * 4;
                     val[u][0] = *reinterpret_cast<const float*>(fp);
                     val[u][1] = *reinterpret_cast<const float*>(fp + cstride);
                     val[u][2] = *reinterpret_cast<const float*>(fp + 2 * cstride);
                 } else {
-                    const int vo = (int)((ha.y + o) * 4u);
+                    const int vo = (int)(fo * 4u);
                     val[u][0] = __builtin_bit_cast(float, __builtin_amdgcn_raw_buffer_load_b32(rs_filt, vo, 0, kFiltLoadAux));
                     val[u][1] = __builtin_bit_cast(float, __builtin_amdgcn_raw_buffer_load_b32(rs_filt, vo, (int)cstride, kFiltLoadAux));
                     val[u][2] = __builtin_bit_cast(float, __builtin_amdgcn_raw_buffer_load_b32(rs_filt, vo, (int)(2 * cstride), kFiltLoadAux));
@@ -159,7 +161,7 @@
 #pragma unroll
                 for (int j = 0; j < 4; j++) {
                     if (m4 & (1u << j)) {
-                        hit_a[slot] = make_uint4(pj[j], off, __float_as_uint(w[0]), __float_as_uint(w[1]));
+                        hit_a[slot] = make_uint4(pj[j], off + filt_rot_d0(rot_mask, rot_org, pj[j]) * (unsigned)k, __float_as_uint(w[0]), __float_as_uint(w[1]));
                         hit_w2[slot] = w[2];
                         slot++;
                     }
@@ -221,7 +223,7 @@
                 const unsigned gl = g[u] - a.ref_begin;
                 if (small24) off = __umul24(__umul24((gl << logN) + nn[u], Af) + stf, (unsigned)(C * k2));
                 else { asm volatile("" ::: "memory"); off = (((gl << logN) + nn[u]) * Af + stf) * C * k2; }
-                hit_a[slot] = make_uint4(p[u], off, __float_as_uint(w[u][0]), __float_as_uint(w[u][1]));
+                hit_a[slot] = make_uint4(p[u], off + filt_rot_d0(rot_mask, rot_org, p[u]) * (unsigned)k, __float_as_uint(w[u][0]), __float_as_uint(w[u][1]));
                 hit_w2[slot] = w[u][2];
             }
             nh += __popcll(bal);
@@ -237,23 +239,27 @@
 
 hipError_t launch_aggregate(hipStream_t s, const AggArgs& a) {
     const bool wide = a.k >= 12;
-    constexpr int kAgg16TW = 16, kAgg16TH = 4, kAgg8TW = 8, kAgg8TH = 8;
-    const unsigned tw = wide ? (a.k == 12 ? 16 : kAgg16TW) : (a.k == 8 ? kAgg8TW : 8), th = wide ? (a.k == 12 ? 4 : kAgg16TH) : (a.k == 8 ? kAgg8TH : 8);
+    constexpr int kAgg16TW = 16, kAgg16TH = 4, kAgg8TW = 16, kAgg8TH = 4;
+    const bool rot = a.filt_rot_mask != 0;
+    if (rot && a.k != 8 && a.k != 16) return hipErrorInvalidValue;
+    const unsigned tw = rot ? (a.k == 16 ? kAgg16TW : kAgg8TW) : wide ? 16 : 8, th = rot ? (a.k == 16 ? kAgg16TH : kAgg8TH) : wide ? 4 : 8;
     const unsigned org = a.direct ? a.nHW : 0u;
     const unsigned tiles = ((a.Wb - 2 * org + tw - 1) / tw) * ((a.Hb - 2 * org + th - 1) / th) * a.A;
     const dim3 grid(((tiles + 7) / 8) * 8), block(64);
     const bool big = (a.filt_sai_stride ? a.filt_sai_stride * sizeof(float) : a.filt_bytes) > 0xfffff000ull || (a.opt & kOptAgg64Bit);
     const bool vec4 = a.N % 4 == 0 && !wide && !(a.opt & kOptAggScalarScan);
-#define LFBM5D_AGG(W_, TW_, TH_, PF_, U_) \
-    do { if (big && vec4) hipLaunchKernelGGL((k_aggregate<W_, TW_, TH_, PF_, U_, true, true>), grid, block, 0, s, a); \
-         else if (big)    hipLaunchKernelGGL((k_aggregate<W_, TW_, TH_, PF_, U_, true, false>), grid, block, 0, s, a); \
-         else if (vec4)   hipLaunchKernelGGL((k_aggregate<W_, TW_, TH_, PF_, U_, false, true>), grid, block, 0, s, a); \
-         else             hipLaunchKernelGGL((k_aggregate<W_, TW_, TH_, PF_, U_, false, false>), grid, block, 0, s, a); } while (0)
+#define LFBM5D_AGG(W_, TW_, TH_, PF_, U_, R_) \
+    do { if (big && vec4) hipLaunchKernelGGL((k_aggregate<W_, TW_, TH_, PF_, U_, true, true, R_>), grid, block, 0, s, a); \
+         else if (big)    hipLaunchKernelGGL((k_aggregate<W_, TW_, TH_, PF_, U_, true, false, R_>), grid, block, 0, s, a); \
+         else if (vec4)   hipLaunchKernelGGL((k_aggregate<W_, TW_, TH_, PF_, U_, false, true, R_>), grid, block, 0, s, a); \
+         else             hipLaunchKernelGGL((k_aggregate<W_, TW_, TH_, PF_, U_, false, false, R_>), grid, block, 0, s, a); } while (0)
     constexpr int kAgg16PF = 3, kAgg16U = 12, kAgg8PF = 3, kAgg8U = 6;
-    if (a.k == 12)      LFBM5D_AGG(true, 16, 4, 3, 12);
-    else if (a.k == 8)  LFBM5D_AGG(true, kAgg8TW, kAgg8TH, kAgg8PF, kAgg8U);
-    else if (wide)      LFBM5D_AGG(false, kAgg16TW, kAgg16TH, kAgg16PF, kAgg16U);
-    else                LFBM5D_AGG(false, 8, 8, 2, 6);
+    if (rot && a.k == 8) LFBM5D_AGG(true, kAgg8TW, kAgg8TH, kAgg8PF, kAgg8U, true);
+    else if (rot)        LFBM5D_AGG(false, kAgg16TW, kAgg16TH, kAgg16PF, kAgg16U, true);
+    else if (a.k == 12)  LFBM5D_AGG(true, 16, 4, 3, 12, false);
+    else if (a.k == 8)   LFBM5D_AGG(true, 8, 8, 3, 6, false);
+    else if (wide)       LFBM5D_AGG(false, 16, 4, 3, 12, false);
+    else                 LFBM5D_AGG(false, 8, 8, 2, 6, false);
 #undef LFBM5D_AGG
     return hipGetLastError();
 }
diff --git a/lfbm5d_amd/csrc/lfbm5d_group_device.h b/lfbm5d_amd/csrc/lfbm5d_group_device.h
--- a/lfbm5d_amd/csrc/lfbm5d_group_device.h
+++ b/lfbm5d_amd/csrc/lfbm5d_group_device.h
@@ -11,6 +11,8 @@
 
 hipError_t launch_group_ht(hipStream_t s, const GroupArgs& a, bool all_sa, bool* launched);
 hipError_t launch_group_wiener(hipStream_t s, const GroupArgs& a, bool all_sa, bool* launched);
+bool group_ht_rotates(const GroupArgs& a);
+bool group_wiener_rotates(const GroupArgs& a);
 hipError_t launch_group_wide(hipStream_t s, const GroupArgs& a, bool* launched);
 hipError_t prepare_group_wide();
 hipError_t launch_group_slab(hipStream_t s, const GroupArgs& a, bool* launched);
diff --git a/lfbm5d_amd/csrc/lfbm5d_group_generic.hip b/lfbm5d_amd/csrc/lfbm5d_group_generic.hip
--- a/lfbm5d_amd/csrc/lfbm5d_group_generic.hip
+++ b/lfbm5d_amd/csrc/lfbm5d_group_generic.hip
@@ -28,6 +28,7 @@
             const bool there = !zero_patch && p != 0xffffffffu;
             a.gofs[(size_t)g * NA + i] = there ? (unsigned)(((size_t)st * a.C * plane + p) * 4) : 0u;
             bits |= there ? 1u << st : 0u;
+            if (p != 0xffffffffu) bits |= filt_rot_d0(a.filt_rot_mask & 1u, a.filt_rot_org, (p / a.Wb) << 16) << (9 + st);
         }
         const bool in_shape = st == (int)a.pst || (masked && a.shape[(size_t)st * plane + k_r]);
         a.aggpos[((size_t)st * a.n_refs_total + g) * N + n] = ((a.tau4 != 6 || in_shape) && p != 0xffffffffu) ? ((p / a.Wb) << 16) | (p % a.Wb) : 0xffffffffu;
@@ -328,6 +329,10 @@
     if (!group_uses_generic(a) || (group_lds_bytes(a) <= (size_t)kGenericLdsLimit && a.A <= (unsigned)kMaxA)) return 0;
     return (size_t)kBigBlocks * (a.step == 2 ? 2 : 1) * a.N * a.A * a.k * a.k * sizeof(float);
 }
+bool group_rotates_filt_rows(const GroupArgs& a) {
+    if ((a.opt & kOptGroupGeneric) || a.filt_sai_stride) return false;
+    return group_ht_rotates(a) || group_wiener_rotates(a);
+}
 hipError_t launch_group(hipStream_t s, const GroupArgs& a) {
     hipLaunchKernelGGL(k_group_pos, grid1d((size_t)a.n_groups * a.N), dim3(256), 0, s, a);
     const bool bigA = a.A > (unsigned)kMaxA;
diff --git a/lfbm5d_amd/csrc/lfbm5d_group_ht.hip b/lfbm5d_amd/csrc/lfbm5d_group_ht.hip
--- a/lfbm5d_amd/csrc/lfbm5d_group_ht.hip
+++ b/lfbm5d_amd/csrc/lfbm5d_group_ht.hip
@@ -202,6 +202,7 @@
     const int voff = (int)(((unsigned)(pq / k) * a.Wb + pq % k) * 4u);
     const int woff = (pq / k) * (k + 1) + pq % k;
     unsigned okbits[NS];
+    unsigned rotbits[NS];
     typedef const __attribute__((address_space(4))) unsigned* cuptr_;
     const cuptr_ ofs = (cuptr_)(a.gofs + (size_t)g * a.N * A), ok = (cuptr_)(a.gok + (size_t)g * a.N);
     const unsigned cbase = (unsigned)c * plane * 4u;
@@ -213,12 +214,13 @@
                 for (int st = 0; st < 9; st++) {
                     const float x = work[(n * A + st) * kT16Patch + woff];
                     if (n < NH) V[n][st].x = x; else V[n - NH][st].y = x;
-                    okbits[n] = 0x1ffu;
+                    okbits[n] = 0x1ffu; rotbits[n] = 0u;
                 }
         } else
 #pragma unroll
         for (int n = 0; n < NS; n++) {
-            okbits[n] = ok[n];
+            const unsigned okw = ok[n];
+            okbits[n] = okw & 0x1ffu; rotbits[n] = okw >> 9;
 #pragma unroll
             for (int st = 0; st < 9; st++) {
                 const unsigned so = ofs[n * A + st] + cbase;
@@ -245,14 +247,15 @@
     if (FAST) near = group_id_compute_fast<NS>(a, c, V, wacc, s1, s2);
     else
     group_id_compute<NS, HAAR, SA_MODE>(a, c, sh, use_sadct, V, wacc, s1, s2);
-    const int vout = pq * 4;
+    const int vout = pq * 4, vout1 = (int)((filt_rot_slot((unsigned)(pq / k), 1u, (unsigned)k) * (unsigned)k + (unsigned)(pq % k)) * 4u);
 #pragma unroll
     for (int n = 0; n < NS; n++)
 #pragma unroll
         for (int st = 0; st < 9; st++) {
             const float r = n < NH ? V[n][st].x : V[n - NH][st].y;
             if (LDSW) work[(n * A + st) * kT16Patch + woff] = r;
-            else __builtin_amdgcn_raw_buffer_store_b32(__builtin_bit_cast(int, r), rs_out, vout, (int)((((unsigned)(n * A + st) * a.C + c) * k2) * 4u), kFiltStoreAux);
+            else __builtin_amdgcn_raw_buffer_store_b32(__builtin_bit_cast(int, r), rs_out, ((rotbits[n] >> st) & 1u) ? vout1 : vout,
+                                                       (int)((((unsigned)(n * A + st) * a.C + c) * k2) * 4u), kFiltStoreAux);
         }
     return near;
 }
@@ -594,9 +597,14 @@
     return hipSuccess;
 }
 
+static bool group_ht_register_resident(const GroupArgs& a) {
+    return a.tau2 == 4 && a.N <= 8 && a.k * a.k <= 256 && a.step == 1 && a.A == 9 && (size_t)a.A * a.C * a.Wb * a.Hb * 4 < 0x7fffffffull;
+}
+bool group_ht_rotates(const GroupArgs& a) { return group_ht_register_resident(a) && a.k == 16; }
+
 hipError_t launch_group_ht(hipStream_t s, const GroupArgs& a, bool all_sa, bool* launched) {
     *launched = true;
-    if (a.tau2 == 4 && a.N <= 8 && a.k * a.k <= 256 && a.step == 1 && a.A == 9 && (size_t)a.A * a.C * a.Wb * a.Hb * 4 < 0x7fffffffull) {
+    if (group_ht_register_resident(a)) {
         const unsigned threads = ((a.k * a.k + 63) / 64) * 64;
         const unsigned gx = ((a.n_groups + 7) / 8) * 8;
         if (all_sa) {
diff --git a/lfbm5d_amd/csrc/lfbm5d_group_wiener.hip b/lfbm5d_amd/csrc/lfbm5d_group_wiener.hip
--- a/lfbm5d_amd/csrc/lfbm5d_group_wiener.hip
+++ b/lfbm5d_amd/csrc/lfbm5d_group_wiener.hip
@@ -889,7 +889,7 @@
 }
 
 template <int NS, int TH, bool SA>
-__device__ __forceinline__ void w3_body(const GroupArgs& a, float* S, const unsigned* pos, float (*red)[TH / 64], int tid,
+__device__ __forceinline__ void w3_body(const GroupArgs& a, float* S, const unsigned* pos, const unsigned char* rot, float (*red)[TH / 64], int tid,
                                         unsigned g, int c) {
     constexpr int A = 9, K2 = 64, NP = NS * A, NPh = (NP + 1) / 2, NPf = kW3Stride;
     static_assert(TH == 256, "the fibre phases deal st 0..3 / 4..7 to 256 threads");
@@ -1057,11 +1057,12 @@
 #pragma unroll
         for (int j = 0; j < 8; j++) x[j] = v2f{ra[j * NPf], ra[j * NPf + (NP > NPh ? NPh : 0)]};
         dct8_inv_t(x);
-        v4f* oa = reinterpret_cast<v4f*>(a.filt + ((size_t)g * N * A + pa) * a.C * K2 + (size_t)c * K2 + i * 8);
+        float* const pa0 = a.filt + ((size_t)g * N * A + pa) * a.C * K2 + (size_t)c * K2;
+        v4f* oa = reinterpret_cast<v4f*>(pa0 + filt_rot_slot((unsigned)i, rot[pa], 8u) * 8u);
         filt_put4_nt(oa, v4f{x[0].x, x[1].x, x[2].x, x[3].x});
         filt_put4_nt(oa + 1, v4f{x[4].x, x[5].x, x[6].x, x[7].x});
         if (has_b) {
-            v4f* ob = oa + (size_t)NPh * a.C * (K2 / 4);
+            v4f* ob = reinterpret_cast<v4f*>(pa0 + (size_t)NPh * a.C * K2 + filt_rot_slot((unsigned)i, rot[pa + NPh], 8u) * 8u);
             filt_put4_nt(ob, v4f{x[0].y, x[1].y, x[2].y, x[3].y});
             filt_put4_nt(ob + 1, v4f{x[4].y, x[5].y, x[6].y, x[7].y});
         }
@@ -1069,7 +1070,7 @@
 }
 
 template <int NS, int TH>
-__device__ __forceinline__ void w3_body_u(const GroupArgs& a, float* S, const unsigned* pos, float (*red)[TH / 64], int tid, unsigned g, int c) {
+__device__ __forceinline__ void w3_body_u(const GroupArgs& a, float* S, const unsigned* pos, const unsigned char* rot, float (*red)[TH / 64], int tid, unsigned g, int c) {
     constexpr int A = 9, K2 = 64, NP = NS * A, NPh = (NP + 1) / 2, NPf = kW3Stride;
     constexpr int L = NS == 16 ? 4 : NS == 8 ? 3 : NS == 4 ? 2 : NS == 2 ? 1 : 0;
     static_assert(TH == 256, "the fibre phases deal st 0..3 / 4..7 to 256 threads");
@@ -1207,23 +1208,29 @@
 #pragma unroll
         for (int j = 0; j < 8; j++) x[j] = v2f{ra[j * NPf], ra[j * NPf + (NP > NPh ? NPh : 0)]};
         dct8_inv_t(x);
-        v4f* oa = reinterpret_cast<v4f*>(a.filt + ((size_t)g * N * A + pa) * a.C * K2 + (size_t)c * K2 + i * 8);
+        float* const pa0 = a.filt + ((size_t)g * N * A + pa) * a.C * K2 + (size_t)c * K2;
+        v4f* oa = reinterpret_cast<v4f*>(pa0 + filt_rot_slot((unsigned)i, rot[pa], 8u) * 8u);
         filt_put4_nt(oa, v4f{x[0].x, x[1].x, x[2].x, x[3].x});
         filt_put4_nt(oa + 1, v4f{x[4].x, x[5].x, x[6].x, x[7].x});
         if (has_b) {
-            v4f* ob = oa + (size_t)NPh * a.C * (K2 / 4);
+            v4f* ob = reinterpret_cast<v4f*>(pa0 + (size_t)NPh * a.C * K2 + filt_rot_slot((unsigned)i, rot[pa + NPh], 8u) * 8u);
             filt_put4_nt(ob, v4f{x[0].y, x[1].y, x[2].y, x[3].y});
             filt_put4_nt(ob + 1, v4f{x[4].y, x[5].y, x[6].y, x[7].y});
         }
     }
 }
 
+__device__ __forceinline__ unsigned w3_rot(const GroupArgs& a, unsigned g, int i) {
+    if (!a.filt_rot_mask) return 0u;
+    return filt_rot_d0(a.filt_rot_mask, a.filt_rot_org, a.aggpos[((size_t)(i % 9) * a.n_refs_total + g) * a.N + i / 9]);
+}
 constexpr int kW3SaWaves = 4;
 template <bool SA>
 __global__ __launch_bounds__(kDct8w3Threads) __attribute__((amdgpu_waves_per_eu(SA ? kW3SaWaves : 1))) void k_group_dct8w3(GroupArgs a) {
     extern __shared__ float lds[];
     __shared__ float red[3][kDct8w3Threads / 64];
     __shared__ unsigned pos[kMaxN * kA3];
+    __shared__ unsigned char rot[kMaxN * kA3];
     constexpr int TH = kDct8w3Threads;
     const int tid = threadIdx.x;
     const unsigned gi = xcd_group_index(a);
@@ -1235,14 +1242,15 @@
     for (int i = tid; i < nSx * 9; i += TH) {
         const unsigned p = a.gpos[(size_t)g * a.N * 9 + i];
         pos[i] = p != 0xffffffffu ? (((unsigned)(i % 9) * a.C + c) * plane + p) * 4u : kW3Empty;
+        rot[i] = (unsigned char)w3_rot(a, g, i);
     }
     __syncthreads();
     switch (nSx) {
-        case 1:  w3_body<1, TH, SA>(a, lds, pos, red, tid, g, c); break;
-        case 2:  w3_body<2, TH, SA>(a, lds, pos, red, tid, g, c); break;
-        case 4:  w3_body<4, TH, SA>(a, lds, pos, red, tid, g, c); break;
-        case 8:  w3_body<8, TH, SA>(a, lds, pos, red, tid, g, c); break;
-        default: w3_body<16, TH, SA>(a, lds, pos, red, tid, g, c); break;
+        case 1:  w3_body<1, TH, SA>(a, lds, pos, rot, red, tid, g, c); break;
+        case 2:  w3_body<2, TH, SA>(a, lds, pos, rot, red, tid, g, c); break;
+        case 4:  w3_body<4, TH, SA>(a, lds, pos, rot, red, tid, g, c); break;
+        case 8:  w3_body<8, TH, SA>(a, lds, pos, rot, red, tid, g, c); break;
+        default: w3_body<16, TH, SA>(a, lds, pos, rot, red, tid, g, c); break;
     }
 }
 
@@ -1250,6 +1258,7 @@
     extern __shared__ float lds[];
     __shared__ float red[3][kDct8w3Threads / 64];
     __shared__ unsigned pos[kMaxN * kA3];
+    __shared__ unsigned char rot[kMaxN * kA3];
     constexpr int TH = kDct8w3Threads;
     const int tid = threadIdx.x;
     const unsigned gi = xcd_group_index(a);
@@ -1262,14 +1271,15 @@
     for (int i = tid; i < nSx * 9; i += TH) {
         const unsigned p = a.gpos[(size_t)g * a.N * 9 + i];
         pos[i] = p != 0xffffffffu ? (((unsigned)(i % 9) * a.C + c) * plane + p) * 4u : kW3Empty;
+        rot[i] = (unsigned char)w3_rot(a, g, i);
     }
     __syncthreads();
     switch (nSx) {
-        case 1:  w3_body_u<1, TH>(a, lds, pos, red, tid, g, c); break;
-        case 2:  w3_body_u<2, TH>(a, lds, pos, red, tid, g, c); break;
-        case 4:  w3_body_u<4, TH>(a, lds, pos, red, tid, g, c); break;
-        case 8:  w3_body_u<8, TH>(a, lds, pos, red, tid, g, c); break;
-        default: w3_body_u<16, TH>(a, lds, pos, red, tid, g, c); break;
+        case 1:  w3_body_u<1, TH>(a, lds, pos, rot, red, tid, g, c); break;
+        case 2:  w3_body_u<2, TH>(a, lds, pos, rot, red, tid, g, c); break;
+        case 4:  w3_body_u<4, TH>(a, lds, pos, rot, red, tid, g, c); break;
+        case 8:  w3_body_u<8, TH>(a, lds, pos, rot, red, tid, g, c); break;
+        default: w3_body_u<16, TH>(a, lds, pos, rot, red, tid, g, c); break;
     }
 }
 constexpr unsigned kW3ListBlocks = 256;
@@ -1277,6 +1287,7 @@
     extern __shared__ float lds[];
     __shared__ float red[3][kDct8w3Threads / 64];
     __shared__ unsigned pos[kMaxN * kA3];
+    __shared__ unsigned char rot[kMaxN * kA3];
     constexpr int TH = kDct8w3Threads;
     const int tid = threadIdx.x;
     const unsigned n_list = a.sa_list[0];
@@ -1288,14 +1299,15 @@
         for (int i = tid; i < nSx * 9; i += TH) {
             const unsigned p = a.gpos[(size_t)g * a.N * 9 + i];
             pos[i] = p != 0xffffffffu ? (((unsigned)(i % 9) * a.C + c) * plane + p) * 4u : kW3Empty;
+            rot[i] = (unsigned char)w3_rot(a, g, i);
         }
         __syncthreads();
         switch (nSx) {
-            case 1:  w3_body<1, TH, true>(a, lds, pos, red, tid, g, c); break;
-            case 2:  w3_body<2, TH, true>(a, lds, pos, red, tid, g, c); break;
-            case 4:  w3_body<4, TH, true>(a, lds, pos, red, tid, g, c); break;
-            case 8:  w3_body<8, TH, true>(a, lds, pos, red, tid, g, c); break;
-            default: w3_body<16, TH, true>(a, lds, pos, red, tid, g, c); break;
+            case 1:  w3_body<1, TH, true>(a, lds, pos, rot, red, tid, g, c); break;
+            case 2:  w3_body<2, TH, true>(a, lds, pos, rot, red, tid, g, c); break;
+            case 4:  w3_body<4, TH, true>(a, lds, pos, rot, red, tid, g, c); break;
+            case 8:  w3_body<8, TH, true>(a, lds, pos, rot, red, tid, g, c); break;
+            default: w3_body<16, TH, true>(a, lds, pos, rot, red, tid, g, c); break;
         }
         __syncthreads();
     }
@@ -1454,6 +1466,12 @@
     return hipSuccess;
 }
 
+static bool group_wiener_w3(const GroupArgs& a) {
+    return a.tau2 == 5 && a.k == 8 && a.A == 9 && a.N <= (unsigned)kMaxN && a.step == 2 && a.tau5 == 9 &&
+           (size_t)9 * a.C * a.Wb * a.Hb * 4 < 0x70000000ull && !(a.opt & kOptDct8wV2);
+}
+bool group_wiener_rotates(const GroupArgs& a) { return group_wiener_w3(a); }
+
 hipError_t launch_group_wiener(hipStream_t s, const GroupArgs& a, bool all_sa, bool* launched) {
     *launched = true;
     if (a.tau2 == 7 && a.k == 8 && a.A == 9 && a.step == 2 && a.N <= (unsigned)kMaxN) {
@@ -1466,7 +1484,7 @@
         const size_t l8 = (size_t)(a.step == 2 ? 2 : 1) * 64 * ((a.N * 9) | 1) * sizeof(float);
         if (a.step == 2) {
             const unsigned gx = ((a.n_groups + 7) / 8) * 8;
-            if (a.tau5 == 9 && (size_t)9 * a.C * a.Wb * a.Hb * 4 < 0x70000000ull && !(a.opt & kOptDct8wV2)) {
+            if (group_wiener_w3(a)) {
                 if (all_sa) hipLaunchKernelGGL(k_group_dct8w3<true>, dim3(gx, a.C), dim3(kDct8w3Threads), kW3Lds, s, a);
                 else if (a.tau4 == 5 || a.tau4 == 6) {
                     if (!a.sa_list) return hipErrorInvalidValue;
diff --git a/lfbm5d_amd/csrc/lfbm5d_kernels.h b/lfbm5d_amd/csrc/lfbm5d_kernels.h
--- a/lfbm5d_amd/csrc/lfbm5d_kernels.h
+++ b/lfbm5d_amd/csrc/lfbm5d_kernels.h
@@ -107,6 +107,8 @@
     unsigned opt;
     unsigned long long filt_sai_stride;
     unsigned bm3d;
+    unsigned filt_rot_mask;
+    unsigned filt_rot_org;
 };
 
 constexpr unsigned kSaiMajorMinA = 121;
@@ -114,6 +116,11 @@
     return a.filt_sai_stride ? (size_t)st * a.filt_sai_stride + ((size_t)g * a.N + n) * a.C * k2
                              : (((size_t)g * a.N + n) * a.A + st) * a.C * k2;
 }
+__host__ __device__ __forceinline__ unsigned filt_rot_d0(unsigned mask, unsigned org, unsigned pos) {
+    return pos == 0xffffffffu ? 0u : (org - (pos >> 16)) & mask;
+}
+__host__ __device__ __forceinline__ unsigned filt_rot_slot(unsigned r, unsigned d0, unsigned k) { return (r - d0) & (k - 1u); }
+inline unsigned filt_rot_mask_of(unsigned k) { return (k >= 8 && 32u % k == 0 && 32u / k >= 2) ? 32u / k - 1u : 0u; }
 
 
 struct SaiList { unsigned st[kBigA]; unsigned n; };
@@ -143,6 +150,7 @@
     unsigned direct;
     unsigned long long lf_stride;
     SaiList sai;
+    unsigned filt_rot_mask, filt_rot_org;
 };
 
 __host__ __device__ inline size_t stereo_table_stride(unsigned W, unsigned H, unsigned k, unsigned nDisp) {
@@ -279,6 +287,7 @@
                                 unsigned* best, unsigned char* shape);
 hipError_t prepare_group_kernels();
 hipError_t launch_group(hipStream_t s, const GroupArgs& a);
+bool group_rotates_filt_rows(const GroupArgs& a);
 size_t group_lds_bytes(const GroupArgs& a);
 size_t group_scratch_bytes(const GroupArgs& a);
 hipError_t launch_aggregate(hipStream_t s, const AggArgs& a);
diff --git a/lfbm5d_amd/csrc/lfbm5d_options.h b/lfbm5d_amd/csrc/lfbm5d_options.h
--- a/lfbm5d_amd/csrc/lfbm5d_options.h
+++ b/lfbm5d_amd/csrc/lfbm5d_options.h
@@ -23,6 +23,7 @@
     kOptSubsetScanV1 = 1u << 11,
     kOptFiltGroupMajor = 1u << 12,
     kOptHtReferenceOrder = 1u << 13,
+    kOptFiltRowsPlain = 1u << 14,
 };
 
 struct Options {
@@ -64,6 +65,7 @@
         {"subset_list_host", "LFBM5D_SUBSET_LIST_HOST", nullptr, kOptSubsetListHost}, {"subset_scan_v1", "LFBM5D_SUBSET_SCAN_V1", nullptr, kOptSubsetScanV1},
         {"filt_group_major", "LFBM5D_FILT_GROUP_MAJOR", nullptr, kOptFiltGroupMajor},
         {"ht_reference_order", "LFBM5D_HT_REF_ORDER", nullptr, kOptHtReferenceOrder},
+        {"filt_rows_plain", "LFBM5D_FILT_ROWS_PLAIN", nullptr, kOptFiltRowsPlain},
     };
     *n = sizeof(keys) / sizeof(keys[0]);
     return keys;
diff --git a/lfbm5d_amd/csrc/lfbm5d_pass.hip b/lfbm5d_amd/csrc/lfbm5d_pass.hip
--- a/lfbm5d_amd/csrc/lfbm5d_pass.hip
+++ b/lfbm5d_amd/csrc/lfbm5d_pass.hip
@@ -442,6 +442,12 @@
         aa.num = c->direct.num; aa.den = c->direct.den; aa.direct = 1u; aa.lf_stride = c->direct.lf_stride; aa.sai = c->direct.sai;
     }
     const bool sai_major = A >= kSaiMajorMinA && !(c->opt->kernels & kOptFiltGroupMajor);
+    if (!sai_major && !(c->opt->kernels & kOptFiltRowsPlain)) {
+        ga.filt_rot_mask = filt_rot_mask_of(k); ga.filt_rot_org = direct ? nHW : 0u;
+        if (!group_rotates_filt_rows(ga)) ga.filt_rot_mask = 0u;
+    }
+    if (!ga.filt_rot_mask) ga.filt_rot_org = 0u;
+    aa.filt_rot_mask = ga.filt_rot_mask; aa.filt_rot_org = ga.filt_rot_org;
     const size_t per_group_bias = sai_major ? per_group / A : per_group;
     if (n_groups <= band_groups) {
         ga.filt_sai_stride = aa.filt_sai_stride = sai_major ? (unsigned long long)n_groups * (per_group / A) : 0ull;
```

Measured after the change: 250.6 SAI-megapixels/s. No clear change (-1.0%).
